# Streampunk/phaneron

Hardware: AMD Instinct MI355X
Metric: frames/sec, 4-layer 2160p50 composite pipeline (v210 unpack->CSC->combine->CSC->v210 pack) (higher is better)
Workload: dtype f32

## Files before the change

### include/phaneron_hip.h

```cpp
#ifndef PHANERON_HIP_H
#define PHANERON_HIP_H

#include <stddef.h>
#include <stdint.h>

#ifdef __cplusplus
extern "C" {
#endif

#define PH_ABI_VERSION 8

enum {
  PH_OK = 0,
  PH_E_INVALID = -1,
  PH_E_NO_DEVICE = -2,
  PH_E_HIP = -3,
  PH_E_UNKNOWN_KERNEL = -4,
  PH_E_RANGE = -5
};

typedef struct ph_ctx ph_ctx;
typedef struct ph_buf ph_buf;
typedef struct ph_program ph_program;

// ... 157 lines not shown
int ph_fused_v210_combine(ph_ctx *ctx, int queue, int n, const void *const *layers, void *out,
                          uint32_t width, uint32_t height, const void *rd_col_matrix12,
                          const void *rd_gamma_lut, const void *rd_gamut_matrix9,
                          const void *wr_col_matrix12, const void *wr_gamma_lut);
int ph_fused_v210_combine_batch(ph_ctx *ctx, int queue, int jobs, int n, const void *const *layers,
                                void *const *outs, uint32_t width, uint32_t height, const void *rd_col_matrix12,
                                const void *rd_gamma_lut, const void *rd_gamut_matrix9, const void *wr_col_matrix12,
                                const void *wr_gamma_lut);

typedef struct ph_layer {
  const void *rgba;
  int width, height;
  const void *matrix9;
} ph_layer;
int ph_compose_write_v210(ph_ctx *ctx, int queue, int n, const ph_layer *layers, void *out,
                          uint32_t out_width, uint32_t out_height, uint32_t interlace,
                          const void *wr_col_matrix12, const void *wr_gamma_lut);

typedef struct ph_layer_wipe {
  const void *incoming_rgba;
  const void *mask_rgba;
} ph_layer_wipe;
int ph_compose_wipe_write_v210(ph_ctx *ctx, int queue, int n, const ph_layer *layers, const ph_layer_wipe *wipes,
                               void *out, uint32_t out_width, uint32_t out_height, uint32_t interlace,
                               const void *wr_col_matrix12, const void *wr_gamma_lut);

typedef struct ph_image_layer {
  const void *data;
  int format;
  int width, height;
  const float *matrix9_host;
} ph_image_layer;
int ph_compose_up_write_v210(ph_ctx *ctx, int queue, int n, const ph_image_layer *layers, void *out, uint32_t out_width,
                             uint32_t out_height, uint32_t interlace, const void *wr_col_matrix12, const void *wr_gamma_lut);
int ph_compose_up_write_v210_pair(ph_ctx *ctx, int queue, int n, const ph_image_layer *layers_a, const ph_image_layer *layers_b, void *out_a,
                                  void *out_b, uint32_t out_width, uint32_t out_height, uint32_t interlace, const void *wr_col_matrix12,
                                  const void *wr_gamma_lut);
int ph_compose_up_write_v210_batch(ph_ctx *ctx, int queue, int jobs, int n, const ph_image_layer *const *layer_sets, void *const *outs,
                                   uint32_t out_width, uint32_t out_height, uint32_t interlace, const void *wr_col_matrix12,
                                   const void *wr_gamma_lut);

#define PH_SRC_NONE 0
#define PH_SRC_V210 1
#define PH_SRC_RGBA_F32 2
#define PH_SRC_YUV422P10 3
#define PH_SRC_YUV422P8 4
#define PH_SRC_YUV420P 5
#define PH_SRC_NV12 6
#define PH_SRC_RGBA8 7
#define PH_SRC_BGRA8 8
#define PH_SRC_YUV420P10 9
#define PH_SRC_P010 10
typedef struct ph_chan_source {
  const void *data;
  int format;
  int width, height;
  const float *matrix9_host;
  const void *data_u, *data_v;
  const void *col_matrix12;
} ph_chan_source;
#define PH_TRANSITION_CUT 0
#define PH_TRANSITION_DISSOLVE 1
#define PH_TRANSITION_WIPE 2
typedef struct ph_chan_layer {
  ph_chan_source src;
  int transition;
  float mix;
  ph_chan_source incoming, mask;
} ph_chan_layer;
int ph_chan_compose_v210(ph_ctx *ctx, int queue, int n, const ph_chan_layer *layers, void *out, uint32_t out_width,
                         uint32_t out_height, uint32_t interlace, const void *rd_col_matrix12, const void *rd_gamma_lut,
                         const void *rd_gamut9, const void *wr_col_matrix12, const void *wr_gamma_lut);
int ph_chan_compose(ph_ctx *ctx, int queue, int n, const ph_chan_layer *layers, int out_format, void *const out_planes[3],
                    uint32_t out_width, uint32_t out_height, uint32_t interlace, const void *rd_col_matrix12, const void *rd_gamma_lut,
                    const void *rd_gamut9, const void *wr_col_matrix12, const void *wr_gamma_lut);
typedef struct ph_chan_job {
  int n;
  const ph_chan_layer *layers;
  void *out;
  uint32_t interlace;
} ph_chan_job;
int ph_chan_compose_batch(ph_ctx *ctx, int queue, int n_jobs, const ph_chan_job *jobs, uint32_t out_width, uint32_t out_height,
                          const void *rd_col_matrix12, const void *rd_gamma_lut, const void *rd_gamut9, const void *wr_col_matrix12,
                          const void *wr_gamma_lut);
typedef struct ph_chan_output {
  int format;
  void *planes[3];
  uint32_t interlace;
  const void *wr_col_matrix12;
  const void *wr_gamma_lut;
} ph_chan_output;
int ph_chan_compose_multi(ph_ctx *ctx, int queue, int n, const ph_chan_layer *layers, int n_out, const ph_chan_output *outs,
                          uint32_t out_width, uint32_t out_height, const void *rd_col_matrix12, const void *rd_gamma_lut,
                          const void *rd_gamut9);
int ph_clip_compose_multi(ph_ctx *ctx, int queue, int n, const ph_chan_layer *layers, int n_out, const ph_chan_output *outs,
                          uint32_t out_width, uint32_t out_height, const void *rd_col_matrix12, const void *rd_gamma_lut,
                          const void *rd_gamut9);
typedef struct ph_chan_job_out {
  int n;
  const ph_chan_layer *layers;
  int n_out;
  const ph_chan_output *outs;
} ph_chan_job_out;
int ph_chan_compose_batch_out(ph_ctx *ctx, int queue, int n_jobs, const ph_chan_job_out *jobs, uint32_t out_width, uint32_t out_height,
                              const void *rd_col_matrix12, const void *rd_gamma_lut, const void *rd_gamut9);
int ph_clip_compose_batch_out(ph_ctx *ctx, int queue, int n_jobs, const ph_chan_job_out *jobs, uint32_t out_width, uint32_t out_height,
                              const void *rd_col_matrix12, const void *rd_gamma_lut, const void *rd_gamut9);
int ph_compose_up_write_multi(ph_ctx *ctx, int queue, int jobs, int n, const ph_image_layer *const *layer_sets, int n_out,
                              const ph_chan_output *outs, uint32_t out_width, uint32_t out_height);
typedef struct ph_image_trans_layer {
  ph_image_layer src;
  int transition;
  float mix;
  ph_image_layer incoming, mask;
} ph_image_trans_layer;
int ph_compose_up_transition_multi(ph_ctx *ctx, int queue, int jobs, int n, const ph_image_trans_layer *const *layer_sets, int n_out,
                                   const ph_chan_output *outs , uint32_t out_width, uint32_t out_height);
int ph_pack_write_multi(ph_ctx *ctx, int queue, const void *in, int n_out, const ph_chan_output *outs, uint32_t width,
                        uint32_t height);
int ph_fused_v210_combine_multi(ph_ctx *ctx, int queue, int n, const void *const *layers, int n_out, const ph_chan_output *outs,
                                uint32_t width, uint32_t height, const void *rd_col_matrix12, const void *rd_gamma_lut,
                                const void *rd_gamut9);
int ph_fused_v210_combine_multi_batch(ph_ctx *ctx, int queue, int jobs, int n, const void *const *layers ,
                                      int n_out, const ph_chan_output *outs , uint32_t width, uint32_t height,
                                      const void *rd_col_matrix12, const void *rd_gamma_lut, const void *rd_gamut9);
typedef struct ph_fused_layer {
  const void *v210;
  int transition;
  float mix;
  const void *incoming_v210;
  const void *mask;
  int mask_format;
} ph_fused_layer;
int ph_fused_v210_transition_multi(ph_ctx *ctx, int queue, int n, const ph_fused_layer *layers, int n_out, const ph_chan_output *outs,
                                   uint32_t width, uint32_t height, const void *rd_col_matrix12, const void *rd_gamma_lut,
                                   const void *rd_gamut9);
typedef struct ph_route_layer {
  const void *data;
  int format;
} ph_route_layer;
int ph_fused_v210_route_multi(ph_ctx *ctx, int queue, int n, const ph_route_layer *layers, void *image_out ,
                              int n_out , const ph_chan_output *outs, uint32_t width, uint32_t height, const void *rd_col_matrix12,
                              const void *rd_gamma_lut, const void *rd_gamut9);

int ph_lut_register(ph_ctx *ctx, const void *device_lut_f32, const float *host_lut65536);
int ph_lut_unregister(ph_ctx *ctx, const void *device_lut_f32);
int ph_lut_query(ph_ctx *ctx, const void *device_lut_f32, uint32_t *lds_bytes, uint32_t *index_bias,
                 uint32_t *blocks_per_octave_log2);
typedef struct ph_lut_layout {
  uint32_t lds_bytes, hole, delta_off, shift, index_bias;
  float a_scale;
} ph_lut_layout;
int ph_lut_layout_of(const float *host_lut65536, ph_lut_layout *layout, void *lds_image, size_t capacity);
int ph_ctx_set_option(ph_ctx *ctx, const char *name, int value);
int ph_debug_image_nt(ph_ctx *ctx, size_t bytes);

int ph_colour_gamma2linear_lut(const char *colspec, float *lut65536);
int ph_colour_linear2gamma_lut(const char *colspec, float *lut65536);
int ph_colour_ycbcr2rgb_matrix(const char *colspec, int num_bits, int luma_black, int luma_white,
                               int chroma_range, float *m12);
int ph_colour_rgb2ycbcr_matrix(const char *colspec, int num_bits, int luma_black, int luma_white,
                               int chroma_range, float *m12);
int ph_colour_rgb2rgb_matrix(const char *src_colspec, const char *dst_colspec, float *m9);
int ph_transform_matrix(int width, int height, int flip_h, int flip_v, double anchor_x,
                        double anchor_y, double scale_x, double scale_y, double offset_x,
                        double offset_y, double rotate, float *m9);

int ph_abi_version(void);

#ifdef __cplusplus
}
#endif
#endif
```

### phaneron_amd/capi.py

```python
import ctypes as C
import os
import sys

import numpy as np

_HERE = os.path.dirname(os.path.abspath(__file__))
LIB_PATH = os.environ.get("PHANERON_HIP_LIB") or os.path.join(_HERE, "lib", "libphaneron_hip.so")

QUEUE_LOAD, QUEUE_PROCESS, QUEUE_UNLOAD = 0, 1, 2
HOST_READONLY, HOST_WRITEONLY, HOST_NONE = 0, 1, 2
ARG_BUF, ARG_U32, ARG_I32, ARG_F32 = 0, 1, 2, 3

EXPORTS = [
    "ph_abi_version", "ph_last_error", "ph_ctx_create", "ph_ctx_destroy", "ph_ctx_info", "ph_ctx_stream",
    "ph_wait_finish", "ph_buf_create", "ph_buf_wrap", "ph_buf_addref", "ph_buf_release", "ph_buf_refcount",
    "ph_buf_bytes", "ph_buf_device_ptr", "ph_buf_dims", "ph_buf_host_access", "ph_buf_host_ptr",
    "ph_ctx_buffer_stats", "ph_program_create", "ph_program_destroy", "ph_program_kernel", "ph_run_program", "ph_check_program", "ph_chan_compose", "ph_yadif_pair_packed",
    "ph_v210_pitch_bytes", "ph_v210_read", "ph_v210_read_batch", "ph_v210_write", "ph_yadif", "ph_yadif_pair", "ph_v210_yadif_pair", "ph_transform", "ph_resize", "ph_combine",
    "ph_transition_dissolve", "ph_transition_wipe", "ph_mixer", "ph_wipe", "ph_fused_v210_combine",
    "ph_colour_gamma2linear_lut", "ph_colour_linear2gamma_lut", "ph_colour_ycbcr2rgb_matrix",
    "ph_colour_rgb2ycbcr_matrix", "ph_colour_rgb2rgb_matrix", "ph_transform_matrix",
    "ph_lut_register", "ph_lut_unregister", "ph_lut_query", "ph_lut_layout_of", "ph_compose_up_write_v210_pair", "ph_compose_up_write_v210_batch", "ph_pack_read_batch", "ph_ctx_set_option", "ph_compose_write_v210", "ph_compose_wipe_write_v210",
    "ph_pack_plane_bytes", "ph_pack_read", "ph_pack_write", "ph_queue_wait_queue", "ph_buf_download_async",
    "ph_event_record", "ph_event_wait", "ph_event_query", "ph_event_destroy", "ph_queue_query",
    "ph_graph_begin", "ph_graph_end", "ph_graph_launch", "ph_graph_destroy", "ph_fused_v210_combine_batch",
    "ph_program_resolve", "ph_route_unique_id", "ph_route_init", "ph_route_destroy", "ph_route_group_begin",
    "ph_route_group_end", "ph_route_send", "ph_route_recv", "ph_route_after_queue", "ph_queue_after_route",
    "ph_route_wait", "ph_route_stream", "ph_route_comm_count", "ph_chan_compose_v210", "ph_chan_compose_batch", "ph_run_programs", "ph_event_record_timed", "ph_event_elapsed_us", "ph_ctx_host_pool_stats",
    "ph_v210_yadif_pair_fmt", "ph_compose_up_write_v210", "ph_trace_begin", "ph_trace_end", "ph_run_programs_progress", "ph_buf_reuse", "ph_image_unpack_rgb",
    "ph_chan_compose_multi", "ph_compose_up_write_multi", "ph_chan_compose_batch_out", "ph_pack_write_multi",
    "ph_fused_v210_combine_multi",
    "ph_fused_v210_combine_multi_batch",
    "ph_compose_up_transition_multi",
    "ph_fused_v210_transition_multi",
    "ph_fused_v210_route_multi",
    "ph_debug_image_nt",
    "ph_clip_compose_multi",
    "ph_clip_compose_batch_out",
]


class PhaneronError(RuntimeError):
    pass


class _ArgVal(C.Union):
    _fields_ = [("buf", C.c_void_p), ("u32", C.c_uint32), ("i32", C.c_int32), ("f32", C.c_float)]


class PhArg(C.Structure):
    _fields_ = [("name", C.c_char_p), ("kind", C.c_int), ("v", _ArgVal)]


class PhLayer(C.Structure):
    _fields_ = [("rgba", C.c_void_p), ("width", C.c_int), ("height", C.c_int), ("matrix9", C.c_void_p)]


class PhLayerWipe(C.Structure):
    _fields_ = [("incoming_rgba", C.c_void_p), ("mask_rgba", C.c_void_p)]


class PhDeintSource(C.Structure):
    _fields_ = [("prev", C.c_void_p), ("cur", C.c_void_p), ("next", C.c_void_p), ("out_parity0", C.c_void_p), ("out_parity1", C.c_void_p),
                ("prev_u", C.c_void_p), ("prev_v", C.c_void_p), ("cur_u", C.c_void_p), ("cur_v", C.c_void_p), ("next_u", C.c_void_p), ("next_v", C.c_void_p)]


class PhChanSource(C.Structure):
    _fields_ = [("data", C.c_void_p), ("format", C.c_int), ("width", C.c_int), ("height", C.c_int),
                ("matrix9_host", C.POINTER(C.c_float)), ("data_u", C.c_void_p), ("data_v", C.c_void_p), ("col_matrix12", C.c_void_p)]


class PhChanLayer(C.Structure):
    _fields_ = [("src", PhChanSource), ("transition", C.c_int), ("mix", C.c_float), ("incoming", PhChanSource), ("mask", PhChanSource)]


class PhChanJob(C.Structure):
    _fields_ = [("n", C.c_int), ("layers", C.POINTER(PhChanLayer)), ("out", C.c_void_p), ("interlace", C.c_uint32)]


class PhChanOutput(C.Structure):
    _fields_ = [("format", C.c_int), ("planes", C.c_void_p * 3), ("interlace", C.c_uint32), ("wr_col_matrix12", C.c_void_p), ("wr_gamma_lut", C.c_void_p)]


class PhChanJobOut(C.Structure):
    _fields_ = [("n", C.c_int), ("layers", C.POINTER(PhChanLayer)), ("n_out", C.c_int), ("outs", C.POINTER(PhChanOutput))]


class PhImageLayer(C.Structure):
    _fields_ = [("data", C.c_void_p), ("format", C.c_int), ("width", C.c_int), ("height", C.c_int), ("matrix9_host", C.POINTER(C.c_float))]


class PhImageTransLayer(C.Structure):
    _fields_ = [("src", PhImageLayer), ("transition", C.c_int), ("mix", C.c_float), ("incoming", PhImageLayer), ("mask", PhImageLayer)]


class PhRouteLayer(C.Structure):
    _fields_ = [("data", C.c_void_p), ("format", C.c_int)]


class PhFusedLayer(C.Structure):
    _fields_ = [("v210", C.c_void_p), ("transition", C.c_int), ("mix", C.c_float), ("incoming_v210", C.c_void_p), ("mask", C.c_void_p), ("mask_format", C.c_int)]


IMG_RGBA_F32, IMG_RGB_F32 = 0, 1
SRC_V210, SRC_RGBA_F32, SRC_YUV422P10, SRC_YUV422P8, SRC_YUV420P, SRC_NV12, SRC_RGBA8, SRC_BGRA8 = 1, 2, 3, 4, 5, 6, 7, 8
SRC_YUV420P10, SRC_P010 = 9, 10
SRC_PLANAR = {"yuv422p10": SRC_YUV422P10, "yuv422p8": SRC_YUV422P8, "yuv420p": SRC_YUV420P, "nv12": SRC_NV12,
              "yuv420p10": SRC_YUV420P10, "p010": SRC_P010}
TRANSITION_CUT, TRANSITION_DISSOLVE, TRANSITION_WIPE = 0, 1, 2


class LutLayout(C.Structure):
    _fields_ = [("lds_bytes", C.c_uint32), ("hole", C.c_uint32), ("delta_off", C.c_uint32), ("shift", C.c_uint32), ("index_bias", C.c_uint32),
                ("a_scale", C.c_float)]


class RunTimings(C.Structure):
    _fields_ = [("data_to_kernel", C.c_uint32), ("kernel_exec", C.c_uint32), ("total_time", C.c_uint32)]


_lib = None


def lib():
    global _lib
    if _lib is not None:
        return _lib
    if not os.path.exists(LIB_PATH):
        raise PhaneronError("%s is missing: build it with `python -m phaneron_amd.build` "
                            "(there is no CPU fallback)" % LIB_PATH)
    if "torch" not in sys.modules and os.environ.get("PH_NO_TORCH_PRELOAD") != "1":
        import importlib.util
        if importlib.util.find_spec("torch") is not None:
            import torch
    l = C.CDLL(LIB_PATH)
    vp, ci, cu, cf, cd, cs = C.c_void_p, C.c_int, C.c_uint32, C.c_float, C.c_double, C.c_size_t
    f32p = np.ctypeslib.ndpointer(dtype=np.float32, flags="C_CONTIGUOUS")
    sig = {
        "ph_abi_version": (ci, []),
        "ph_last_error": (C.c_char_p, [vp]),
        "ph_ctx_create": (ci, [ci, C.POINTER(vp)]),
        "ph_ctx_destroy": (ci, [vp]),
        "ph_ctx_info": (ci, [vp, C.c_char_p, cs, C.c_char_p, cs]),
        "ph_ctx_stream": (vp, [vp, ci]),
        "ph_wait_finish": (ci, [vp, ci]),
        "ph_buf_create": (ci, [vp, cs, ci, ci, ci, ci, C.c_char_p, C.POINTER(vp)]),
        "ph_buf_wrap": (ci, [vp, vp, cs, ci, ci, C.POINTER(vp)]),
        "ph_buf_addref": (ci, [vp]),
        "ph_buf_release": (ci, [vp]),
        "ph_buf_refcount": (ci, [vp]),
        "ph_buf_bytes": (cs, [vp]),
        "ph_buf_device_ptr": (vp, [vp]),
        "ph_buf_dims": (ci, [vp, C.POINTER(ci), C.POINTER(ci)]),
        "ph_buf_host_access": (ci, [vp, ci, ci, vp, cs]),
        "ph_buf_host_ptr": (vp, [vp]),
        "ph_queue_wait_queue": (ci, [vp, ci, ci]),
        "ph_buf_download_async": (ci, [vp, ci]),
        "ph_queue_query": (ci, [vp, ci]),
        "ph_graph_begin": (ci, [vp, ci]),
        "ph_graph_end": (ci, [vp, ci, C.POINTER(vp)]),
        "ph_graph_launch": (ci, [vp, ci]),
        "ph_graph_destroy": (ci, [vp]),
        "ph_event_record": (ci, [vp, ci, C.POINTER(vp)]),
        "ph_event_wait": (ci, [vp]),
        "ph_event_query": (ci, [vp]),
        "ph_event_destroy": (ci, [vp]),
        "ph_ctx_buffer_stats": (ci, [vp, C.POINTER(cs), C.POINTER(cs), C.POINTER(cs)]),
        "ph_program_create": (ci, [vp, C.c_char_p, C.c_char_p, C.POINTER(cu), ci, cu, C.POINTER(vp)]),
        "ph_program_resolve": (ci, [C.c_char_p, C.c_char_p, C.c_char_p, cs, C.POINTER(ci), C.POINTER(ci)]),
        "ph_program_destroy": (ci, [vp]),
        "ph_program_kernel": (C.c_char_p, [vp]),
        "ph_run_program": (ci, [vp, vp, C.POINTER(PhArg), ci, ci, C.POINTER(RunTimings)]),
        "ph_check_program": (ci, [vp, vp, C.POINTER(PhArg), ci, ci]),
        "ph_v210_pitch_bytes": (cu, [cu]),
        "ph_v210_read": (ci, [vp, ci, vp, vp, cu, cu, vp, vp, vp]),
        "ph_v210_read_batch": (ci, [vp, ci, ci, vp, vp, cu, cu, vp, vp, vp]),
        "ph_v210_write": (ci, [vp, ci, vp, vp, cu, cu, cu, vp, vp]),
        "ph_yadif": (ci, [vp, ci, vp, vp, vp, ci, ci, ci, ci, ci, vp]),
        "ph_yadif_pair": (ci, [vp, ci, vp, vp, vp, ci, ci, ci, ci, vp, vp]),
        "ph_v210_yadif_pair": (ci, [vp, ci, ci, vp, cu, cu, ci, ci, vp, vp, vp]),
        "ph_v210_yadif_pair_fmt": (ci, [vp, ci, ci, vp, cu, cu, ci, ci, ci, vp, vp, vp]),
        "ph_yadif_pair_packed": (ci, [vp, ci, ci, vp, ci, cu, cu, ci, ci, ci, vp, vp, vp]),
        "ph_transform": (ci, [vp, ci, vp, ci, ci, vp, vp, ci, ci]),
        "ph_resize": (ci, [vp, ci, vp, ci, ci, cf, cf, cf, vp, vp, ci, ci]),
        "ph_combine": (ci, [vp, ci, ci, C.POINTER(vp), ci, ci, vp]),
        "ph_transition_dissolve": (ci, [vp, ci, vp, vp, cf, ci, ci, vp]),
        "ph_transition_wipe": (ci, [vp, ci, vp, vp, vp, ci, ci, vp]),
        "ph_mixer": (ci, [vp, ci, vp, vp, cf, ci, ci, vp]),
        "ph_wipe": (ci, [vp, ci, vp, vp, cf, ci, ci, vp]),
        "ph_fused_v210_combine": (ci, [vp, ci, ci, C.POINTER(vp), vp, cu, cu, vp, vp, vp, vp, vp]),
        "ph_fused_v210_combine_batch": (ci, [vp, ci, ci, ci, C.POINTER(vp), C.POINTER(vp), cu, cu, vp, vp, vp, vp, vp]),
        "ph_colour_gamma2linear_lut": (ci, [C.c_char_p, f32p]),
        "ph_colour_linear2gamma_lut": (ci, [C.c_char_p, f32p]),
        "ph_colour_ycbcr2rgb_matrix": (ci, [C.c_char_p, ci, ci, ci, ci, f32p]),
        "ph_colour_rgb2ycbcr_matrix": (ci, [C.c_char_p, ci, ci, ci, ci, f32p]),
        "ph_colour_rgb2rgb_matrix": (ci, [C.c_char_p, C.c_char_p, f32p]),
        "ph_transform_matrix": (ci, [ci, ci, ci, ci, cd, cd, cd, cd, cd, cd, cd, f32p]),
        "ph_lut_register": (ci, [vp, vp, f32p]),
        "ph_lut_unregister": (ci, [vp, vp]),
        "ph_lut_query": (ci, [vp, vp, C.POINTER(cu), C.POINTER(cu), C.POINTER(cu)]),
        "ph_lut_layout_of": (ci, [f32p, C.POINTER(LutLayout), vp, C.c_size_t]),
        "ph_compose_up_write_v210_pair": (ci, [vp, ci, ci, C.POINTER(PhImageLayer), C.POINTER(PhImageLayer), vp, vp, cu, cu, cu, vp, vp]),
        "ph_compose_up_write_v210_batch": (ci, [vp, ci, ci, ci, C.POINTER(C.POINTER(PhImageLayer)), C.POINTER(vp), cu, cu, cu, vp, vp]),
        "ph_pack_read_batch": (ci, [vp, ci, ci, ci, C.POINTER(vp * 3), C.POINTER(vp), cu, cu, vp, vp, vp]),
        "ph_ctx_set_option": (ci, [vp, C.c_char_p, ci]),
        "ph_pack_plane_bytes": (ci, [ci, cu, cu, C.POINTER(cs)]),
        "ph_pack_read": (ci, [vp, ci, ci, C.POINTER(vp), vp, cu, cu, vp, vp, vp]),
        "ph_pack_write": (ci, [vp, ci, ci, vp, C.POINTER(vp), cu, cu, cu, vp, vp]),
        "ph_compose_write_v210": (ci, [vp, ci, ci, C.POINTER(PhLayer), vp, cu, cu, cu, vp, vp]),
        "ph_compose_wipe_write_v210": (ci, [vp, ci, ci, C.POINTER(PhLayer), C.POINTER(PhLayerWipe), vp, cu, cu, cu, vp, vp]),
        "ph_compose_up_write_v210": (ci, [vp, ci, ci, C.POINTER(PhImageLayer), vp, cu, cu, cu, vp, vp]),
        "ph_chan_compose_v210": (ci, [vp, ci, ci, C.POINTER(PhChanLayer), vp, cu, cu, cu, vp, vp, vp, vp, vp]),
        "ph_chan_compose": (ci, [vp, ci, ci, C.POINTER(PhChanLayer), ci, C.POINTER(C.c_void_p), cu, cu, cu, vp, vp, vp, vp, vp]),
        "ph_chan_compose_batch": (ci, [vp, ci, ci, C.POINTER(PhChanJob), cu, cu, vp, vp, vp, vp, vp]),
        "ph_chan_compose_multi": (ci, [vp, ci, ci, C.POINTER(PhChanLayer), ci, C.POINTER(PhChanOutput), cu, cu, vp, vp, vp]),
        "ph_clip_compose_multi": (ci, [vp, ci, ci, C.POINTER(PhChanLayer), ci, C.POINTER(PhChanOutput), cu, cu, vp, vp, vp]),
        "ph_compose_up_write_multi": (ci, [vp, ci, ci, ci, C.POINTER(C.POINTER(PhImageLayer)), ci, C.POINTER(PhChanOutput), cu, cu]),
        "ph_compose_up_transition_multi": (ci, [vp, ci, ci, ci, C.POINTER(C.POINTER(PhImageTransLayer)), ci, C.POINTER(PhChanOutput), cu, cu]),
        "ph_pack_write_multi": (ci, [vp, ci, vp, ci, C.POINTER(PhChanOutput), cu, cu]),
        "ph_fused_v210_combine_multi": (ci, [vp, ci, ci, C.POINTER(C.c_void_p), ci, C.POINTER(PhChanOutput), cu, cu, vp, vp, vp]),
        "ph_fused_v210_transition_multi": (ci, [vp, ci, ci, C.POINTER(PhFusedLayer), ci, C.POINTER(PhChanOutput), cu, cu, vp, vp, vp]),
        "ph_fused_v210_route_multi": (ci, [vp, ci, ci, C.POINTER(PhRouteLayer), vp, ci, C.POINTER(PhChanOutput), cu, cu, vp, vp, vp]),
        "ph_fused_v210_combine_multi_batch": (ci, [vp, ci, ci, ci, C.POINTER(C.c_void_p), ci, C.POINTER(PhChanOutput), cu, cu, vp, vp, vp]),
        "ph_chan_compose_batch_out": (ci, [vp, ci, ci, C.POINTER(PhChanJobOut), cu, cu, vp, vp, vp]),
        "ph_clip_compose_batch_out": (ci, [vp, ci, ci, C.POINTER(PhChanJobOut), cu, cu, vp, vp, vp]),
        "ph_ctx_host_pool_stats": (ci, [vp, C.POINTER(C.c_size_t), C.POINTER(C.c_size_t), C.POINTER(C.c_size_t), C.POINTER(C.c_uint64)]),
        "ph_event_record_timed": (ci, [vp, ci, C.POINTER(vp)]),
        "ph_event_elapsed_us": (ci, [vp, vp, C.POINTER(cu)]),
        "ph_run_programs": (ci, [vp, ci, C.POINTER(vp), C.POINTER(C.POINTER(PhArg)), C.POINTER(ci), ci]),
        "ph_route_unique_id": (ci, [vp]),
        "ph_route_init": (ci, [vp, vp, ci, ci, C.POINTER(vp)]),
        "ph_route_destroy": (ci, [vp]),
        "ph_route_group_begin": (ci, [vp]),
        "ph_route_group_end": (ci, [vp]),
        "ph_route_send": (ci, [vp, vp, cs, ci]),
        "ph_route_recv": (ci, [vp, vp, cs, ci]),
        "ph_route_after_queue": (ci, [vp, ci]),
        "ph_queue_after_route": (ci, [vp, ci]),
        "ph_route_wait": (ci, [vp]),
        "ph_route_stream": (vp, [vp]),
        "ph_route_comm_count": (ci, [vp, C.POINTER(C.c_int)]),
        "ph_run_programs_progress": (ci, [C.POINTER(ci)]),
        "ph_buf_reuse": (ci, [vp]),
        "ph_image_unpack_rgb": (ci, [vp, ci, vp, ci, ci]),
        "ph_trace_begin": (ci, [ci]),
        "ph_trace_end": (ci, [C.c_char_p, cs]),
        "ph_debug_image_nt": (ci, [vp, cs]),
    }
    for name, (res, args) in sig.items():
        fn = getattr(l, name)
        fn.restype, fn.argtypes = res, args
    _lib = l
    return l


def check(rc, ctx=None):
    if rc != 0:
        msg = lib().ph_last_error(ctx)
        raise PhaneronError("libphaneron_hip error %d: %s" % (rc, msg.decode() if msg else "?"))


class trace:

    def __init__(self, dry_run=False):
        self.dry_run, self.route = dry_run, None

    def __enter__(self):
        check(lib().ph_trace_begin(1 if self.dry_run else 0))
        return self

    def __exit__(self, *exc):
        buf = C.create_string_buffer(4096)
        rc = lib().ph_trace_end(buf, len(buf))
        if exc[0] is None:
            check(rc)
        self.route = buf.value.decode()
        return False

    @property
    def kernels(self):
        return self.route.split("+") if self.route else []


def lut_layout(lut):
    lut = np.ascontiguousarray(lut, np.float32)
    assert lut.shape == (65536,)
    lay = LutLayout()
    n = lib().ph_lut_layout_of(lut, C.byref(lay), None, 0)
    if n < 0:
        check(n)
    if n == 0:
        return None, None
    image = np.zeros(n, np.uint8)
    if lib().ph_lut_layout_of(lut, C.byref(lay), image.ctypes.data_as(C.c_void_p), n) != n:
        check(-1)
    return {k: getattr(lay, k) for k, _ in LutLayout._fields_}, image


def gamma2linear_lut(colspec):
    out = np.empty(65536, np.float32)
    check(lib().ph_colour_gamma2linear_lut(colspec.encode(), out))
    return out


def linear2gamma_lut(colspec):
    out = np.empty(65536, np.float32)
    check(lib().ph_colour_linear2gamma_lut(colspec.encode(), out))
    return out


def ycbcr2rgb_matrix(colspec, num_bits=10, luma_black=64, luma_white=940, chroma_range=896):
    out = np.empty(12, np.float32)
    check(lib().ph_colour_ycbcr2rgb_matrix(colspec.encode(), num_bits, luma_black, luma_white, chroma_range, out))
    return out


def rgb2ycbcr_matrix(colspec, num_bits=10, luma_black=64, luma_white=940, chroma_range=896):
    out = np.empty(12, np.float32)
    check(lib().ph_colour_rgb2ycbcr_matrix(colspec.encode(), num_bits, luma_black, luma_white, chroma_range, out))
    return out


def rgb2rgb_matrix(src, dst):
    out = np.empty(9, np.float32)
    check(lib().ph_colour_rgb2rgb_matrix(src.encode(), dst.encode(), out))
    return out


def transform_matrix(width, height, flip_h=False, flip_v=False, anchor_x=0.0, anchor_y=0.0, scale_x=1.0,
                     scale_y=1.0, offset_x=0.0, offset_y=0.0, rotate=0.0):
    out = np.empty(9, np.float32)
    check(lib().ph_transform_matrix(width, height, int(flip_h), int(flip_v), anchor_x, anchor_y, scale_x, scale_y,
                                    offset_x, offset_y, rotate, out))
    return out


RESOLVED_HOW = {0: "tag", 1: "name", 2: "text", 3: "signature"}


def resolve_program(source, name):
    buf = C.create_string_buffer(64)
    fmt, how = C.c_int(), C.c_int()
    src = source.encode() if isinstance(source, str) else source
    check(lib().ph_program_resolve(src, name.encode(), buf, 64, C.byref(fmt), C.byref(how)))
    names = {v: k for k, v in FORMATS.items()}
    return buf.value.decode(), names.get(fmt.value), RESOLVED_HOW[how.value]


def v210_pitch_bytes(width):
    return int(lib().ph_v210_pitch_bytes(width))


FORMATS = {"v210": 0, "yuv422p10": 1, "yuv422p8": 2, "yuv420p": 3, "nv12": 4, "rgba8": 5, "bgra8": 6, "yuv420p10": 7, "p010": 8}
FORMAT_RANGE = {"v210": (10, 64, 940, 896), "yuv422p10": (10, 64, 940, 896), "yuv422p8": (8, 16, 235, 224),
                "yuv420p": (8, 16, 235, 224), "nv12": (8, 16, 235, 224), "rgba8": None, "bgra8": None,
                "yuv420p10": (10, 64, 940, 896), "p010": (10, 64, 940, 896)}


def pack_plane_bytes(fmt, width, height):
    b = (C.c_size_t * 3)()
    n = lib().ph_pack_plane_bytes(FORMATS[fmt], width, height, b)
    if n < 0:
        check(n)
    return [int(b[i]) for i in range(n)]


def _ptr(t):
    return C.c_void_p(t if isinstance(t, int) else t.data_ptr())


class Context:

    def __init__(self, device_index=0):
        h = C.c_void_p()
        check(lib().ph_ctx_create(device_index, C.byref(h)))
        self.h = h
        self.device_index = device_index

    def close(self):
        if self.h:
            lib().ph_ctx_destroy(self.h)
            self.h = None

    def __enter__(self):
        return self

    def __exit__(self, *a):
        self.close()

    def info(self):
        v, d = C.create_string_buffer(128), C.create_string_buffer(256)
        check(lib().ph_ctx_info(self.h, v, 128, d, 256), self.h)
        return v.value.decode(), d.value.decode()

    def stream_ptr(self, queue=QUEUE_PROCESS):
        return lib().ph_ctx_stream(self.h, queue)

    def torch_stream(self, queue=QUEUE_PROCESS):
        import torch
        return torch.cuda.ExternalStream(self.stream_ptr(queue), device=torch.device("cuda", self.device_index))

    def wait(self, queue=QUEUE_PROCESS):
        check(lib().ph_wait_finish(self.h, queue), self.h)

    def register_lut(self, device_lut, host_lut):
        rc = lib().ph_lut_register(self.h, _ptr(device_lut), np.ascontiguousarray(host_lut, np.float32))
        if rc < 0:
            check(rc, self.h)
        return rc == 1

    def unregister_lut(self, device_lut):
        check(lib().ph_lut_unregister(self.h, _ptr(device_lut)), self.h)

    def lut_info(self, device_lut):
        b, t, s = C.c_uint32(), C.c_uint32(), C.c_uint32()
        check(lib().ph_lut_query(self.h, _ptr(device_lut), C.byref(b), C.byref(t), C.byref(s)), self.h)
        return dict(lds_bytes=b.value, index_bias=t.value, blocks_per_octave_log2=s.value)

    def set_option(self, name, value):
        check(lib().ph_ctx_set_option(self.h, name.encode(), int(value)), self.h)

    def debug_image_nt(self, nbytes):
        rc = lib().ph_debug_image_nt(self.h, int(nbytes))
        if rc < 0:
            check(rc, self.h)
        return rc

    def v210_read(self, src, dst, width, height, col_matrix, lut, gamut, queue=QUEUE_PROCESS):
        check(lib().ph_v210_read(self.h, queue, _ptr(src), _ptr(dst), width, height, _ptr(col_matrix), _ptr(lut),
                                 _ptr(gamut)), self.h)

    def v210_read_batch(self, srcs, dsts, width, height, col_matrix, lut, gamut, queue=QUEUE_PROCESS):
        n = len(srcs)
        ins = (C.c_void_p * n)(*[_ptr(b).value for b in srcs])
        outs = (C.c_void_p * n)(*[_ptr(b).value for b in dsts])
        check(lib().ph_v210_read_batch(self.h, queue, n, ins, outs, width, height, _ptr(col_matrix), _ptr(lut), _ptr(gamut)), self.h)

    def v210_write(self, src, dst, width, height, interlace, col_matrix, lut, queue=QUEUE_PROCESS):
        check(lib().ph_v210_write(self.h, queue, _ptr(src), _ptr(dst), width, height, interlace, _ptr(col_matrix),
                                  _ptr(lut)), self.h)

    def yadif(self, prev, cur, nxt, dst, width, height, parity, tff, skip_spatial=False, queue=QUEUE_PROCESS):
        check(lib().ph_yadif(self.h, queue, _ptr(prev), _ptr(cur), _ptr(nxt), width, height, int(parity), int(tff),
                             int(skip_spatial), _ptr(dst)), self.h)

    def yadif_pair(self, prev, cur, nxt, dst_parity0, dst_parity1, width, height, tff, skip_spatial=False, queue=QUEUE_PROCESS):
        check(lib().ph_yadif_pair(self.h, queue, _ptr(prev), _ptr(cur), _ptr(nxt), width, height, int(tff), int(skip_spatial),
                                  _ptr(dst_parity0), _ptr(dst_parity1)), self.h)

    def v210_yadif_pair(self, sources, width, height, tff, skip_spatial, col_matrix, lut, gamut, queue=QUEUE_PROCESS, rgb=False,
                        prepare_only=False, packing="v210"):
        arr = (PhDeintSource * len(sources))()
        for i, s in enumerate(sources):
            if packing == "v210":
                arr[i].prev, arr[i].cur, arr[i].next = (_ptr(b).value for b in s[:3])
            else:
                (arr[i].prev, arr[i].prev_u, arr[i].prev_v), (arr[i].cur, arr[i].cur_u, arr[i].cur_v), (arr[i].next, arr[i].next_u, arr[i].next_v) = (
                    (tuple(_ptr(p).value for p in frame) + (None,))[:3] for frame in s[:3])
            arr[i].out_parity0, arr[i].out_parity1 = _ptr(s[3]).value, _ptr(s[4]).value
        args = (self.h, queue, len(sources), arr, FORMATS[packing], width, height, int(tff), int(skip_spatial), IMG_RGB_F32 if rgb else IMG_RGBA_F32,
                _ptr(col_matrix), _ptr(lut), _ptr(gamut))
        if prepare_only:
            fn, h = lib().ph_yadif_pair_packed, self.h

            def job(_keep=(sources,)):
                check(fn(*args), h)
            return job
        check(lib().ph_yadif_pair_packed(*args), self.h)

    def compose_up_write_v210_pair(self, layers_a, layers_b, dst_a, dst_b, out_w, out_h, interlace, wr_cm, wr_lut, queue=QUEUE_PROCESS, rgb=False,
                                   prepare_only=False):
        import numpy as np
        keep = []

        def arr_of(layers):
            arr = (PhImageLayer * len(layers))()
            for i, (t, w, h, m) in enumerate(layers):
                mh = np.ascontiguousarray(m, np.float32)
                keep.append(mh)
                arr[i].data, arr[i].width, arr[i].height = _ptr(t).value, w, h
                arr[i].format = IMG_RGB_F32 if rgb else IMG_RGBA_F32
                arr[i].matrix9_host = mh.ctypes.data_as(C.POINTER(C.c_float))
            return arr
        assert len(layers_a) == len(layers_b)
        aa, ab = arr_of(layers_a), arr_of(layers_b)
        args = (self.h, queue, len(layers_a), aa, ab, _ptr(dst_a), _ptr(dst_b), out_w, out_h, interlace, _ptr(wr_cm), _ptr(wr_lut))
        if prepare_only:
            fn, h = lib().ph_compose_up_write_v210_pair, self.h

            def job(_keep=(keep, layers_a, layers_b, dst_a, dst_b, aa, ab)):
                check(fn(*args), h)
            return job
        check(lib().ph_compose_up_write_v210_pair(*args), self.h)

    def compose_up_write_v210_batch(self, layer_sets, dsts, out_w, out_h, interlace, wr_cm, wr_lut, queue=QUEUE_PROCESS, rgb=False, prepare_only=False):
        import numpy as np
        keep = []
        arrs = []
        for layers in layer_sets:
            arr = (PhImageLayer * len(layers))()
            for i, (t, w, h, m) in enumerate(layers):
                mh = np.ascontiguousarray(m, np.float32)
                keep.append(mh)
                arr[i].data, arr[i].width, arr[i].height = _ptr(t).value, w, h
                arr[i].format = IMG_RGB_F32 if rgb else IMG_RGBA_F32
                arr[i].matrix9_host = mh.ctypes.data_as(C.POINTER(C.c_float))
            arrs.append(arr)
        sets = (C.POINTER(PhImageLayer) * len(arrs))(*[C.cast(a, C.POINTER(PhImageLayer)) for a in arrs])
        outs = (C.c_void_p * len(dsts))(*[_ptr(d).value for d in dsts])
        args = (self.h, queue, len(layer_sets), len(layer_sets[0]), sets, outs, out_w, out_h, interlace, _ptr(wr_cm), _ptr(wr_lut))
        if prepare_only:
            fn, h = lib().ph_compose_up_write_v210_batch, self.h

            def job(_keep=(keep, arrs, layer_sets, dsts, sets, outs)):
                check(fn(*args), h)
            return job
        check(lib().ph_compose_up_write_v210_batch(*args), self.h)

    def compose_up_write_v210(self, layers, dst, out_w, out_h, interlace, wr_cm, wr_lut, queue=QUEUE_PROCESS, rgb=False, prepare_only=False):
        import numpy as np
        arr = (PhImageLayer * len(layers))()
        keep = []
        for i, (t, w, h, m) in enumerate(layers):
            mh = np.ascontiguousarray(m, np.float32)
            keep.append(mh)
            arr[i].data, arr[i].width, arr[i].height = _ptr(t).value, w, h
            arr[i].format = IMG_RGB_F32 if rgb else IMG_RGBA_F32
            arr[i].matrix9_host = mh.ctypes.data_as(C.POINTER(C.c_float))
        args = (self.h, queue, len(layers), arr, _ptr(dst), out_w, out_h, interlace, _ptr(wr_cm), _ptr(wr_lut))
        if prepare_only:
            fn, h = lib().ph_compose_up_write_v210, self.h

            def job(_keep=(keep, layers, dst)):
                check(fn(*args), h)
            return job
        check(lib().ph_compose_up_write_v210(*args), self.h)

    def compose_up_write_multi(self, layer_sets, outputs, out_w, out_h, queue=QUEUE_PROCESS, rgb=False, prepare_only=False):
        import numpy as np
        keep = []
        arrs = []
        for layers in layer_sets:
            arr = (PhImageLayer * len(layers))()
            for i, (t, w, h, m) in enumerate(layers):
                mh = np.ascontiguousarray(m, np.float32)
                keep.append(mh)
                arr[i].data, arr[i].width, arr[i].height = _ptr(t).value, w, h
                arr[i].format = IMG_RGB_F32 if rgb else IMG_RGBA_F32
                arr[i].matrix9_host = mh.ctypes.data_as(C.POINTER(C.c_float))
            arrs.append(arr)
        sets = (C.POINTER(PhImageLayer) * len(arrs))(*[C.cast(a, C.POINTER(PhImageLayer)) for a in arrs])
        n_out = len(outputs[0])
        outs = (PhChanOutput * max(len(outputs) * n_out, 1))()
        for j, per_job in enumerate(outputs):
            if len(per_job) != n_out:
                raise PhaneronError("compose_up_write_multi: every set of layers needs the same number of outputs")
            for k, o in enumerate(per_job):
                d = outs[j * n_out + k]
                planes = o["planes"] if isinstance(o["planes"], (list, tuple)) else [o["planes"]]
                d.format = FORMATS[o["fmt"]]
                for i, p in enumerate(planes):
                    d.planes[i] = _ptr(p).value
                d.interlace = int(o.get("interlace", 0))
                d.wr_col_matrix12 = None if o.get("wr_cm") is None else _ptr(o["wr_cm"]).value
                d.wr_gamma_lut = _ptr(o["wr_lut"]).value
        args = (self.h, queue, len(layer_sets), len(layer_sets[0]), sets, n_out, outs, out_w, out_h)
        fn, h = lib().ph_compose_up_write_multi, self.h
        if prepare_only:

            def job(_keep=(keep, arrs, layer_sets, outputs, sets, outs)):
# ... 580 lines not shown
```

### phaneron_amd/csrc/ph_api.cpp

```cpp
#include <algorithm>
#include <atomic>
#include <chrono>
#include <cstdarg>
#include <cstdio>
#include <cstring>
#include <dlfcn.h>
#include <map>
#include <mutex>
#include <string>
#include <vector>

#include "../../include/phaneron_hip.h"
#include "ph_internal.h"
#include "ph_kernels.h"
#include "ph_lut_host.h"

using ph::KernelId;
using namespace ph;

namespace {
thread_local std::string g_err;
}

int fail(int code, const char *fmt, ...) {
// ... 632 lines not shown
int ph_route_unique_id(void *id128) {
  if (!id128) return fail(PH_E_INVALID, "ph_route_unique_id: NULL argument");
  int rc = load_rccl();
  if (rc) return rc;
  static_assert(PH_ROUTE_ID_BYTES == sizeof(Id128), "ncclUniqueId is 128 bytes");
  PH_NCCL(g_rccl.GetUniqueId(id128));
  return PH_OK;
}

int ph_route_init(ph_ctx *ctx, const void *id128, int rank, int world, ph_route **out) {
  if (!ctx || !id128 || !out) return fail(PH_E_INVALID, "ph_route_init: NULL argument");
  if (world < 1 || rank < 0 || rank >= world) return fail(PH_E_INVALID, "ph_route_init: rank %d of %d", rank, world);
  int rc = set_device(ctx);
  if (rc) return rc;
  rc = load_rccl();
  if (rc) return rc;
  Id128 id;
  memcpy(id.bytes, id128, sizeof id.bytes);
  void *comm = nullptr;
  PH_NCCL(g_rccl.CommInitRank(&comm, world, id, rank));
  hipStream_t s = nullptr;
  hipError_t e = hipStreamCreateWithFlags(&s, hipStreamNonBlocking);
  if (e != hipSuccess) {
    g_rccl.CommDestroy(comm);
    return fail(PH_E_HIP, "ph_route_init: hipStreamCreate: %s", hipGetErrorString(e));
  }
  hipEvent_t ev = nullptr;
  e = hipEventCreateWithFlags(&ev, hipEventDisableTiming);
  if (e != hipSuccess) {
    g_rccl.CommDestroy(comm);
    hipStreamDestroy(s);
    return fail(PH_E_HIP, "ph_route_init: hipEventCreate: %s", hipGetErrorString(e));
  }
  ph_route *r = new ph_route{ctx, comm, s, rank, world};
  r->last = ev;
  {
    std::lock_guard<std::mutex> lock(ctx->mu);
    ctx->routes.push_back(r);
  }
  *out = r;
  ctx_ref(ctx);
  return PH_OK;
}

int ph_route_destroy(ph_route *r) {
  if (!r) return PH_OK;
  hipSetDevice(r->ctx->device);
  hipStreamSynchronize(r->stream);
  ph_ctx *ctx = r->ctx;
  {
    std::lock_guard<std::mutex> lock(ctx->mu);
    for (size_t i = 0; i < ctx->routes.size(); ++i)
      if (ctx->routes[i] == r) {
        ctx->routes.erase(ctx->routes.begin() + (long)i);
        break;
      }
  }
  g_rccl.CommDestroy(r->comm);
  hipStreamDestroy(r->stream);
  if (r->last) hipEventDestroy(r->last);
  delete r;
  ctx_unref(ctx);
  return PH_OK;
}

int ph_route_group_begin(ph_route *r) {
  if (!r) return fail(PH_E_INVALID, "ph_route_group_begin: NULL route");
  PH_NCCL(g_rccl.GroupStart());
  r->in_group = true;
  return PH_OK;
}
int ph_route_group_end(ph_route *r) {
  if (!r) return fail(PH_E_INVALID, "ph_route_group_end: NULL route");
  int rc = set_device(r->ctx);
  if (rc) return rc;
  PH_NCCL(g_rccl.GroupEnd());
  r->in_group = false;
  return route_mark(r);
}

static int route_args(ph_route *r, const void *p, size_t bytes, int peer, const char *fn) {
  if (!r || !p) return fail(PH_E_INVALID, "%s: NULL argument", fn);
  if (bytes % 4) return fail(PH_E_INVALID, "%s: %zu bytes is not a multiple of 4", fn, bytes);
  if (peer < 0 || peer >= r->world) return fail(PH_E_INVALID, "%s: peer %d of %d ranks", fn, peer, r->world);
  return set_device(r->ctx);
}
int ph_route_send(ph_route *r, const void *src, size_t bytes, int peer) {
  int rc = route_args(r, src, bytes, peer, "ph_route_send");
  if (rc) return rc;
  PH_NCCL(g_rccl.Send(src, bytes / 4, kNcclUint32, peer, r->comm, r->stream));
  return r->in_group ? PH_OK : route_mark(r);
}
int ph_route_recv(ph_route *r, void *dst, size_t bytes, int peer) {
  int rc = route_args(r, dst, bytes, peer, "ph_route_recv");
  if (rc) return rc;
  PH_NCCL(g_rccl.Recv(dst, bytes / 4, kNcclUint32, peer, r->comm, r->stream));
  return r->in_group ? PH_OK : route_mark(r);
}

static int order_streams(ph_ctx *ctx, hipStream_t waiter, hipStream_t signal, const char *fn) {
  int rc = set_device(ctx);
  if (rc) return rc;
  hipEvent_t ev;
  PH_HIP(hipEventCreateWithFlags(&ev, hipEventDisableTiming));
  hipError_t e = hipEventRecord(ev, signal);
  if (e == hipSuccess) e = hipStreamWaitEvent(waiter, ev, 0);
  hipEventDestroy(ev);
  if (e != hipSuccess) return fail(PH_E_HIP, "%s: %s", fn, hipGetErrorString(e));
  return PH_OK;
}
int ph_route_after_queue(ph_route *r, int queue) {
  if (!r || queue < 0 || queue > 2) return fail(PH_E_INVALID, "ph_route_after_queue: bad argument");
  return order_streams(r->ctx, r->stream, r->ctx->streams[queue], "ph_route_after_queue");
}
int ph_queue_after_route(ph_route *r, int queue) {
  if (!r || queue < 0 || queue > 2) return fail(PH_E_INVALID, "ph_queue_after_route: bad argument");
  return order_streams(r->ctx, r->ctx->streams[queue], r->stream, "ph_queue_after_route");
}
int ph_route_wait(ph_route *r) {
  if (!r) return fail(PH_E_INVALID, "ph_route_wait: NULL route");
  int rc = set_device(r->ctx);
  if (rc) return rc;
  PH_HIP(hipStreamSynchronize(r->stream));
  return PH_OK;
}
void *ph_route_stream(ph_route *r) { return r ? (void *)r->stream : nullptr; }
int ph_route_comm_count(ph_route *r, int *count) {
  if (!r || !count) return fail(PH_E_INVALID, "ph_route_comm_count: NULL argument");
  PH_NCCL(g_rccl.CommCount(r->comm, count));
  return PH_OK;
}

int ph_ctx_buffer_stats(ph_ctx *ctx, size_t *live_buffers, size_t *live_bytes, size_t *pooled_bytes) {
  if (!ctx) return fail(PH_E_INVALID, "ph_ctx_buffer_stats: ctx is NULL");
  std::lock_guard<std::mutex> lock(ctx->mu);
  if (live_buffers) *live_buffers = ctx->live_buffers;
  if (live_bytes) *live_bytes = ctx->live_bytes;
  if (pooled_bytes) *pooled_bytes = ctx->pooled_bytes;
  return PH_OK;
}

int ph_ctx_host_pool_stats(ph_ctx *ctx, size_t *in_use_bytes, size_t *pooled_bytes, size_t *peak_in_use_bytes, uint64_t *pins) {
  if (!ctx) return fail(PH_E_INVALID, "ph_ctx_host_pool_stats: ctx is NULL");
  std::lock_guard<std::mutex> lock(ctx->mu);
  if (in_use_bytes) *in_use_bytes = ctx->host_live_bytes;
  if (pooled_bytes) *pooled_bytes = ctx->host_pooled_bytes;
  if (peak_in_use_bytes) *peak_in_use_bytes = ctx->host_peak_bytes;
  if (pins) *pins = ctx->host_pins;
  return PH_OK;
}

int ph_lut_unregister(ph_ctx *ctx, const void *dev) {
  if (!ctx) return fail(PH_E_INVALID, "ph_lut_unregister: ctx is NULL");
  void *blob = nullptr;
  {
    std::lock_guard<std::mutex> lock(ctx->mu);
    auto it = ctx->luts.find(dev);
    if (it == ctx->luts.end()) return PH_OK;
    blob = it->second.blob_dev;
    ctx->luts.erase(it);
  }
  if (blob) {
    for (int q = 0; q < 3; ++q) hipStreamSynchronize(ctx->streams[q]);
    hipFree(blob);
  }
  return PH_OK;
}

int ph_lut_register(ph_ctx *ctx, const void *dev, const float *host) {
  if (!ctx || !dev || !host) return fail(PH_E_INVALID, "ph_lut_register: NULL argument");
  int rc = set_device(ctx);
  if (rc) return rc;
  ph_lut_unregister(ctx, dev);
  std::vector<uint32_t> blob;
  ph::LutHostInfo info;
  LutEntry e;
  if (ph::lut_compress(host, ph::kLutMaxLdsBytes, blob, info)) {
    if (!ctx->lds_base_checked.load()) {
      uint32_t *probe = nullptr, base = ~0u;
      PH_HIP(hipMalloc(&probe, 4));
      hipError_t pe = ph::launch_lds_base_probe(ctx->streams[0], probe);
      if (pe == hipSuccess) pe = hipStreamSynchronize(ctx->streams[0]);
      if (pe == hipSuccess) pe = hipMemcpy(&base, probe, 4, hipMemcpyDeviceToHost);
      hipFree(probe);
      if (pe != hipSuccess) return fail(PH_E_HIP, "ph_lut_register: LDS base probe: %s", hipGetErrorString(pe));
      if (base != 0) return fail(PH_E_HIP, "ph_lut_register: dynamic shared memory starts at LDS address %u, not 0: the table kernels cannot run", base);
      ctx->lds_base_checked.store(true);
    }
    const size_t blob_bytes = blob.size() * sizeof(uint32_t);
    PH_HIP(hipMalloc(&e.blob_dev, blob_bytes));
    PH_HIP(hipMemcpy(e.blob_dev, blob.data(), blob_bytes, hipMemcpyHostToDevice));
    e.view = ph::lut_view(info, e.blob_dev);
  }
  {
    std::lock_guard<std::mutex> lock(ctx->mu);
    ctx->luts[dev] = e;
  }
  return e.view.bytes ? 1 : 0;
}

int ph_lut_layout_of(const float *host, ph_lut_layout *layout, void *lds_image, size_t capacity) {
  if (!host || !layout) return fail(PH_E_INVALID, "ph_lut_layout_of: NULL argument");
  std::vector<uint32_t> blob;
  ph::LutHostInfo info;
  memset(layout, 0, sizeof(*layout));
  if (!ph::lut_compress(host, ph::kLutMaxLdsBytes, blob, info)) return 0;
  const ph::LutView v = ph::lut_view(info, nullptr);
  layout->lds_bytes = info.bytes, layout->hole = info.hole, layout->delta_off = info.delta_off, layout->shift = info.shift;
  layout->index_bias = (uint32_t)info.bias, layout->a_scale = v.a_scale;
  if (lds_image) {
    if (capacity < info.bytes) return fail(PH_E_INVALID, "ph_lut_layout_of: the image needs %u bytes, %zu given", info.bytes, capacity);
    memset(lds_image, 0, info.hole);
    memcpy(static_cast<char *>(lds_image) + info.hole, blob.data(), info.bytes - info.hole);
  }
  return (int)info.bytes;
}

int ph_debug_fused_lut_k(const float *host, uint32_t k5[5]) {
  if (!host || !k5) return fail(PH_E_INVALID, "ph_debug_fused_lut_k: NULL argument");
  std::vector<uint32_t> blob;
  ph::LutHostInfo info;
  if (!ph::lut_compress(host, ph::kLutMaxLdsBytes, blob, info)) return 0;
  const ph::FusedLutK k = ph::fused_lut_k(ph::lut_view(info, nullptr));
  memcpy(k5, &k, 5 * sizeof(uint32_t));
  return (int)info.bytes;
}
uint32_t ph_debug_fused_job_of(uint32_t wg_per_job, uint32_t block) {
  return wg_per_job ? ph::fused_job_of(block, ph::fused_wg_magic(wg_per_job)) : 0;
}
int ph_debug_image_nt(ph_ctx *ctx, size_t bytes) {
  if (!ctx) return fail(PH_E_INVALID, "ph_debug_image_nt: ctx is NULL");
  if (int rc = set_device(ctx)) return rc;
  return (int)ph::image_nt(bytes);
}

int ph_lut_query(ph_ctx *ctx, const void *dev, uint32_t *lds_bytes, uint32_t *toe, uint32_t *shift) {
  if (!ctx) return fail(PH_E_INVALID, "ph_lut_query: ctx is NULL");
  std::lock_guard<std::mutex> lock(ctx->mu);
  auto it = ctx->luts.find(dev);
  const bool have = it != ctx->luts.end();
  if (lds_bytes) *lds_bytes = have ? it->second.view.bytes : 0;
  if (toe) *toe = have ? (uint32_t)it->second.view.bias : 0;
  if (shift) *shift = have ? 23 - it->second.view.shift : 0;
  return PH_OK;
}

int ph_ctx_set_option(ph_ctx *ctx, const char *name, int value) {
  if (!ctx || !name) return fail(PH_E_INVALID, "ph_ctx_set_option: NULL argument");
  if (0 == strcmp(name, "lds_lut")) return ctx->use_lds_lut = (value != 0), PH_OK;
  if (0 == strcmp(name, "stream_images")) {
    if (value < 0 || value > 2) return fail(PH_E_INVALID, "stream_images: 0 (cached), 1 (streamed) or 2 (by size)");
    return ctx->stream_images = value, PH_OK;
  }
  if (0 == strcmp(name, "stream_threshold_mb")) {
    if (value < 0) return fail(PH_E_INVALID, "stream_threshold_mb: a size in MiB");
    return ctx->stream_threshold_mb = value, PH_OK;
  }
  if (0 == strcmp(name, "fail_launches")) return ctx->fail_launches.store(value), PH_OK;
  if (0 == strcmp(name, "chan_enlarged")) return ctx->chan_enlarged = (value < 0 || value > 2 ? 1 : value), PH_OK;
  if (0 == strcmp(name, "chan_batch_outs")) {
    if (value != 0 && value != 1) return fail(PH_E_INVALID, "chan_batch_outs: 0 (a launch per such job) or 1 (shared launches)");
    return ctx->chan_batch_outs = value, PH_OK;
  }
  if (0 == strcmp(name, "clip_batch")) {
    if (value != 0 && value != 1) return fail(PH_E_INVALID, "clip_batch: 0 (a launch per such job) or 1 (shared launches)");
    return ctx->clip_batch = value, PH_OK;
  }
  if (0 == strcmp(name, "fused_multi_wgs")) {
    if (value < 0) return fail(PH_E_INVALID, "fused_multi_wgs: a number of workgroups, or 0 for no cap");
    return ctx->fused_multi_wgs = value, PH_OK;
  }
  if (0 == strcmp(name, "fused_multi_batch")) {
    if (value != 0 && value != 1) return fail(PH_E_INVALID, "fused_multi_batch: 0 (a launch per such job) or 1 (shared launches)");
    return ctx->fused_multi_batch = value, PH_OK;
  }
  if (0 == strcmp(name, "host_pool_mb")) {
    if (value < 0) return fail(PH_E_INVALID, "host_pool_mb: a size in MiB");
    std::vector<ph_ctx::HostBlock> drop;
    {
      std::lock_guard<std::mutex> lock(ctx->mu);
      ctx->host_pool_mb = value;
      ctx->host_peak_bytes = ctx->host_live_bytes;
      while (ctx->host_pooled_bytes > (size_t)value << 20 && !ctx->host_pool.empty()) {
        auto it = std::prev(ctx->host_pool.end());
        ctx->host_pooled_bytes -= it->first;
        drop.push_back(it->second);
        ctx->host_pool.erase(it);
      }
    }
    for (auto &v : drop) {
      hipHostFree(v.p);
      if (v.busy) hipEventDestroy(v.busy);
    }
    return PH_OK;
  }
  return fail(PH_E_INVALID, "unknown option '%s'", name);
}

struct LutRef {
  ph::LutView view{};
  bool found = false;
  const ph::LutView *get() const { return found ? &view : nullptr; }
};
static LutRef lds_view(ph_ctx *ctx, const void *dev) {
  LutRef r;
  if (!ctx || !ctx->use_lds_lut) return r;
  std::lock_guard<std::mutex> lock(ctx->mu);
  auto it = ctx->luts.find(dev);
  if (it == ctx->luts.end() || !it->second.view.bytes) return r;
  r.view = it->second.view, r.found = true;
  return r;
}

extern "C++" void refresh_buf_lut(ph_ctx *ctx, ph_buf *b) {
  if (b->lut_dirty && b->hptr && b->bytes >= 65536 * 4) {
    hipStreamSynchronize(ctx->streams[PH_QUEUE_LOAD]);
    ph_lut_register(ctx, b->dptr, (const float *)b->hptr);
    b->lut_dirty = false;
  }
}

extern "C++" int chan_out_refused(const char *fn, int fmt) {
  return fail(PH_E_INVALID, "%s: the channel kernel does not write %s frames - run the separate kernels: the channel's frame as an image, then the format's writer (ph_pack_write)", fn,
              fmt_name(fmt));
}

extern "C++" bool inject_failure(ph_ctx *ctx) {
  const int v = ctx->fail_launches.load();
  if (v > 0) return true;
  if (v < 0 && ctx->fail_launches.fetch_add(1) == -1) ctx->fail_launches.store(1);
  return false;
}

uint32_t ph_v210_pitch_bytes(uint32_t width) { return width ? ph::v210_pitch_bytes(width) : 0; }

#define PH_LAUNCH(expr)                                                                         \
  do {                                                                                          \
    if (!ctx) return fail(PH_E_INVALID, "%s: ctx is NULL", __func__);                           \
    PH_QUEUE(__func__, queue);                                                                  \
    int rc_ = set_device(ctx);                                                                  \
    if (rc_) return rc_;                                                                        \
    hipError_t e_ = ph::trace_launch(#expr) ? hipSuccess : (expr);                              \
    if (e_ != hipSuccess) return fail(PH_E_HIP, "%s: launch failed: %s", __func__, hipGetErrorString(e_)); \
    return PH_OK;                                                                               \
  } while (0)

int ph_v210_read(ph_ctx *ctx, int queue, const void *in, void *out, uint32_t width, uint32_t height, const void *cm,
                 const void *lut, const void *gm) {
  if (!in || !out || !cm || !lut || !gm || !width) return fail(PH_E_INVALID, "ph_v210_read: NULL/zero argument");
  if (!height) return PH_OK;
  if (ctx && width % 2 == 0) {
    const LutRef lref = lds_view(ctx, lut);
    if (const ph::LutView *v = lref.get())
      PH_LAUNCH(ph::launch_v210_read_lds(stream_of(ctx, queue), in, out, width, height, cm, gm, *v,
                                         (uint32_t)ctx->props.multiProcessorCount));
  }
  PH_LAUNCH(ph::launch_v210_read(stream_of(ctx, queue), in, out, width, height, cm, lut, gm));
}

int ph_v210_read_batch(ph_ctx *ctx, int queue, int n, const void *const *ins, void *const *outs, uint32_t width,
                       uint32_t height, const void *cm, const void *lut, const void *gm) {
  if (n < 1 || n > ph::kMaxLayers) return fail(PH_E_INVALID, "ph_v210_read_batch: 1..%d frames", ph::kMaxLayers);
  if (!ins || !outs || !cm || !lut || !gm || !width) return fail(PH_E_INVALID, "ph_v210_read_batch: NULL/zero argument");
  for (int i = 0; i < n; ++i)
    if (!ins[i] || !outs[i]) return fail(PH_E_INVALID, "ph_v210_read_batch: frame %d is NULL", i);
  if (!height) return PH_OK;
  if (ctx && width % 2 == 0) {
    const LutRef lref = lds_view(ctx, lut);
    if (const ph::LutView *v = lref.get())
      PH_LAUNCH(ph::launch_v210_read_lds_batch(stream_of(ctx, queue), n, ins, outs, width, height, cm, gm, *v,
                                               (uint32_t)ctx->props.multiProcessorCount));
  }
  for (int i = 0; i < n; ++i) {
    const int rc = ph_v210_read(ctx, queue, ins[i], outs[i], width, height, cm, lut, gm);
    if (rc) return rc;
  }
  return PH_OK;
}

int ph_v210_write(ph_ctx *ctx, int queue, const void *in, void *out, uint32_t width, uint32_t height,
                  uint32_t interlace, const void *cm, const void *lut) {
  if (!in || !out || !cm || !lut || !width) return fail(PH_E_INVALID, "ph_v210_write: NULL/zero argument");
  if (interlace != 0 && interlace != 1 && interlace != 3) return fail(PH_E_INVALID, "ph_v210_write: interlace must be 0, 1 or 3");
  if (!height) return PH_OK;
  if (ctx && width % 2 == 0) {
    const LutRef lref = lds_view(ctx, lut);
    if (const ph::LutView *v = lref.get())
      PH_LAUNCH(ph::launch_v210_write_lds(stream_of(ctx, queue), in, out, width, height, interlace, cm, *v,
                                          (uint32_t)ctx->props.multiProcessorCount));
  }
  PH_LAUNCH(ph::launch_v210_write(stream_of(ctx, queue), in, out, width, height, interlace, cm, lut));
}

int ph_fused_v210_combine(ph_ctx *ctx, int queue, int n, const void *const *layers, void *out, uint32_t width,
                          uint32_t height, const void *rd_cm, const void *rd_lut, const void *rd_gm,
                          const void *wr_cm, const void *wr_lut) {
  if (n < 1 || n > ph::kMaxLayers) return fail(PH_E_INVALID, "ph_fused_v210_combine: 1..%d layers", ph::kMaxLayers);
  if (!layers || !out || !rd_cm || !rd_lut || !rd_gm || !wr_cm || !wr_lut || !width)
    return fail(PH_E_INVALID, "ph_fused_v210_combine: NULL/zero argument");
  const bool ragged = width % 48 != 0;
  if (width & 1) return fail(PH_E_INVALID, "ph_fused_v210_combine: width %u is odd; run the separate kernels", width);
  if (!height) return PH_OK;
  ph::FusedArgs a{};
  for (int i = 0; i < n; ++i) {
    if (!layers[i]) return fail(PH_E_INVALID, "ph_fused_v210_combine: layer %d is NULL", i);
    a.layers[i] = layers[i];
  }
  a.out = out;
  a.quads_per_line_used = width / 6;
  a.quads_per_line_pitch = ph::v210_pitch_bytes(width) / 16;
  a.total_quads = (ragged ? a.quads_per_line_pitch : a.quads_per_line_used) * height;
  a.tail_px = width % 6, a.magic_qpp = (uint32_t)(((1ull << 32) + a.quads_per_line_pitch - 1) / a.quads_per_line_pitch);
  if (ragged && (uint64_t)a.total_quads * a.quads_per_line_pitch >= (1ull << 32))
    return fail(PH_E_INVALID, "ph_fused_v210_combine: a %u x %u frame with ragged lines is too large; run the separate kernels", width, height);
  a.rd_cm = (const float *)rd_cm, a.rd_lut = (const float *)rd_lut, a.rd_gm = (const float *)rd_gm;
  a.wr_cm = (const float *)wr_cm, a.wr_lut = (const float *)wr_lut;
  if (ctx) {
    const LutRef rref = lds_view(ctx, rd_lut), wref = lds_view(ctx, wr_lut);
    const ph::LutView *rv = rref.get(), *wv = wref.get();
    if (rv && wv) {
      const ph::FusedLdsArgs la = ph::fused_lds_args(a, *rv, *wv);
      PH_LAUNCH(ph::launch_fused_v210_combine_lds(stream_of(ctx, queue), n, la, (uint32_t)ctx->props.multiProcessorCount));
    }
  }
  PH_LAUNCH(ph::launch_fused_v210_combine(stream_of(ctx, queue), n, a));
}

int ph_pack_plane_bytes(int format, uint32_t width, uint32_t height, size_t bytes[3]) {
  if (!bytes || !width) return fail(PH_E_INVALID, "ph_pack_plane_bytes: NULL/zero argument");
  if (const int rc = even_dims("ph_pack_plane_bytes", format, width, height)) return rc;
  const int n = ph::pack_plane_bytes(format, width, height, bytes);
  return n < 0 ? fail(PH_E_INVALID, "ph_pack_plane_bytes: unknown format %d", format) : n;
}

int ph_fused_v210_combine_batch(ph_ctx *ctx, int queue, int jobs, int n, const void *const *layers, void *const *outs,
                                uint32_t width, uint32_t height, const void *rd_cm, const void *rd_lut, const void *rd_gm,
                                const void *wr_cm, const void *wr_lut) {
  if (jobs < 1 || jobs > ph::kMaxBatch) return fail(PH_E_INVALID, "ph_fused_v210_combine_batch: 1..%d jobs", ph::kMaxBatch);
  if (n < 1 || n > ph::kMaxLayers) return fail(PH_E_INVALID, "ph_fused_v210_combine_batch: 1..%d layers", ph::kMaxLayers);
  if (!layers || !outs || !rd_cm || !rd_lut || !rd_gm || !wr_cm || !wr_lut)
    return fail(PH_E_INVALID, "ph_fused_v210_combine_batch: NULL argument");
  for (int j = 0; j < jobs; ++j) {
    if (!outs[j]) return fail(PH_E_INVALID, "ph_fused_v210_combine_batch: output %d is NULL", j);
    for (int l = 0; l < n; ++l)
      if (!layers[j * n + l]) return fail(PH_E_INVALID, "ph_fused_v210_combine_batch: job %d layer %d is NULL", j, l);
  }
  const LutRef rref = lds_view(ctx, rd_lut), wref = lds_view(ctx, wr_lut);
  const ph::LutView *rv = rref.get(), *wv = wref.get();
  if (jobs == 1 || !rv || !wv || !width || width % 48 || !height) {
    for (int j = 0; j < jobs; ++j) {
      int rc = ph_fused_v210_combine(ctx, queue, n, layers + (size_t)j * n, outs[j], width, height, rd_cm, rd_lut, rd_gm,
                                     wr_cm, wr_lut);
      if (rc != PH_OK) return rc;
    }
    return PH_OK;
  }
  ph::FusedArgs f{};
  for (int l = 0; l < n; ++l) f.layers[l] = layers[l];
  f.out = outs[0];
  f.quads_per_line_used = width / 6;
  f.quads_per_line_pitch = ph::v210_pitch_bytes(width) / 16;
  f.total_quads = f.quads_per_line_used * height;
  f.rd_cm = (const float *)rd_cm, f.rd_lut = (const float *)rd_lut, f.rd_gm = (const float *)rd_gm;
  f.wr_cm = (const float *)wr_cm, f.wr_lut = (const float *)wr_lut;
  ph::FusedLdsArgs la = ph::fused_lds_args(f, *rv, *wv);
  la.jobs = (uint32_t)jobs;
  for (int j = 1; j < jobs; ++j) {
    for (int l = 0; l < n; ++l) la.more_layers[j - 1][l] = layers[(size_t)j * n + l];
    la.more_out[j - 1] = outs[j];
  }
  PH_LAUNCH(ph::launch_fused_v210_combine_lds(stream_of(ctx, queue), n, la, (uint32_t)ctx->props.multiProcessorCount));
}

int ph_pack_read(ph_ctx *ctx, int queue, int format, const void *const planes[3], void *out, uint32_t width,
                 uint32_t height, const void *cm, const void *lut, const void *gm) {
  if (!ctx || !planes || !out || !lut || !gm || !width) return fail(PH_E_INVALID, "ph_pack_read: NULL/zero argument");
  if (format == PH_FMT_V210) return ph_v210_read(ctx, queue, planes[0], out, width, height, cm, lut, gm);
  if (const int rc = even_dims("ph_pack_read", format, width, height)) return rc;
  size_t pb[3];
  const int np = ph::pack_plane_bytes(format, width, height, pb);
  if (np < 0) return fail(PH_E_INVALID, "ph_pack_read: unknown format %d", format);
  for (int i = 0; i < np; ++i)
    if (!planes[i]) return fail(PH_E_INVALID, "ph_pack_read: plane %d is NULL", i);
  if (!fmt_rgb8(format) && !cm) return fail(PH_E_INVALID, "ph_pack_read: YCbCr formats need a colMatrix");
  if (!height) return PH_OK;
  PH_LAUNCH(ph::launch_pack_read(stream_of(ctx, queue), format, planes, out, width, height, cm, lut, gm, lds_view(ctx, lut).get(),
                                 (uint32_t)ctx->props.multiProcessorCount));
}

int ph_pack_read_batch(ph_ctx *ctx, int queue, int format, int n, const void *const (*planes)[3], void *const *outs, uint32_t width, uint32_t height,
                       const void *cm, const void *lut, const void *gm) {
  if (!ctx || !planes || !outs || !lut || !gm || !width) return fail(PH_E_INVALID, "ph_pack_read_batch: NULL/zero argument");
  if (n < 1 || n > ph::kMaxLayers) return fail(PH_E_INVALID, "ph_pack_read_batch: 1..%d frames", ph::kMaxLayers);
  if (const int rc = even_dims("ph_pack_read_batch", format, width, height)) return rc;
  const LutRef lref = lds_view(ctx, lut);
  const ph::LutView *v = format == PH_FMT_V210 ? nullptr : lref.get();
  if (n == 1 || !v) {
    if (format == PH_FMT_V210) {
      const void *ins[ph::kMaxLayers];
      for (int i = 0; i < n; ++i) ins[i] = planes[i][0];
      return ph_v210_read_batch(ctx, queue, n, ins, outs, width, height, cm, lut, gm);
    }
    for (int i = 0; i < n; ++i) {
      const int rc = ph_pack_read(ctx, queue, format, planes[i], outs[i], width, height, cm, lut, gm);
      if (rc) return rc;
    }
    return PH_OK;
  }
  size_t pb[3];
  const int np = ph::pack_plane_bytes(format, width, height, pb);
  if (np < 0) return fail(PH_E_INVALID, "ph_pack_read_batch: unknown format %d", format);
  for (int i = 0; i < n; ++i) {
    if (!outs[i]) return fail(PH_E_INVALID, "ph_pack_read_batch: output %d is NULL", i);
    for (int k = 0; k < np; ++k)
      if (!planes[i][k]) return fail(PH_E_INVALID, "ph_pack_read_batch: frame %d: plane %d is NULL", i, k);
  }
  if (!fmt_rgb8(format) && !cm) return fail(PH_E_INVALID, "ph_pack_read_batch: YCbCr formats need a colMatrix");
  if (!height) return PH_OK;
  PH_LAUNCH(ph::launch_pack_read_batch(stream_of(ctx, queue), format, n, planes, outs, width, height, cm, gm, *v, (uint32_t)ctx->props.multiProcessorCount));
}

int ph_pack_write(ph_ctx *ctx, int queue, int format, const void *in, void *const planes[3], uint32_t width,
                  uint32_t height, uint32_t interlace, const void *cm, const void *lut) {
  if (!ctx || !planes || !in || !lut || !width) return fail(PH_E_INVALID, "ph_pack_write: NULL/zero argument");
  if (interlace != 0 && interlace != 1 && interlace != 3) return fail(PH_E_INVALID, "ph_pack_write: interlace must be 0, 1 or 3");
  if (format == PH_FMT_V210) return ph_v210_write(ctx, queue, in, planes[0], width, height, interlace, cm, lut);
  if (const int rc = even_dims("ph_pack_write", format, width, height)) return rc;
  size_t pb[3];
  const int np = ph::pack_plane_bytes(format, width, height, pb);
  if (np < 0) return fail(PH_E_INVALID, "ph_pack_write: unknown format %d", format);
  for (int i = 0; i < np; ++i)
    if (!planes[i]) return fail(PH_E_INVALID, "ph_pack_write: plane %d is NULL", i);
  if (!fmt_rgb8(format) && !cm) return fail(PH_E_INVALID, "ph_pack_write: YCbCr formats need a colMatrix");
  if (!height) return PH_OK;
  PH_LAUNCH(ph::launch_pack_write(stream_of(ctx, queue), format, in, planes, width, height, interlace, cm, lut,
                                  lds_view(ctx, lut).get(), (uint32_t)ctx->props.multiProcessorCount));
}

int ph_pack_write_multi(ph_ctx *ctx, int queue, const void *in, int n_out, const ph_chan_output *outs, uint32_t width, uint32_t height) {
  const char *const fn = "ph_pack_write_multi";
  if (!ctx || !in || !outs || !width) return fail(PH_E_INVALID, "%s: NULL/zero argument", fn);
  if (n_out < 1 || n_out > ph::kMaxPackOuts) return fail(PH_E_INVALID, "%s: 1..%d outputs (%d)", fn, ph::kMaxPackOuts, n_out);
  if (n_out == 1)
    return ph_pack_write(ctx, queue, outs[0].format, in, outs[0].planes, width, height, outs[0].interlace, outs[0].wr_col_matrix12, outs[0].wr_gamma_lut);
  PH_QUEUE(fn, queue);
  for (int k = 0; k < n_out; ++k) {
    const ph_chan_output &o = outs[k];
    if (!o.wr_gamma_lut) return fail(PH_E_INVALID, "%s: output %d: the writer's gamma LUT is missing", fn, k);
    if (!fmt_known(o.format)) return fail(PH_E_INVALID, "%s: output %d: unknown format %d", fn, k, o.format);
    if (o.interlace != 0 && o.interlace != 1 && o.interlace != 3) return fail(PH_E_INVALID, "%s: output %d: interlace must be 0, 1 or 3", fn, k);
    if (const int rc = even_dims(fn, o.format, width, height)) return rc;
    for (int i = 0; i < fmt_planes(o.format); ++i)
      if (!o.planes[i]) return fail(PH_E_INVALID, "%s: output %d: plane %d is NULL", fn, k, i);
    if (!fmt_rgb8(o.format) && !o.wr_col_matrix12) return fail(PH_E_INVALID, "%s: output %d: YCbCr formats need a colMatrix", fn, k);
    for (int j = 0; j < k; ++j)
      if (outs[j].planes[0] == o.planes[0]) return fail(PH_E_INVALID, "%s: outputs %d and %d name the same plane", fn, j, k);
  }
  if (!height) return PH_OK;
  struct Launch {
    int solo;
    ph::PackMultiArgs m;
  };
  std::vector<Launch> launches;
  for (int k = 0; k < n_out; ++k) {
    bool seen = false;
    for (int j = 0; j < k; ++j) seen = seen || outs[j].wr_gamma_lut == outs[k].wr_gamma_lut;
    if (seen) continue;
    const LutRef wref = lds_view(ctx, outs[k].wr_gamma_lut);
    int group[ph::kMaxPackOuts], members = 0, share = 0;
    bool shared_ok[ph::kMaxPackOuts];
    for (int j = k; j < n_out; ++j) {
      if (outs[j].wr_gamma_lut != outs[k].wr_gamma_lut) continue;
      const int f = outs[j].format;
      shared_ok[members] = wref.get() && !(f == PH_FMT_V210 && width % 48) && !(fmt_planar(f) && width % 8);
      share += shared_ok[members] ? 1 : 0;
      group[members++] = j;
    }
    Launch shared{};
    shared.solo = -1;
    for (int g = 0; g < members; ++g) {
      const ph_chan_output &o = outs[group[g]];
      if (!shared_ok[g] || share < 2) {
        Launch own{};
        own.solo = group[g];
        launches.push_back(own);
        continue;
      }
      ph::PackOut &d = shared.m.out[shared.m.n_out++];
      d.fmt = (uint32_t)o.format;
      d.pitch = o.format == PH_FMT_V210 ? width / 6u : ph::pack_pitch(o.format, width);
      d.wr_cm = fmt_rgb8(o.format) ? nullptr : (const float *)o.wr_col_matrix12;
      for (int i = 0; i < 3; ++i) d.plane[i] = i < fmt_planes(o.format) ? o.planes[i] : nullptr;
      d.takes = o.interlace;
    }
    if (!shared.m.n_out) continue;
    ph::PackMultiArgs &m = shared.m;
    const uint32_t first_il = m.out[0].takes;
    bool same_lines = true;
    for (uint32_t i = 0; i < m.n_out; ++i) same_lines = same_lines && m.out[i].takes == first_il;
    const uint32_t il = same_lines ? first_il : 0u;
    m.in = in, m.width = width, m.wr = *wref.get();
    m.line_step = il ? 2 : 1, m.first_line = il == 3 ? 1 : 0, m.lines = il ? height / 2 : height;
    for (uint32_t i = 0; i < m.n_out; ++i) {
      ph::PackOut &d = m.out[i];
      const uint32_t oil = d.takes;
      d.takes = same_lines || !oil ? 0u : oil == 1 ? 1u : 2u;
      d.line_end = oil || fmt_v420((int)d.fmt) ? 2u * (height / 2u) : height;
      d.field = oil ? 1u : 0u;
    }
    launches.push_back(shared);
  }
  int rc = set_device(ctx);
  if (rc) return rc;
  for (const Launch &l : launches) {
    if (l.solo >= 0) {
      const ph_chan_output &o = outs[l.solo];
      if ((rc = ph_pack_write(ctx, queue, o.format, in, o.planes, width, height, o.interlace, o.wr_col_matrix12, o.wr_gamma_lut))) return rc;
      continue;
// ... 1670 lines not shown
```

### phaneron_amd/csrc/ph_internal.h

```cpp
#pragma once
#include <atomic>
#include <cstdlib>
#include <map>
#include <mutex>
#include <string>
#include <vector>

#include "../../include/phaneron_hip.h"
#include "ph_kernels.h"
#include "ph_program.h"
#include "ph_spans.h"

static_assert(ph::kSpanLayers == ph::kMaxLayers && ph::kSpanOuts >= ph::kMaxChanOuts && ph::kSpanOuts >= ph::kMaxFusedOuts && ph::kSpanOuts >= ph::kMaxUpOuts,
              "a Footprint holds any job's ranges: ph_spans.h sizes it by these limits without seeing ph_kernels.h");
static_assert(ph::kMaxChanOps <= ph::kSpanLayers * 3, "a channel job's op list is at most three sources per layer");

#pragma GCC visibility push(hidden)
int fail(int code, const char *fmt, ...) __attribute__((format(printf, 2, 3)));
#pragma GCC visibility pop

#define PH_HIP(call)                                                                          \
  do {                                                                                        \
    hipError_t e_ = (call);                                                                   \
    if (e_ != hipSuccess) return fail(PH_E_HIP, "%s failed: %s", #call, hipGetErrorString(e_)); \
  } while (0)

struct LutEntry {
  ph::LutView view{};
  void *blob_dev = nullptr;
};

struct ph_ctx {
  int device = 0;
  std::map<const void *, LutEntry> luts;
  bool use_lds_lut = true;
  int stream_images = 0;
  int stream_threshold_mb = 64;
  hipStream_t streams[3] = {nullptr, nullptr, nullptr};
  hipDeviceProp_t props;
  std::multimap<size_t, void *> pool;
  size_t pooled_bytes = 0, live_buffers = 0, live_bytes = 0;
  struct HostBlock {
    void *p;
    hipEvent_t busy;
    uint64_t seq;
  };
  std::multimap<size_t, HostBlock> host_pool;
  size_t host_pooled_bytes = 0;
  uint64_t host_pool_seq = 0;
  int chan_enlarged = !(getenv("PH_CHAN_ENLARGED") && getenv("PH_CHAN_ENLARGED")[0] == '0');
  int chan_batch_outs = 0;
  int clip_batch = 0;
  int fused_multi_wgs = 0;
  int fused_multi_batch = 0;
  std::atomic<int> fail_launches{0};
  int host_pool_mb = 4096;
  size_t host_live_bytes = 0, host_peak_bytes = 0;
  uint64_t host_pins = 0;
  void *chan_index[3] = {nullptr, nullptr, nullptr};
  size_t chan_index_bytes[3] = {0, 0, 0};
  std::mutex chan_scratch_mu[3];
  unsigned chan_scratch_turn[3] = {0, 0, 0};
  std::vector<struct ph_route *> routes;
  std::mutex mu;
  std::atomic<int> refs{1};
  std::atomic<bool> closed{false};
  std::atomic<bool> lds_base_checked{false};
};

struct ph_buf {
  ph_ctx *ctx;
  void *dptr;
  void *hptr;
  size_t bytes;
  int width, height;
  std::atomic<int> refs;
  bool owned;
  std::atomic<bool> host_dirty;
  std::atomic<bool> lut_dirty;
  std::string owner;
  hipEvent_t mirror_busy = nullptr;
  hipStream_t mirror_stream = nullptr;
};

struct ph_program {
  ph_ctx *ctx;
  ph::KernelId id;
  int n_layers;
  int format;
  std::string kernel;
  uint32_t global[2];
  uint32_t local;
};

#pragma GCC visibility push(hidden)
int set_device(ph_ctx *ctx);
void ctx_ref(ph_ctx *ctx);
void ctx_unref(ph_ctx *ctx);
int closed_error(const char *fn);
void refresh_buf_lut(ph_ctx *ctx, ph_buf *b);
void mirror_mark(ph_buf *b, hipStream_t s);
int chan_out_refused(const char *fn, int fmt);
bool inject_failure(ph_ctx *ctx);

inline bool queue_ok(int queue) { return queue >= 0 && queue < 3; }
inline int bad_queue(const char *fn, int queue) {
  return fail(PH_E_INVALID, "%s: queue %d is not PH_QUEUE_LOAD (0), PH_QUEUE_PROCESS (1) or PH_QUEUE_UNLOAD (2)", fn, queue);
}
#pragma GCC visibility pop
#define stream_of(ctx, queue)                                  \
  ({                                                           \
    const int ph_q_ = (queue);                                 \
    if (!queue_ok(ph_q_)) return bad_queue(__func__, ph_q_);   \
    (ctx)->streams[ph_q_];                                     \
  })
#define PH_QUEUE(fn, queue)                        \
  do {                                             \
    if (!queue_ok(queue)) return bad_queue(fn, queue); \
  } while (0)
```

### phaneron_amd/csrc/ph_kernels.h

```cpp
#pragma once
#include <hip/hip_runtime.h>
#include <stddef.h>
#include <stdint.h>

#include "ph_formats.h"
#include "ph_lut.h"

namespace ph {

constexpr int kMaxLayers = 8;
constexpr int kMaxDynamicLds = 160 * 1024;

extern thread_local uint32_t t_stream_images;
extern thread_local uint32_t t_stream_threshold_mb;
static inline uint32_t image_nt(size_t bytes) {
  return t_stream_images == 2 ? (bytes > ((size_t)t_stream_threshold_mb << 20) ? 1u : 0u) : t_stream_images;
}

struct FusedArgs {
  const void *layers[kMaxLayers];
  void *out;
  uint32_t quads_per_line_used;
  uint32_t quads_per_line_pitch;
  uint32_t total_quads;
  const float *rd_cm, *rd_lut, *rd_gm, *wr_cm, *wr_lut;
  uint32_t tail_px, magic_qpp;
};

constexpr int kMaxBatch = 8;
struct FusedLutK {
  float a_scale, a_base, delta_scale, delta_base;
  uint32_t a_shift;
};
FusedLutK fused_lut_k(const LutView &v);

static inline uint32_t fused_wg_magic(uint32_t wg_per_job) { return (uint32_t)(((1ull << 31) + wg_per_job - 1) / wg_per_job); }
static inline __host__ __device__ uint32_t fused_job_of(uint32_t block, uint32_t magic) {
#if defined(__HIP_DEVICE_COMPILE__)
  return __umulhi(2u * block + 1u, magic);
#else
  return (uint32_t)(((uint64_t)(2u * block + 1u) * magic) >> 32);
#endif
}

struct alignas(64) FusedLdsArgs {
  const uint32_t *rd_blob;
  uint32_t rd_bytes, rd_hole;
  uint32_t total_quads;
  uint32_t wg_per_job;
  uint32_t per_wg;
  uint32_t magic_wg;
  const void *layers[kMaxLayers];
  void *out;
  const float *rd_cm, *rd_gm, *wr_cm;
  FusedLutK rd_k, wr_k;
  uint32_t wr_bytes, wr_hole;
  const uint32_t *wr_blob;
  uint32_t jobs;
  uint32_t quads_per_line_used;
  uint32_t quads_per_line_pitch;
  uint32_t tail_px, magic_qpp;
  const void *more_layers[kMaxBatch - 1][kMaxLayers];
  void *more_out[kMaxBatch - 1];
};
constexpr size_t kFusedHeadBytes = 192;
static_assert(offsetof(FusedLdsArgs, rd_blob) == 0 && offsetof(FusedLdsArgs, rd_bytes) == 8 && offsetof(FusedLdsArgs, rd_hole) == 12 &&
              offsetof(FusedLdsArgs, total_quads) == 16 && offsetof(FusedLdsArgs, wg_per_job) == 20 && offsetof(FusedLdsArgs, per_wg) == 24 &&
              offsetof(FusedLdsArgs, magic_wg) == 28 && offsetof(FusedLdsArgs, layers) == 32,
              "line 0 of the fused kernel's head: ph_kernels_lds.hip reads it by offset");
static_assert(offsetof(FusedLdsArgs, out) == 96 && offsetof(FusedLdsArgs, rd_cm) == 104 && offsetof(FusedLdsArgs, rd_gm) == 112 &&
              offsetof(FusedLdsArgs, wr_cm) == 120, "the head's pointers end with the first 128 bytes");
static_assert(offsetof(FusedLdsArgs, rd_k) == 128 && offsetof(FusedLdsArgs, wr_k) == 148 && offsetof(FusedLdsArgs, wr_bytes) == 168 &&
              offsetof(FusedLdsArgs, wr_hole) == 172 && offsetof(FusedLdsArgs, wr_blob) == 176 && offsetof(FusedLdsArgs, jobs) == 184 &&
              offsetof(FusedLdsArgs, quads_per_line_used) == 188 && offsetof(FusedLdsArgs, quads_per_line_pitch) == kFusedHeadBytes,
              "line 2 of the fused kernel's head");
static_assert(offsetof(FusedLdsArgs, more_layers) >= kFusedHeadBytes, "the batch arrays lie behind the head");
FusedLdsArgs fused_lds_args(const FusedArgs &f, const LutView &rd, const LutView &wr);

constexpr int kMaxFusedOuts = 4;
struct FusedOut {
  uint32_t fmt;
  uint32_t takes;
  uint32_t line_end;
  uint32_t field;
  uint32_t half_pitch;
  uint32_t pad;
  const float *wr_cm;
  void *plane[3];
  LutView wr;
};
struct FusedMultiArgs {
  const void *layers[kMaxLayers];
  uint32_t quads_per_line, total_quads;
  uint32_t magic_qpl, need_line;
  const float *rd_cm, *rd_gm;
  LutView rd;
  uint32_t n_out;
  FusedOut out[kMaxFusedOuts];
};
hipError_t launch_fused_v210_combine_multi(hipStream_t s, int n, const FusedMultiArgs &a, uint32_t num_cus, uint32_t max_wgs);
hipError_t fused_multi_plan(const FusedMultiArgs &a, uint32_t num_cus, uint32_t max_wgs, FusedMultiArgs &b, uint32_t &grid, uint32_t &lds);
struct FusedMultiBatchArgs {
  FusedMultiArgs m;
  const void *layers[kMaxBatch][kMaxLayers];
  void *plane[kMaxBatch][kMaxFusedOuts][3];
};
hipError_t launch_fused_v210_combine_multi_batch(hipStream_t s, int n, uint32_t jobs, const FusedMultiBatchArgs &a, uint32_t num_cus, uint32_t max_wgs);
enum : uint32_t { kFusedCut = 0, kFusedDissolve = 1, kFusedWipeV210 = 2, kFusedWipeF32 = 3 };
struct FusedTransArgs {
  FusedMultiArgs m;
  const void *incoming[kMaxLayers];
  const void *mask[kMaxLayers];
  uint32_t kind[kMaxLayers];
  float mix[kMaxLayers];
};
hipError_t launch_fused_v210_trans_multi(hipStream_t s, int n, const FusedTransArgs &a, uint32_t num_cus, uint32_t max_wgs);
struct FusedRouteArgs {
  FusedMultiArgs m;
  uint32_t is_image[kMaxLayers];
  void *image_out;
  uint32_t nt;
};
hipError_t launch_fused_v210_route_multi(hipStream_t s, int n, const FusedRouteArgs &a, uint32_t num_cus, uint32_t max_wgs);

struct ComposeArgs {
  const void *layers[kMaxLayers];
  const float *matrix[kMaxLayers];
  const void *wipe_with[kMaxLayers], *wipe_mask[kMaxLayers];
  int lw[kMaxLayers], lh[kMaxLayers];
  int n;
  void *out;
  uint32_t out_w, out_h, lines, first_line, line_step;
  const float *wr_cm;
  LutView wr;
};

enum : uint32_t { kChanNone = 0, kChanV210 = 1, kChanRgba = 2, kChanP10 = 3, kChanP8x422 = 4, kChanP8x420 = 5, kChanNv12 = 6, kChanP10x420 = 7,
                  kChanP010 = 8, kChanRgba8 = 9, kChanBgra8 = 10, kChanPlanarLast = kChanP010 };
enum : uint32_t { kChanCut = 0, kChanDissolve = 1, kChanWipe = 2 };
struct ChanSrc {
  const void *ptr;
  uint32_t w, h, pitch;
  uint32_t kind;
  uint32_t sampled;
  uint32_t tail_from;
  float m[6];
};
enum : uint32_t { kChanActLayer = 0, kChanActHold = 1, kChanActDissolve = 2, kChanActIncoming = 3, kChanActWipe = 4, kChanActFirst = 0x100,
                  kChanActShare = 0x200, kChanActShareShift = 12 };
constexpr int kMaxChanOps = 3 * kMaxLayers;
struct ChanOp {
  ChanSrc src;
  uint32_t action;
  float mix;
};
struct ChanArgs {
  ChanOp op[kMaxChanOps];
  int n_ops;
  uint32_t magic_cpr, magic_cpg;
  void *out;
  void *index;
  uint32_t out_w, out_h, lines, first_line, line_step;
  const float *rd_cm, *rd_gm, *wr_cm;
  LutView rd, wr;
  const void *plane_u[kMaxChanOps], *plane_v[kMaxChanOps];
  const float *cm_op[kMaxChanOps];
  uint32_t planar;
  uint32_t out_fmt, out_pitch;
  void *out_u, *out_v;
  uint32_t out_qpitch, out_tail_from;
  uint32_t halo_off, halo_steps;
  uint32_t any_cm;
  uint32_t images_only;
};

constexpr int kMaxChanOuts = 4;
struct ChanOut {
  uint32_t fmt;
  uint32_t pitch;
  void *plane[3];
  uint32_t tail_from;
  uint32_t takes;
  uint32_t line_end;
  uint32_t field;
  uint32_t round;
  const float *wr_cm;
  LutView wr;
};
struct ChanMultiArgs {
  ChanArgs c;
  uint32_t n_out;
  ChanOut out[kMaxChanOuts];
};
static_assert(sizeof(ChanMultiArgs) < 4096, "kernel arguments are limited to 4 KiB");

constexpr int kMaxChanJobs = 8;
constexpr int kMaxChanBatchOps = 40;
struct ChanJob {
  void *out, *index;
  uint32_t first_op, n_ops, first_line, pad;
};
struct ChanBatchArgs {
  ChanOp op[kMaxChanBatchOps];
  ChanJob job[kMaxChanJobs];
  uint8_t op_job[kMaxChanBatchOps];
  uint32_t share_op[8];
  uint32_t jobs, n_ops, n_share;
  uint32_t magic_cpr, magic_cpg;
  uint32_t steps;
  uint32_t magic_spj, magic_qpj;
  uint32_t out_w, out_h, lines, line_step;
  const float *rd_cm, *rd_gm, *wr_cm;
  LutView rd, wr;
  uint32_t tails;
  uint32_t out_qpitch, out_tail_from;
  uint32_t job_rot[kMaxChanJobs][4];
  uint32_t sched_off;
  uint32_t halo_off, halo_steps;
  uint32_t images_only;
  const void *plane_u[kMaxChanBatchOps], *plane_v[kMaxChanBatchOps];
  const float *cm_tab[8];
  uint8_t cm_idx[kMaxChanBatchOps];
  uint32_t planar;
  uint32_t any_cm;
};
static_assert(sizeof(ChanBatchArgs) <= 4096, "kernel arguments are limited to 4 KiB");
bool trace_launch(const char *name);
hipError_t launch_chan_compose_batch(hipStream_t s, const ChanBatchArgs &a, uint32_t num_cus);

constexpr int kMaxChanOutJobs = 4;
// ... 201 lines not shown
```

### phaneron_amd/csrc/ph_kernels_lds.hip

```cpp
#include "ph_device.h"
#include "ph_kernels.h"
#include "ph_ldslut.h"

#include <atomic>
#include <cstdlib>

#include <type_traits>
#include <utility>

#pragma clang fp contract(off)

#ifndef PH_PROBE
#define PH_PROBE 0
#endif
#if PH_PROBE
constexpr int kProbeWords = 16;
__device__ unsigned long long g_fused_probe[2048 * kProbeWords];
extern "C" int ph_debug_fused_probe(unsigned long long *out, int n_words) {
  return (int)hipMemcpyFromSymbol(out, HIP_SYMBOL(g_fused_probe), (size_t)n_words * 8);
}
#define PH_STAMP_ENTRY() \
  const unsigned long long ph_entry_cycles = __builtin_amdgcn_s_memtime(), ph_entry_ticks = __builtin_amdgcn_s_memrealtime()
#define PH_STAMP(k) PH_STAMP_IF(k, tile_begin == wg_begin)
#define PH_STAMP_IF(k, first_tile)                                                   \
  do {                                                                               \
    if (threadIdx.x == 0 && (first_tile)) {                                          \
      g_fused_probe[blockIdx.x * kProbeWords + 2 * (k)] = __builtin_amdgcn_s_memtime();       \
      g_fused_probe[blockIdx.x * kProbeWords + 2 * (k) + 1] = __builtin_amdgcn_s_memrealtime(); \
      if ((k) == 0) {                                                                \
        g_fused_probe[blockIdx.x * kProbeWords + 10] = ph_entry_cycles;              \
        g_fused_probe[blockIdx.x * kProbeWords + 11] = ph_entry_ticks;               \
      }                                                                              \
    }                                                                                \
  } while (0)
#else
#define PH_STAMP_ENTRY() do { } while (0)
#define PH_STAMP(k) do { } while (0)
#define PH_STAMP_IF(k, first_tile) do { } while (0)
#endif

#ifndef PH_BALANCE_WAVES
#define PH_BALANCE_WAVES 1
#endif
#if PH_BALANCE_WAVES
__device__ __forceinline__ void ph_set_wave_priority(int level) {
  switch (level) {
    case 3: __builtin_amdgcn_s_setprio(3); break;
    case 2: __builtin_amdgcn_s_setprio(2); break;
    case 1: __builtin_amdgcn_s_setprio(1); break;
    default: __builtin_amdgcn_s_setprio(0); break;
  }
}
#define PH_BALANCE(p) ph_set_wave_priority(3 - ((p) * 4) / P)
#else
#define PH_BALANCE(p) do { } while (0)
#endif

namespace ph {


__device__ __forceinline__ uint4 write_quad_lds(const float (&rgb)[18], const WriteK &wk, const LutK &lut) {
  uint32_t y[6], u[3], v[3];
#pragma unroll
  for (int j = 0; j < 6; ++j) {
    if ((j & 1) == 0) {
      const Yuv1 c = write_px_lds(rgb[3 * j], rgb[3 * j + 1], rgb[3 * j + 2], wk, lut);
      y[j] = c.y, u[j >> 1] = c.u, v[j >> 1] = c.v;
    } else {
      y[j] = write_px_luma_lds(rgb[3 * j], rgb[3 * j + 1], rgb[3 * j + 2], wk, lut);
    }
  }
  return pack_quad(y, u, v);
}

#ifndef PH_FUSED_SPLIT
#define PH_FUSED_SPLIT 0
#endif
typedef uint32_t fused_head_line __attribute__((ext_vector_type(16)));
struct FusedHead {
  fused_head_line l0, l1, l2;
  __device__ __forceinline__ uint32_t word(int byte) const { return byte < 64 ? l0[byte / 4] : byte < 128 ? l1[byte / 4 - 16] : l2[byte / 4 - 32]; }
  __device__ __forceinline__ void set_word(int byte, uint32_t v) {
    if (byte < 64) l0[byte / 4] = v;
    else if (byte < 128) l1[byte / 4 - 16] = v;
    else l2[byte / 4 - 32] = v;
  }
  template <typename P>
  __device__ __forceinline__ P ptr(int byte) const { return (P)((uintptr_t)word(byte) | ((uintptr_t)word(byte + 4) << 32)); }
  __device__ __forceinline__ LutK lut_k(int byte) const {
    return LutK{__uint_as_float(word(byte)), __uint_as_float(word(byte + 4)), __uint_as_float(word(byte + 8)), __uint_as_float(word(byte + 12)), word(byte + 16)};
  }
};
typedef const __attribute__((address_space(1))) ph_u4v *global_quad_ptr;
typedef const __attribute__((address_space(1))) uint32_t *global_u32_ptr;
typedef const __attribute__((address_space(4))) float *const_f32_ptr;
__device__ __forceinline__ uint4 load_stream(global_quad_ptr p) {
  const ph_u4v v = __builtin_nontemporal_load(p);
  return make_uint4(v.x, v.y, v.z, v.w);
}
__device__ __forceinline__ ReadK load_read_k(const_f32_ptr cm, const_f32_ptr gm) {
  ReadK k;
  k.r = make_float4(cm[0], cm[1], cm[2], cm[3]);
  k.g = make_float4(cm[4], cm[5], cm[6], cm[7]);
  k.b = make_float4(cm[8], cm[9], cm[10], cm[11]);
#pragma unroll
  for (int i = 0; i < 9; ++i) k.gm[i] = gm[i];
  return k;
}
__device__ __forceinline__ WriteK load_write_k(const_f32_ptr cm) {
  WriteK k;
  k.y = make_float4(cm[0], cm[1], cm[2], cm[3]);
  k.u = make_float4(cm[4], cm[5], cm[6], cm[7]);
  k.v = make_float4(cm[8], cm[9], cm[10], cm[11]);
  return k;
}
static_assert(kFusedHeadBytes == 3 * sizeof(fused_head_line), "fused_head_load asks for three lines");
__device__ __forceinline__ FusedHead fused_head_load() {
  FusedHead h;
  const auto *args = __builtin_amdgcn_kernarg_segment_ptr();
  asm volatile("s_load_dwordx16 %0, %3, 0x0\n\ts_load_dwordx16 %1, %3, 0x40\n\ts_load_dwordx16 %2, %3, 0x80\n\ts_waitcnt lgkmcnt(0)"
               : "=&s"(h.l0), "=&s"(h.l1), "=&s"(h.l2)
               : "s"(args));
  return h;
}

constexpr int kLayerFirst = 1, kLayerLast = 2;
template <int... I, typename F>
__device__ __forceinline__ void static_for_each(std::integer_sequence<int, I...>, F &&f) {
  (f(std::integral_constant<int, I>{}), ...);
}
template <int COUNT, typename F>
__device__ __forceinline__ void static_for(F &&f) {
  static_for_each(std::make_integer_sequence<int, COUNT>{}, f);
}
template <int PLACE, bool STD>
__device__ __forceinline__ void fused_layer_combine(float (&acc)[18], const uint4 w, const ReadK &rk, const LutK &rlut, float last) {
  __builtin_amdgcn_sched_barrier(0);
  const Yuv6 q = unpack_quad(w);
#pragma unroll
  for (int j = 0; j < 6; ++j) {
    const float4 t = read_px_lds<STD>(q.y[j], q.cb[j >> 1], q.cr[j >> 1], rk, rlut, last);
    if (PLACE & kLayerFirst) {
      acc[3 * j] = t.x, acc[3 * j + 1] = t.y, acc[3 * j + 2] = t.z;
      if (PLACE & kLayerLast) {
#pragma unroll
        for (int c = 0; c < 3; ++c) acc[3 * j + c] = __builtin_fminf(__builtin_fmaxf(acc[3 * j + c], 0.0f), 1.0f);
      }
      asm volatile("" : "+v"(acc[3 * j]), "+v"(acc[3 * j + 1]), "+v"(acc[3 * j + 2]));
    } else {
      const float kk = 1.0f - t.w;
      if (PLACE & kLayerLast)
        asm volatile("v_fma_f32 %0, %0, %3, %4 clamp\n\tv_fma_f32 %1, %1, %3, %5 clamp\n\tv_fma_f32 %2, %2, %3, %6 clamp"
                     : "+v"(acc[3 * j]), "+v"(acc[3 * j + 1]), "+v"(acc[3 * j + 2])
                     : "v"(kk), "v"(t.x), "v"(t.y), "v"(t.z));
      else
        asm volatile("v_fma_f32 %0, %0, %3, %4\n\tv_fma_f32 %1, %1, %3, %5\n\tv_fma_f32 %2, %2, %3, %6"
                     : "+v"(acc[3 * j]), "+v"(acc[3 * j + 1]), "+v"(acc[3 * j + 2])
                     : "v"(kk), "v"(t.x), "v"(t.y), "v"(t.z));
    }
  }
}
__device__ __forceinline__ float lds_lut_index_clamped(float t) { return t * 65535.0f + kRoundMagic; }
__device__ __forceinline__ float lds_lut_index_clamped_tail(float t, bool trunc) {
  const float x = t * 65535.0f;
  return (trunc ? __builtin_floorf(x) : x) + kRoundMagic;
}

template <int N, int P, int BS, bool PIPE = false, int MODE = 0, bool TAIL = false>
__global__ __launch_bounds__(BS) void fused_v210_combine_lds_kernel(FusedLdsArgs a, uint32_t *handoff = nullptr) {
  static_assert(!TAIL || (!PIPE && MODE == 0), "the tail instantiation exists for the shipped form only");
  PH_STAMP_ENTRY();
  FusedHead head = fused_head_load();
  const uint32_t total_quads = head.word(offsetof(FusedLdsArgs, total_quads)), wg_per_job = head.word(offsetof(FusedLdsArgs, wg_per_job));
  const uint32_t per_wg = head.word(offsetof(FusedLdsArgs, per_wg));
  uint32_t job = fused_job_of(blockIdx.x, head.word(offsetof(FusedLdsArgs, magic_wg)));
  asm("" : "+s"(job));
  const uint32_t wg_in_job = blockIdx.x - job * wg_per_job;
  auto layer_ptr = [&](int l) { return reinterpret_cast<const uint4 *>(job ? a.more_layers[job - 1][l] : a.layers[l]); };
  const uint32_t wg_begin = wg_in_job * per_wg;
  const uint32_t wg_end = wg_begin + per_wg < total_quads ? wg_begin + per_wg : total_quads;
  if (wg_begin >= wg_end) return;
  const uint32_t tile_quads = BS * P;
  auto quad_at = [&](uint32_t tile_begin, int p) {
    const uint32_t f = tile_begin + p * BS + threadIdx.x;
    return f < wg_end ? f : wg_end - 1;
  };
  constexpr bool kSplitLayers = !PIPE && MODE == 0;
  if (kSplitLayers && job) {
    auto own_layer = [&](int l) {
      const uintptr_t p = (uintptr_t)a.more_layers[job - 1][l];
      head.set_word(offsetof(FusedLdsArgs, layers) + 8 * l, (uint32_t)p);
      head.set_word(offsetof(FusedLdsArgs, layers) + 8 * l + 4, (uint32_t)(p >> 32));
    };
    own_layer(0);
    if (N > 1) own_layer(1);
    if (N > 2) own_layer(2);
    if (N > 3) own_layer(3);
    if (N > 4) own_layer(4);
    if (N > 5) own_layer(5);
    if (N > 6) own_layer(6);
    if (N > 7) own_layer(7);
  }
  static_assert(N <= 8, "the layers' pointers are named one by one");
  typedef const __attribute__((address_space(1))) char *global_byte_ptr;
  auto layer_base = [&](int l) { return (global_byte_ptr)head.ptr<global_quad_ptr>(offsetof(FusedLdsArgs, layers) + 8 * l); };
  auto layer_word = [&](int l, uint32_t at) { return load_stream((global_quad_ptr)(layer_base(l) + at)); };
  auto layer_word_any = [&](int l, uint32_t at) {
    global_byte_ptr base = layer_base(N - 1);
    if (N > 3 && l == 2) base = layer_base(2);
    if (N > 4 && l == 3) base = layer_base(3);
    if (N > 5 && l == 4) base = layer_base(4);
    if (N > 6 && l == 5) base = layer_base(5);
    if (N > 7 && l == 6) base = layer_base(6);
    return load_stream((global_quad_ptr)(base + at));
  };
  uint4 w;
  if (kSplitLayers) w = layer_word(0, quad_at(wg_begin, 0) << 4);
  else if (job) w = load_stream(layer_ptr(0) + quad_at(wg_begin, 0));
  else w = load_stream(head.ptr<global_quad_ptr>(offsetof(FusedLdsArgs, layers)) + quad_at(wg_begin, 0));
  const uint32_t *const rd_blob = (const uint32_t *)head.ptr<global_u32_ptr>(offsetof(FusedLdsArgs, rd_blob));
  const uint32_t rd_bytes = head.word(offsetof(FusedLdsArgs, rd_bytes)), rd_hole = head.word(offsetof(FusedLdsArgs, rd_hole));
  PH_STAMP_IF(0, true);
  if (MODE != 2) lds_lut_load<BS, false>(rd_blob, rd_bytes, rd_hole);
  __builtin_amdgcn_sched_barrier(0);
  const ReadK rk = load_read_k(head.ptr<const_f32_ptr>(offsetof(FusedLdsArgs, rd_cm)), head.ptr<const_f32_ptr>(offsetof(FusedLdsArgs, rd_gm)));
  const WriteK wk = load_write_k(head.ptr<const_f32_ptr>(offsetof(FusedLdsArgs, wr_cm)));
  LutK rlut = head.lut_k(offsetof(FusedLdsArgs, rd_k)), wlut = head.lut_k(offsetof(FusedLdsArgs, wr_k));
  asm("" : "+v"(rlut.a_base), "+v"(rlut.delta_base), "+v"(wlut.a_base), "+v"(wlut.delta_base));
  const uint32_t *const wr_blob = (const uint32_t *)head.ptr<global_u32_ptr>(offsetof(FusedLdsArgs, wr_blob));
  const uint32_t wr_bytes = head.word(offsetof(FusedLdsArgs, wr_bytes)), wr_hole = head.word(offsetof(FusedLdsArgs, wr_hole));
  uint4 *const out_ptr = reinterpret_cast<uint4 *>(job ? a.more_out[job - 1] : a.out);
  const bool std_matrix = ycbcr_matrix_is_standard(rk);
  for (uint32_t tile_begin = wg_begin; tile_begin < wg_end; tile_begin += tile_quads) {
    uint32_t st[P][9];
    auto quad_of = [&](int p) { return quad_at(tile_begin, p); };
    if (tile_begin != wg_begin) {
      w = kSplitLayers ? layer_word(0, quad_of(0) << 4) : load_stream(layer_ptr(0) + quad_of(0));
      if (MODE == 0) lds_lut_load<BS, false>(rd_blob, rd_bytes, rd_hole);
    }
    auto slot_kind = [&](uint32_t f) -> uint32_t {
      const uint32_t g = f - __umulhi(f, a.magic_qpp) * a.quads_per_line_pitch;
      return g < a.quads_per_line_used ? 0u : (g == a.quads_per_line_used && a.tail_px) ? 1u : 2u;
    };
    auto phase1_slice = [&](auto tag, uint4 w, uint32_t f, uint32_t f_next, bool more, uint32_t(&st)[9]) -> uint4 {
      const bool in_tail = TAIL && slot_kind(f) == 1u;
      const float last = TAIL ? (in_tail ? 0.0f : 1.0f) : 1.0f;
      float acc[18];
#pragma unroll
      for (int i = 0; i < 18; ++i) acc[i] = 0.0f;
#pragma unroll 1
      for (int l = 0; l < N; ++l) {
        uint4 nxt = w;
        if (l + 1 < N) nxt = load_stream(layer_ptr(l + 1) + f);
        else if (more) nxt = load_stream(layer_ptr(0) + f_next);
        const Yuv6 q = unpack_quad(w);
#pragma unroll
        for (int j = 0; j < 6; ++j) {
          const float4 t = read_px_lds<decltype(tag)::value>(q.y[j], q.cb[j >> 1], q.cr[j >> 1], rk, rlut, last);
          const float kk = 1.0f - t.w;
          asm volatile("v_fma_f32 %0, %0, %3, %4\n\tv_fma_f32 %1, %1, %3, %5\n\tv_fma_f32 %2, %2, %3, %6"
                       : "+v"(acc[3 * j]), "+v"(acc[3 * j + 1]), "+v"(acc[3 * j + 2])
                       : "v"(kk), "v"(t.x), "v"(t.y), "v"(t.z));
        }
        w = nxt;
      }
#pragma unroll
      for (int i = 0; i < 9; ++i) {
        const uint32_t lo = __float_as_uint(TAIL ? lds_lut_index_unit_tail(acc[2 * i], in_tail) : lds_lut_index_unit(acc[2 * i]));
        const uint32_t hi = __float_as_uint(TAIL ? lds_lut_index_unit_tail(acc[2 * i + 1], in_tail) : lds_lut_index_unit(acc[2 * i + 1]));
        st[i] = __builtin_amdgcn_perm(hi, lo, 0x05040100u);
        asm volatile("" : "+v"(st[i]));
      }
      return w;
    };
    auto phase1_slice_split = [&](auto tag, uint4 w, uint32_t f, uint32_t f_next, bool more, uint32_t(&st)[9]) __attribute__((always_inline)) -> uint4 {
      constexpr int MID = N > 2 ? N - 2 : 0;
      const bool in_tail = TAIL && slot_kind(f) == 1u;
      const float last = TAIL ? (in_tail ? 0.0f : 1.0f) : 1.0f;
      float acc[18];
      constexpr bool STD = decltype(tag)::value;
      auto combine = [&](auto place, const uint4 word) __attribute__((always_inline)) {
        fused_layer_combine<decltype(place)::value, STD>(acc, word, rk, rlut, last);
      };
      constexpr std::integral_constant<int, N == 1 ? (kLayerFirst | kLayerLast) : kLayerFirst> first_layer{};
      constexpr std::integral_constant<int, 0> middle_layer{};
      constexpr std::integral_constant<int, kLayerLast> last_layer{};
      uint32_t at = f << 4;
      if (STD) asm volatile("; standard matrix" : "+v"(at));
      else asm volatile("; any matrix" : "+v"(at));
      uint4 nxt = w;
      if (N > 1) nxt = layer_word(1, at);
      else if (more) nxt = layer_word(0, f_next << 4);
      combine(first_layer, w);
      w = nxt;
      if constexpr (MID > 0 && MID <= 2) {
        nxt = layer_word(2, at);
        combine(middle_layer, w);
        w = nxt;
        if constexpr (MID == 2) {
          nxt = layer_word(3, at);
          combine(middle_layer, w);
          w = nxt;
        }
      } else if constexpr (MID > 2) {
#pragma unroll 1
        for (int l = 1; l + 1 <= MID; l += 2) {
          const uint4 w2 = layer_word_any(l + 1, at);
          combine(middle_layer, w);
          w = layer_word_any(l + 2, at);
          combine(middle_layer, w2);
        }
        if (MID & 1) {
          nxt = layer_word(N - 1, at);
          combine(middle_layer, w);
          w = nxt;
        }
      }
      if constexpr (N > 1) {
        nxt = w;
        if (more) nxt = layer_word(0, f_next << 4);
        combine(last_layer, w);
        w = nxt;
      }
#pragma unroll
      for (int i = 0; i < 9; ++i) {
        const uint32_t lo = __float_as_uint(TAIL ? lds_lut_index_clamped_tail(acc[2 * i], in_tail) : lds_lut_index_clamped(acc[2 * i]));
        const uint32_t hi = __float_as_uint(TAIL ? lds_lut_index_clamped_tail(acc[2 * i + 1], in_tail) : lds_lut_index_clamped(acc[2 * i + 1]));
        st[i] = __builtin_amdgcn_perm(hi, lo, 0x05040100u);
        asm volatile("" : "+v"(st[i]));
      }
      return w;
    };
    if (MODE == 0 || (MODE == 1 && tile_begin == wg_begin)) {
      asm volatile("s_waitcnt vmcnt(0)" ::: "memory");
      __syncthreads();
    }
    PH_STAMP(1);
    const uint32_t tile_left = wg_end - tile_begin;
    if constexpr (PIPE) {
      auto phase1_all = [&](auto tag) {
        constexpr bool STD = decltype(tag)::value;
        auto issue_first = [&](const uint4 &word) {
          return read_px_issue<STD>((float)((word.x >> 10) & 0x3ff), (float)(word.x & 0x3ff), (float)((word.x >> 20) & 0x3ff), rk, rlut);
        };
        auto issue_px = [&](const uint4 &word, int j) {
          const uint32_t wy = j == 0 ? word.x : j < 3 ? word.y : j == 3 ? word.z : word.w;
          const uint32_t sy = (j == 0 || j == 3) ? 10u : (j == 1 || j == 4) ? 0u : 20u;
          const int pr = j >> 1;
          const uint32_t wcb = pr == 0 ? word.x : pr == 1 ? word.y : word.z, scb = 10u * pr;
          const uint32_t wcr = pr == 0 ? word.x : pr == 1 ? word.z : word.w, scr = pr == 0 ? 20u : pr == 1 ? 0u : 10u;
          return read_px_issue<STD>((float)((wy >> sy) & 0x3ff), (float)((wcb >> scb) & 0x3ff), (float)((wcr >> scr) & 0x3ff), rk, rlut);
        };
        PxPending pend = issue_first(w);
#pragma unroll
        for (int p = 0; p < P; ++p) {
          if (p * BS < tile_left) {
            PH_BALANCE(p);
            const uint32_t f = quad_of(p);
            const bool more = (p + 1 < P) && ((p + 1) * BS < tile_left);
            const uint32_t f_next = more ? quad_of(p + 1) : f;
            float acc[18];
#pragma unroll
            for (int i = 0; i < 18; ++i) acc[i] = 0.0f;
#pragma unroll 1
            for (int l = 0; l < N; ++l) {
              uint4 nxt = w;
              if (l + 1 < N) nxt = load_stream(layer_ptr(l + 1) + f);
              else if (more) nxt = load_stream(layer_ptr(0) + f_next);
#pragma unroll
              for (int j = 0; j < 6; ++j) {
                PxPending nx;
                if (j < 5) nx = issue_px(w, j + 1);
                else {
                  uint4 first = nxt;
                  asm volatile("" : "+v"(first.x));
                  nx = issue_first(first);
                }
                __builtin_amdgcn_sched_barrier(0);
                const float4 t = read_px_finish(pend, rk);
                const float kk = 1.0f - t.w;
                asm volatile("v_fma_f32 %0, %0, %3, %4\n\tv_fma_f32 %1, %1, %3, %5\n\tv_fma_f32 %2, %2, %3, %6"
                             : "+v"(acc[3 * j]), "+v"(acc[3 * j + 1]), "+v"(acc[3 * j + 2])
                             : "v"(kk), "v"(t.x), "v"(t.y), "v"(t.z));
                __builtin_amdgcn_sched_barrier(0);
                pend = nx;
              }
              w = nxt;
            }
#pragma unroll
            for (int i = 0; i < 9; ++i) {
              const uint32_t lo = __float_as_uint(lds_lut_index_unit(acc[2 * i]));
              const uint32_t hi = __float_as_uint(lds_lut_index_unit(acc[2 * i + 1]));
              st[p][i] = __builtin_amdgcn_perm(hi, lo, 0x05040100u);
              asm volatile("" : "+v"(st[p][i]));
            }
          }
        }
      };
      if (std_matrix) phase1_all(std::true_type{});
      else phase1_all(std::false_type{});
      PH_STAMP(2);
      __syncthreads();
      lds_lut_load<BS>(wr_blob, wr_bytes, wr_hole);
      __syncthreads();
      PH_STAMP(3);
      auto idx_at = [&](int p, int i) {
        const uint32_t v = st[p][i >> 1];
        return __uint_as_float(((i & 1) ? (v >> 16) : (v & 0xFFFFu)) | 0x4B400000u);
      };
      PxPending wp = write_px_issue(idx_at(0, 0), idx_at(0, 1), idx_at(0, 2), wlut);
#pragma unroll
      for (int p = 0; p < P; ++p) {
        if (p * BS < tile_left) {
          PH_BALANCE(p);
          const uint32_t f = tile_begin + p * BS + threadIdx.x;
          uint32_t y[6], u[3], v[3];
#pragma unroll
          for (int j = 0; j < 6; ++j) {
            PxPending nx = wp;
            if (j < 5) nx = write_px_issue(idx_at(p, 3 * j + 3), idx_at(p, 3 * j + 4), idx_at(p, 3 * j + 5), wlut);
            else if (p + 1 < P) {
              if ((p + 1) * BS < tile_left) nx = write_px_issue(idx_at(p + 1 < P ? p + 1 : p, 0), idx_at(p + 1 < P ? p + 1 : p, 1), idx_at(p + 1 < P ? p + 1 : p, 2), wlut);
            }
            __builtin_amdgcn_sched_barrier(0);
            const float gr = lds_lut_finish(wp.r), gg = lds_lut_finish(wp.g), gb = lds_lut_finish(wp.b);
            y[j] = sat_u16_rte(dot4(gr, gg, gb, 1.0f, wk.y));
            if ((j & 1) == 0) {
              u[j >> 1] = sat_u16_rte(dot4(gr, gg, gb, 1.0f, wk.u));
              v[j >> 1] = sat_u16_rte(dot4(gr, gg, gb, 1.0f, wk.v));
            }
            __builtin_amdgcn_sched_barrier(0);
            wp = nx;
          }
          if (f < wg_end) store_stream(out_ptr + f, pack_quad(y, u, v));
        }
      }
    } else {
    const uint32_t wave_first = (uint32_t)__builtin_amdgcn_readfirstlane((int)(threadIdx.x & ~63u));
    if constexpr (kSplitLayers) {
      static_for<P>([&](auto slice) __attribute__((always_inline)) {
        constexpr int p = decltype(slice)::value;
        const uint32_t f = quad_of(p);
        if (p * BS + wave_first < wg_end - tile_begin) {
          PH_BALANCE(p);
          const bool more = (p + 1 < P) && ((p + 1) * BS + wave_first < wg_end - tile_begin);
          const uint32_t f_next = more ? quad_of(p + 1) : f;
          if (std_matrix) w = phase1_slice_split(std::true_type{}, w, f, f_next, more, st[p]);
          else w = phase1_slice_split(std::false_type{}, w, f, f_next, more, st[p]);
        }
      });
    } else if (MODE != 2) {
#pragma unroll
    for (int p = 0; p < P; ++p) {
      const uint32_t f = quad_of(p);
      if (p * BS + wave_first < wg_end - tile_begin) {
        PH_BALANCE(p);
        const bool more = (p + 1 < P) && ((p + 1) * BS + wave_first < wg_end - tile_begin);
        const uint32_t f_next = more ? quad_of(p + 1) : f;
        if (std_matrix) w = phase1_slice(std::true_type{}, w, f, f_next, more, st[p]);
        else w = phase1_slice(std::false_type{}, w, f, f_next, more, st[p]);
      }
    }
    }
    if (MODE == 1) {
#pragma unroll
      for (int p = 0; p < P; ++p)
        if (p * BS + wave_first < wg_end - tile_begin) {
          const uint32_t f = quad_of(p);
#pragma unroll
          for (int i = 0; i < 9; ++i) handoff[(size_t)i * a.total_quads + f] = st[p][i];
        }
      continue;
    }
    if (MODE == 2) {
#pragma unroll
      for (int p = 0; p < P; ++p)
        if (p * BS + wave_first < wg_end - tile_begin) {
          const uint32_t f = quad_of(p);
#pragma unroll
          for (int i = 0; i < 9; ++i) st[p][i] = __builtin_nontemporal_load(handoff + (size_t)i * a.total_quads + f);
        }
    }
    PH_STAMP(2);
    if (MODE == 0 || tile_begin == wg_begin) {
      __syncthreads();
      lds_lut_load<BS>(wr_blob, wr_bytes, wr_hole);
      __syncthreads();
    }
    PH_STAMP(3);
#pragma unroll
    for (int p = 0; p < P; ++p) {
      const uint32_t f = tile_begin + p * BS + threadIdx.x;
      if (p * BS + wave_first < wg_end - tile_begin) {
        PH_BALANCE(p);
        float yi[18];
#pragma unroll
        for (int i = 0; i < 9; ++i) {
          yi[2 * i] = __uint_as_float((st[p][i] & 0xFFFFu) | 0x4B400000u);
          yi[2 * i + 1] = __uint_as_float((st[p][i] >> 16) | 0x4B400000u);
        }
        uint4 packed;
        if (TAIL) {
          const uint32_t kind = slot_kind(f < wg_end ? f : wg_end - 1);
          if (kind == 0u) packed = write_quad_idx_lds(yi, wk, wlut);
          else if (kind == 1u) packed = write_quad_idx_lds_tail(yi, wk, wlut, a.tail_px);
          else packed = make_uint4(0u, 0u, 0u, 0u);
        } else {
          packed = write_quad_idx_lds(yi, wk, wlut);
        }
        if (f < wg_end) store_stream(out_ptr + f, packed);
      }
    }
    }
    PH_STAMP(4);
    if (PIPE || MODE != 0 || tile_begin + tile_quads < wg_end) __syncthreads();
    PH_STAMP(6);
  }
}

__global__ __launch_bounds__(kLdsBlock) void v210_read_lds_kernel(const uint4 *__restrict__ in, float4 *__restrict__ out,
                                                                   uint32_t width, uint32_t quads_per_line_pitch,
                                                                   uint32_t total_px, const float *__restrict__ cm,
                                                                   const float *__restrict__ gm, LutView lut, uint32_t nt) {
  const ReadK k = load_read_k(cm, gm);
  const LutK lk = make_lut_k(lut);
  lds_lut_load(lut);
  __syncthreads();
  const uint32_t tail_from = width - width % 6u;
  for (uint32_t p = blockIdx.x * kLdsBlock + threadIdx.x; p < total_px; p += gridDim.x * kLdsBlock) {
    const uint32_t line = p / width, x = p - line * width;
    const uint32_t g = x / 6, j = x - 6 * g, pr = j >> 1;
    const uint4 w = in[(size_t)line * quads_per_line_pitch + g];
    const uint32_t wy = (j == 0) ? w.x : (j < 3) ? w.y : (j == 3) ? w.z : w.w;
    const uint32_t sy = (j == 0 || j == 3) ? 10u : (j == 1 || j == 4) ? 0u : 20u;
    const uint32_t wcb = pr == 0 ? w.x : pr == 1 ? w.y : w.z;
    const uint32_t wcr = pr == 0 ? w.x : pr == 1 ? w.z : w.w;
    const uint32_t scr = pr == 0 ? 20u : pr == 1 ? 0u : 10u;
    const float yf = (float)((wy >> sy) & 0x3ff);
    const float cbf = (float)((wcb >> (10u * pr)) & 0x3ff);
    const float crf = (float)((wcr >> scr) & 0x3ff);
    store_image(out + p, read_px_lds(yf, cbf, crf, k, lk, x < tail_from ? 1.0f : 0.0f), nt);
  }
}

struct ReadBatchArgs {
  const uint4 *in[kMaxLayers];
  float4 *out[kMaxLayers];
  uint32_t wg_per_frame;
};
__global__ __launch_bounds__(kLdsBlock) void v210_read_lds_batch_kernel(ReadBatchArgs a, uint32_t width, uint32_t quads_per_line_pitch,
                                                                         uint32_t total_px, const float *__restrict__ cm,
                                                                         const float *__restrict__ gm, LutView lut, uint32_t nt) {
  const ReadK k = load_read_k(cm, gm);
  const LutK lk = make_lut_k(lut);
  lds_lut_load(lut);
  __syncthreads();
  const uint32_t frame = blockIdx.x / a.wg_per_frame, wg = blockIdx.x - frame * a.wg_per_frame;
  const uint4 *__restrict__ in = a.in[frame];
  float4 *__restrict__ out = a.out[frame];
  const uint32_t tail_from = width - width % 6u;
  for (uint32_t p = wg * kLdsBlock + threadIdx.x; p < total_px; p += a.wg_per_frame * kLdsBlock) {
    const uint32_t line = p / width, x = p - line * width;
    const uint32_t g = x / 6, j = x - 6 * g, pr = j >> 1;
    const uint4 w = in[(size_t)line * quads_per_line_pitch + g];
    const uint32_t wy = (j == 0) ? w.x : (j < 3) ? w.y : (j == 3) ? w.z : w.w;
    const uint32_t sy = (j == 0 || j == 3) ? 10u : (j == 1 || j == 4) ? 0u : 20u;
    const uint32_t wcb = pr == 0 ? w.x : pr == 1 ? w.y : w.z;
    const uint32_t wcr = pr == 0 ? w.x : pr == 1 ? w.z : w.w;
    const uint32_t scr = pr == 0 ? 20u : pr == 1 ? 0u : 10u;
    const float yf = (float)((wy >> sy) & 0x3ff);
    const float cbf = (float)((wcb >> (10u * pr)) & 0x3ff);
    const float crf = (float)((wcr >> scr) & 0x3ff);
    store_image(out + p, read_px_lds(yf, cbf, crf, k, lk, x < tail_from ? 1.0f : 0.0f), nt);
  }
}

__global__ __launch_bounds__(kLdsBlock) void v210_write_lds_kernel(const float4 *__restrict__ in, uint4 *__restrict__ out,
                                                                    uint32_t width, uint32_t quads_per_line,
                                                                    uint32_t lines, uint32_t first_line,
                                                                    uint32_t line_step, const float *__restrict__ cm,
                                                                    LutView lut) {
  const WriteK k = load_write_k(cm);
  const LutK lk = make_lut_k(lut);
  lds_lut_load(lut);
  __syncthreads();
  const uint32_t total = quads_per_line * lines, full = width / 6u, remain = width - 6u * full;
  for (uint32_t f = blockIdx.x * kLdsBlock + threadIdx.x; f < total; f += gridDim.x * kLdsBlock) {
    const uint32_t li = f / quads_per_line, g = f - li * quads_per_line;
    const uint32_t line = first_line + li * line_step;
    if (g > full || (g == full && !remain)) {
      store_stream(out + (size_t)line * quads_per_line + g, make_uint4(0u, 0u, 0u, 0u));
      continue;
    }
    const float4 *row = in + (size_t)line * width;
    float rgb[18];
#pragma unroll
    for (int j = 0; j < 6; ++j) {
      const uint32_t x = 6u * g + (uint32_t)j < width ? 6u * g + (uint32_t)j : width - 1u;
      const float4 p = row[x];
      rgb[3 * j] = p.x, rgb[3 * j + 1] = p.y, rgb[3 * j + 2] = p.z;
    }
    if (g == full) {
      float yi[18];
#pragma unroll
      for (int i = 0; i < 18; ++i) yi[i] = lds_lut_index_unit_tail(rgb[i], true);
      store_stream(out + (size_t)line * quads_per_line + g, write_quad_idx_lds_tail(yi, k, lk, remain));
      continue;
    }
    store_stream(out + (size_t)line * quads_per_line + g, write_quad_lds(rgb, k, lk));
  }
}

__global__ __launch_bounds__(kLdsBlock) void compose_write_v210_kernel(ComposeArgs a) {
  const WriteK wk = load_write_k(a.wr_cm);
  const LutK lk = make_lut_k(a.wr);
  lds_lut_load(a.wr);
  __syncthreads();
  const uint32_t qpl = (a.out_w + 47u) / 48u * 8u, full = a.out_w / 6u, remain = a.out_w - 6u * full;
  const uint32_t total = qpl * a.lines;
  for (uint32_t f = blockIdx.x * kLdsBlock + threadIdx.x; f < total; f += gridDim.x * kLdsBlock) {
    const uint32_t li = f / qpl, g = f - li * qpl;
    const uint32_t line = a.first_line + li * a.line_step;
    if (g > full || (g == full && !remain)) {
      store_stream(reinterpret_cast<uint4 *>(a.out) + (size_t)line * qpl + g, make_uint4(0u, 0u, 0u, 0u));
      continue;
    }
    float acc[24];
#pragma unroll 1
    for (int l = 0; l < a.n; ++l) {
      const float4 *img = reinterpret_cast<const float4 *>(a.layers[l]);
      const int lw = a.lw[l], lh = a.lh[l];
      const float *m = a.matrix[l];
      float m0 = 0, m1 = 0, m2 = 0, m3 = 0, m4 = 0, m5 = 0;
      if (m) m0 = m[0], m1 = m[1], m2 = m[2], m3 = m[3], m4 = m[4], m5 = m[5];
      const float py = (float)(int)line / (float)(int)a.out_h - 0.5f;
#pragma unroll
      for (int j = 0; j < 6; ++j) {
        const int x = 6 * g + j < a.out_w ? (int)(6 * g + j) : (int)a.out_w - 1;
        float4 t;
        if (m) {
          const float px = (float)x / (float)(int)a.out_w - 0.5f;
          const float s = dot3(m0, m1, m2, px, py, 1.0f) + 0.5f;
          const float tt = dot3(m3, m4, m5, px, py, 1.0f) + 0.5f;
          t = sample_linear(img, lw, lh, s, tt);
        } else {
          t = img[(size_t)line * a.out_w + x];
        }
        if (l == 0) {
          acc[4 * j] = t.x, acc[4 * j + 1] = t.y, acc[4 * j + 2] = t.z, acc[4 * j + 3] = t.w;
        } else {
          const float kk = 1.0f - t.w;
          acc[4 * j] = fma_rn(acc[4 * j], kk, t.x);
          acc[4 * j + 1] = fma_rn(acc[4 * j + 1], kk, t.y);
          acc[4 * j + 2] = fma_rn(acc[4 * j + 2], kk, t.z);
          acc[4 * j + 3] = fma_rn(acc[4 * j + 3], 0.0f, t.w);
        }
      }
    }
    float rgb[18];
#pragma unroll
    for (int j = 0; j < 6; ++j) rgb[3 * j] = acc[4 * j], rgb[3 * j + 1] = acc[4 * j + 1], rgb[3 * j + 2] = acc[4 * j + 2];
// ... 204 lines not shown
        t.y = ((w00 * t00.y + w10 * t10.y) + w01 * t01.y) + w11 * t11.y;
        t.z = ((w00 * t00.z + w10 * t10.z) + w01 * t01.z) + w11 * t11.z;
        t.w = ((w00 * t00.w + w10 * t10.w) + w01 * t01.w) + w11 * t11.w;
        if (MIXED) t.x = direct[l] ? t00.x : t.x, t.y = direct[l] ? t00.y : t.y, t.z = direct[l] ? t00.z : t.z, t.w = direct[l] ? t00.w : t.w;
        if (WIPE && a.wipe_with[l]) {
          const float m = wipe_m[l], rm = 1.0f - m;
          t.x = fma_rn(wipe_b[l].x, m, t.x * rm), t.y = fma_rn(wipe_b[l].y, m, t.y * rm);
          t.z = fma_rn(wipe_b[l].z, m, t.z * rm), t.w = fma_rn(wipe_b[l].w, m, t.w * rm);
        }
        if (l == 0) {
          r = t.x, g = t.y, b = t.z;
        } else {
          const float kk = 1.0f - t.w;
          r = fma_rn(r, kk, t.x), g = fma_rn(g, kk, t.y), b = fma_rn(b, kk, t.z);
        }
      }
      const Yuv1 c = write_px_lds(r, g, b, wk, lk);
      ys[local] = (uint16_t)c.y;
      if (!(x & 1)) us[local >> 1] = (uint16_t)c.u, vs[local >> 1] = (uint16_t)c.v;
    }
    __builtin_amdgcn_fence(__ATOMIC_RELEASE, "wavefront");
    __builtin_amdgcn_wave_barrier();
    __builtin_amdgcn_fence(__ATOMIC_ACQUIRE, "wavefront");
    if (lane < kComposeChunk / 6) {
      uint32_t y[6], u[3], v[3];
#pragma unroll
      for (int j = 0; j < 6; ++j) y[j] = ys[lane * 6 + j];
#pragma unroll
      for (int j = 0; j < 3; ++j) u[j] = us[lane * 3 + j], v[j] = vs[lane * 3 + j];
      store_stream(reinterpret_cast<uint4 *>(a.out) + (size_t)line * qpl + (x_first + lane * 6) / 6, pack_quad(y, u, v));
    }
    __builtin_amdgcn_wave_barrier();
  }
}

template <int N, bool MIXED, bool SHARED = false, bool WIPE = false>
__global__ __launch_bounds__(kLdsBlock) void compose_write_v210_taps_kernel(ComposeArgs a, uint32_t stage_off) {
  const WriteK wk = load_write_k(a.wr_cm);
  const LutK lk = make_lut_k(a.wr);
  float mm[N][6];
  bool direct[N];
  __amdgpu_buffer_rsrc_t img[N];
  bool all_aligned = true;
#pragma unroll
  for (int l = 0; l < N; ++l) {
    direct[l] = a.matrix[l] == nullptr;
#pragma unroll
    for (int i = 0; i < 6; ++i) mm[l][i] = direct[l] ? 0.0f : a.matrix[l][i];
    all_aligned = all_aligned && mm[l][1] == 0.0f && mm[l][3] == 0.0f;
    img[l] = __builtin_amdgcn_make_buffer_rsrc(const_cast<void *>(a.layers[l]), 0, a.lw[l] * a.lh[l] * 16, 0x00020000);
  }
  lds_lut_load(a.wr);
  __syncthreads();
  const uint32_t wave = __builtin_amdgcn_readfirstlane(threadIdx.x >> 6), lane = threadIdx.x & 63;
  uint16_t *ys = reinterpret_cast<uint16_t *>(g_lds + stage_off + wave * kComposeChunk * 4);
  uint16_t *us = ys + kComposeChunk, *vs = us + kComposeChunk / 2;
  if (all_aligned)
    compose_taps_body<N, MIXED, true, SHARED, WIPE>(a, mm, direct, img, wk, lk, ys, us, vs, wave, lane);
  else
    compose_taps_body<N, MIXED, false, SHARED, WIPE>(a, mm, direct, img, wk, lk, ys, us, vs, wave, lane);
}

template <int N>
static hipError_t launch_compose_taps_n(hipStream_t s, const ComposeArgs &a, uint32_t grid, uint32_t stage_off) {
  bool mixed = false, shared = N > 1, wipe = false;
  for (int l = 0; l < N; ++l) {
    wipe = wipe || a.wipe_with[l] != nullptr;
    mixed = mixed || a.matrix[l] == nullptr;
    shared = shared && a.matrix[l] != nullptr && a.matrix[l] == a.matrix[0] && a.lw[l] == a.lw[0] && a.lh[l] == a.lh[0];
  }
  if (wipe) {
    hipError_t e = hipFuncSetAttribute(reinterpret_cast<const void *>(compose_write_v210_taps_kernel<N, true, false, true>),
                                       hipFuncAttributeMaxDynamicSharedMemorySize, kMaxDynamicLds);
    if (e != hipSuccess) return e;
    compose_write_v210_taps_kernel<N, true, false, true><<<grid, kLdsBlock, stage_off + kComposeStageBytes, s>>>(a, stage_off);
    return hipGetLastError();
  }
  const void *fn = shared ? reinterpret_cast<const void *>(compose_write_v210_taps_kernel<N, false, true>)
                   : mixed ? reinterpret_cast<const void *>(compose_write_v210_taps_kernel<N, true>)
                           : reinterpret_cast<const void *>(compose_write_v210_taps_kernel<N, false>);
  hipError_t e = hipFuncSetAttribute(fn, hipFuncAttributeMaxDynamicSharedMemorySize, kMaxDynamicLds);
  if (e != hipSuccess) return e;
  if (shared)
    compose_write_v210_taps_kernel<N, false, true><<<grid, kLdsBlock, stage_off + kComposeStageBytes, s>>>(a, stage_off);
  else if (mixed)
    compose_write_v210_taps_kernel<N, true><<<grid, kLdsBlock, stage_off + kComposeStageBytes, s>>>(a, stage_off);
  else
    compose_write_v210_taps_kernel<N, false><<<grid, kLdsBlock, stage_off + kComposeStageBytes, s>>>(a, stage_off);
  return hipGetLastError();
}

static bool compose_taps_eligible(const ComposeArgs &a) {
  if (a.out_w % kComposeChunk) return false;
  bool sampled = false;
  for (int l = 0; l < a.n; ++l) {
    const uint64_t bytes = (uint64_t)a.lw[l] * (uint64_t)a.lh[l] * 16u, pitch = (uint64_t)a.lw[l] * 16u;
    if (bytes + 2 * pitch > 0x80000000ull || pitch >= (1u << 23) || a.lh[l] >= (1 << 22)) return false;
    sampled = sampled || a.matrix[l] != nullptr;
  }
  for (int l = 0; l < a.n; ++l) sampled = sampled || a.wipe_with[l] != nullptr;
  return sampled;
}
static bool compose_stage_fits(const ComposeArgs &a) { return ((a.wr.bytes + 15u) & ~15u) + kComposeStageBytes <= 160u * 1024u; }
static bool compose_quad_forced() {
  static const int quad_env = [] {
    const char *e = getenv("PH_COMPOSE_QUAD");
    return e ? atoi(e) : 0;
  }();
  return quad_env != 0;
}
static bool compose_taps_enabled() {
  static const int taps_env = [] {
    const char *e = getenv("PH_COMPOSE_TAPS");
    return e ? atoi(e) : 1;
  }();
  return taps_env != 0;
}
static bool compose_uses_taps(const ComposeArgs &a) {
  return !compose_quad_forced() && compose_stage_fits(a) && compose_taps_enabled() && compose_taps_eligible(a);
}
bool compose_can_wipe(const ComposeArgs &a) { return compose_uses_taps(a); }

template <int N, bool ALL_DIRECT>
static hipError_t launch_compose_px_nd(hipStream_t s, const ComposeArgs &a, uint32_t grid, uint32_t stage_off) {
  hipError_t e = hipFuncSetAttribute(reinterpret_cast<const void *>(compose_write_v210_px_kernel<N, ALL_DIRECT>),
                                     hipFuncAttributeMaxDynamicSharedMemorySize, kMaxDynamicLds);
  if (e != hipSuccess) return e;
  compose_write_v210_px_kernel<N, ALL_DIRECT><<<grid, kLdsBlock, stage_off + kComposeStageBytes, s>>>(a, stage_off);
  return hipGetLastError();
}
template <int N>
static hipError_t launch_compose_px_n(hipStream_t s, const ComposeArgs &a, uint32_t grid, uint32_t stage_off) {
  bool all_direct = true;
  for (int l = 0; l < N; ++l) all_direct = all_direct && a.matrix[l] == nullptr;
  return all_direct ? launch_compose_px_nd<N, true>(s, a, grid, stage_off) : launch_compose_px_nd<N, false>(s, a, grid, stage_off);
}

template <typename K>
static hipError_t allow_lds(K kernel, uint32_t bytes) {
  return hipFuncSetAttribute(reinterpret_cast<const void *>(kernel), hipFuncAttributeMaxDynamicSharedMemorySize, kMaxDynamicLds);
}
template <typename K>
static hipError_t allow_lds_once(K kernel, std::atomic<uint64_t> &done) {
  int dev = 0;
  hipError_t e = hipGetDevice(&dev);
  if (e != hipSuccess) return e;
  const uint64_t bit = 1ull << (dev & 63);
  if (dev < 64 && (done.load(std::memory_order_acquire) & bit)) return hipSuccess;
  e = allow_lds(kernel, kMaxDynamicLds);
  if (e == hipSuccess && dev < 64) done.fetch_or(bit, std::memory_order_release);
  return e;
}

FusedLutK fused_lut_k(const LutView &v) {
#if defined(__x86_64__)
  const unsigned csr = __builtin_ia32_stmxcsr();
  __builtin_ia32_ldmxcsr(csr & ~0x8040u);
#endif
  const volatile float lds0 = 0.0f, magic = 12582912.0f;
  const float small = (v.delta_base + lds0) + v.bias * v.delta_scale;
  const float b = small - magic * v.delta_scale;
  const FusedLutK k{v.a_scale, -((magic - v.bias) * v.a_scale), v.delta_scale, b, v.shift - 2u};
#if defined(__x86_64__)
  __builtin_ia32_ldmxcsr(csr);
#endif
  return k;
}

FusedLdsArgs fused_lds_args(const FusedArgs &f, const LutView &rd, const LutView &wr) {
  FusedLdsArgs a{};
  a.rd_blob = rd.blob, a.rd_bytes = rd.bytes, a.rd_hole = rd.hole;
  a.wr_blob = wr.blob, a.wr_bytes = wr.bytes, a.wr_hole = wr.hole;
  a.rd_k = fused_lut_k(rd), a.wr_k = fused_lut_k(wr);
  for (int l = 0; l < kMaxLayers; ++l) a.layers[l] = f.layers[l];
  a.out = f.out, a.rd_cm = f.rd_cm, a.rd_gm = f.rd_gm, a.wr_cm = f.wr_cm;
  a.total_quads = f.total_quads, a.quads_per_line_used = f.quads_per_line_used, a.quads_per_line_pitch = f.quads_per_line_pitch;
  a.tail_px = f.tail_px, a.magic_qpp = f.magic_qpp, a.jobs = 1;
  return a;
}

#if PH_FUSED_SPLIT
template <int N, int P, int BS, int MODE>
static hipError_t launch_fused_half(hipStream_t s, FusedLdsArgs b, uint32_t lds) {
  static uint32_t *handoff = nullptr;
  static size_t handoff_quads = 0;
  if (handoff_quads < b.total_quads) {
    if (handoff) hipFree(handoff);
    if (hipMalloc(&handoff, (size_t)b.total_quads * 36) != hipSuccess) return hipErrorOutOfMemory;
    handoff_quads = b.total_quads;
  }
  static std::atomic<uint64_t> lds_allowed{0};
  hipError_t e = allow_lds_once(fused_v210_combine_lds_kernel<N, P, BS, false, MODE>, lds_allowed);
  if (e != hipSuccess) return e;
  fused_v210_combine_lds_kernel<N, P, BS, false, MODE><<<b.wg_per_job * b.jobs, BS, lds, s>>>(b, handoff);
  return hipGetLastError();
}
#endif

template <int N, int P, int BS, bool PIPE = false, bool TAIL = false>
static hipError_t launch_fused_npb(hipStream_t s, const FusedLdsArgs &a, uint32_t grid_in, uint32_t lds) {
  uint32_t grid = grid_in;
#if PH_FUSED_SPLIT
  static const int cus_env = [] {
    const char *e = getenv("PH_FUSED_CUS");
    return e ? atoi(e) : 0;
  }();
  if (cus_env > 0 && (uint32_t)cus_env < grid) grid = (uint32_t)cus_env;
#endif
  static std::atomic<uint64_t> lds_allowed{0};
  hipError_t e = allow_lds_once(fused_v210_combine_lds_kernel<N, P, BS, PIPE, 0, TAIL>, lds_allowed);
  if (e != hipSuccess) return e;
  const uint32_t slices = (a.total_quads + BS - 1) / BS;
  FusedLdsArgs b = a;
  if (b.jobs < 1) b.jobs = 1;
  b.wg_per_job = grid / b.jobs ? grid / b.jobs : 1;
  if (b.wg_per_job > slices) b.wg_per_job = slices;
  b.per_wg = (b.total_quads + b.wg_per_job - 1) / b.wg_per_job;
  b.magic_wg = fused_wg_magic(b.wg_per_job);
#if PH_FUSED_SPLIT
  if (!PIPE && N == 4) {
    static const int mode_env = [] {
      const char *e = getenv("PH_FUSED_MODE");
      return e ? atoi(e) : 0;
    }();
    if (mode_env == 1) return launch_fused_half<N, P, BS, 1>(s, b, lds);
    if (mode_env == 2) return launch_fused_half<N, P, BS, 2>(s, b, lds);
    if (mode_env == 3) {
      hipError_t e1 = launch_fused_half<N, P, BS, 1>(s, b, lds);
      return e1 != hipSuccess ? e1 : launch_fused_half<N, P, BS, 2>(s, b, lds);
    }
  }
#endif
  fused_v210_combine_lds_kernel<N, P, BS, PIPE, 0, TAIL><<<b.wg_per_job * b.jobs, BS, lds, s>>>(b);
  return hipGetLastError();
}

template <int N>
static hipError_t launch_fused_n(hipStream_t s, const FusedLdsArgs &a, uint32_t grid, uint32_t lds) {
  static const int geom_env = [] {
    const char *e = getenv("PH_FUSED_GEOM");
    return e ? atoi(e) : 0;
  }();
  if (a.quads_per_line_used != a.quads_per_line_pitch) return launch_fused_npb<N, 6, 1024, false, true>(s, a, grid, lds);
  int geom = geom_env ? geom_env : 6;
  static const int pipe_env = [] {
    const char *e = getenv("PH_FUSED_PIPE");
    return e ? atoi(e) : 0;
  }();
#ifdef PH_FUSED_EXPERIMENT
  static const int bs_env = [] {
    const char *e = getenv("PH_FUSED_BS");
    return e ? atoi(e) : 0;
  }();
  if (N == 4 && bs_env == 768) return pipe_env ? launch_fused_npb<4, 8, 768, true>(s, a, grid, lds) : launch_fused_npb<4, 8, 768>(s, a, grid, lds);
  if (N == 4 && bs_env == 512) return pipe_env ? launch_fused_npb<4, 11, 512, true>(s, a, grid, lds) : launch_fused_npb<4, 11, 512>(s, a, grid, lds);
#endif
  if (pipe_env && geom == 6) return launch_fused_npb<N, 6, 1024, true>(s, a, grid, lds);
  if (geom == 4) return launch_fused_npb<N, 4, 1024>(s, a, grid, lds);
  if (geom == 8) return launch_fused_npb<N, 8, 1024>(s, a, grid, lds);
  return launch_fused_npb<N, 6, 1024>(s, a, grid, lds);
}

hipError_t launch_fused_v210_combine_lds(hipStream_t s, int n, const FusedLdsArgs &a, uint32_t num_cus) {
  const uint32_t lds = a.rd_bytes > a.wr_bytes ? a.rd_bytes : a.wr_bytes;
  if (a.total_quads > (1u << 28)) return hipErrorInvalidValue;
  switch (n) {
    case 1: return launch_fused_n<1>(s, a, num_cus, lds);
    case 2: return launch_fused_n<2>(s, a, num_cus, lds);
    case 3: return launch_fused_n<3>(s, a, num_cus, lds);
    case 4: return launch_fused_n<4>(s, a, num_cus, lds);
    case 5: return launch_fused_n<5>(s, a, num_cus, lds);
    case 6: return launch_fused_n<6>(s, a, num_cus, lds);
    case 7: return launch_fused_n<7>(s, a, num_cus, lds);
    case 8: return launch_fused_n<8>(s, a, num_cus, lds);
    default: return hipErrorInvalidValue;
  }
}

hipError_t launch_compose_write_v210(hipStream_t s, const ComposeArgs &a, uint32_t num_cus) {
  const uint32_t total = (a.out_w + 47u) / 48u * 8u * a.lines;
  if (!total) return hipSuccess;
  bool any_wipe = false;
  for (int l = 0; l < a.n; ++l) any_wipe = any_wipe || a.wipe_with[l] != nullptr;
  if (any_wipe && !compose_uses_taps(a)) return hipErrorInvalidValue;
  const uint32_t stage_off = (a.wr.bytes + 15u) & ~15u;
  if (!compose_quad_forced() && compose_stage_fits(a) && a.out_w % 48u == 0) {
    const uint32_t chunks = (a.out_w * a.lines + kComposeChunk - 1) / kComposeChunk;
    const uint32_t want = (chunks + kLdsBlock / 64 - 1) / (kLdsBlock / 64);
    const uint32_t grid = want < num_cus ? want : num_cus;
    if (compose_uses_taps(a)) {
      switch (a.n) {
        case 1: return launch_compose_taps_n<1>(s, a, grid, stage_off);
        case 2: return launch_compose_taps_n<2>(s, a, grid, stage_off);
        case 3: return launch_compose_taps_n<3>(s, a, grid, stage_off);
        case 4: return launch_compose_taps_n<4>(s, a, grid, stage_off);
        case 5: return launch_compose_taps_n<5>(s, a, grid, stage_off);
        case 6: return launch_compose_taps_n<6>(s, a, grid, stage_off);
        case 7: return launch_compose_taps_n<7>(s, a, grid, stage_off);
        case 8: return launch_compose_taps_n<8>(s, a, grid, stage_off);
        default: return hipErrorInvalidValue;
      }
    }
    switch (a.n) {
      case 1: return launch_compose_px_n<1>(s, a, grid, stage_off);
      case 2: return launch_compose_px_n<2>(s, a, grid, stage_off);
      case 3: return launch_compose_px_n<3>(s, a, grid, stage_off);
      case 4: return launch_compose_px_n<4>(s, a, grid, stage_off);
      case 5: return launch_compose_px_n<5>(s, a, grid, stage_off);
      case 6: return launch_compose_px_n<6>(s, a, grid, stage_off);
      case 7: return launch_compose_px_n<7>(s, a, grid, stage_off);
      case 8: return launch_compose_px_n<8>(s, a, grid, stage_off);
      default: return hipErrorInvalidValue;
    }
  }
  hipError_t e = allow_lds(compose_write_v210_kernel, a.wr.bytes);
  if (e != hipSuccess) return e;
  const uint32_t want = (total + kLdsBlock - 1) / kLdsBlock;
  compose_write_v210_kernel<<<want < num_cus ? want : num_cus, kLdsBlock, a.wr.bytes, s>>>(a);
  return hipGetLastError();
}

__global__ void lds_base_probe_kernel(uint32_t *out) {
  *out = (uint32_t)(uintptr_t)(__attribute__((address_space(3))) unsigned char *)g_lds;
}
hipError_t launch_lds_base_probe(hipStream_t s, uint32_t *out_dev) {
  lds_base_probe_kernel<<<1, 64, 16, s>>>(out_dev);
  return hipGetLastError();
}

hipError_t launch_v210_read_lds(hipStream_t s, const void *in, void *out, uint32_t width, uint32_t height,
                                const void *cm, const void *gm, const LutView &lut, uint32_t num_cus) {
  hipError_t e = allow_lds(v210_read_lds_kernel, lut.bytes);
  if (e != hipSuccess) return e;
  const uint32_t total = width * height;
  const uint32_t want = (total + kLdsBlock - 1) / kLdsBlock;
  v210_read_lds_kernel<<<want < num_cus ? want : num_cus, kLdsBlock, lut.bytes, s>>>(
      (const uint4 *)in, (float4 *)out, width, v210_pitch_bytes(width) / 16, total, (const float *)cm, (const float *)gm,
      lut, image_nt((size_t)width * height * 16));
  return hipGetLastError();
}

hipError_t launch_v210_read_lds_batch(hipStream_t s, int n, const void *const *ins, void *const *outs, uint32_t width,
                                      uint32_t height, const void *cm, const void *gm, const LutView &lut, uint32_t num_cus) {
  hipError_t e = allow_lds(v210_read_lds_batch_kernel, lut.bytes);
  if (e != hipSuccess) return e;
  ReadBatchArgs a{};
  for (int i = 0; i < n; ++i) a.in[i] = (const uint4 *)ins[i], a.out[i] = (float4 *)outs[i];
  const uint32_t total = width * height;
  const uint32_t want = (total + kLdsBlock - 1) / kLdsBlock;
  uint32_t per = num_cus / (uint32_t)n ? num_cus / (uint32_t)n : 1;
  a.wg_per_frame = want < per ? want : per;
  v210_read_lds_batch_kernel<<<a.wg_per_frame * n, kLdsBlock, lut.bytes, s>>>(a, width, v210_pitch_bytes(width) / 16, total,
                                                                              (const float *)cm, (const float *)gm, lut,
                                                                              image_nt((size_t)width * height * 16));
  return hipGetLastError();
}

hipError_t launch_v210_write_lds(hipStream_t s, const void *in, void *out, uint32_t width, uint32_t height,
                                 uint32_t interlace, const void *cm, const LutView &lut, uint32_t num_cus) {
  hipError_t e = allow_lds(v210_write_lds_kernel, lut.bytes);
  if (e != hipSuccess) return e;
  const uint32_t step = interlace ? 2 : 1, first = (interlace == 3) ? 1 : 0;
  const uint32_t lines = interlace ? height / 2 : height, qpl = v210_pitch_bytes(width) / 16;
  if (!lines) return hipSuccess;
  const uint32_t want = (qpl * lines + kLdsBlock - 1) / kLdsBlock;
  v210_write_lds_kernel<<<want < num_cus ? want : num_cus, kLdsBlock, lut.bytes, s>>>(
      (const float4 *)in, (uint4 *)out, width, qpl, lines, first, step, (const float *)cm, lut);
  return hipGetLastError();
}

}
```

### phaneron_amd/csrc/ph_ldslut.h

```cpp
#pragma once
#include "ph_device.h"
#include "ph_lut.h"

#pragma clang fp contract(off)

namespace ph {

constexpr int kLdsBlock = 1024;

#ifndef PH_ABLATE
#define PH_ABLATE 0
#endif

extern __shared__ __attribute__((aligned(16))) unsigned char g_lds[];

template <int BS = kLdsBlock, bool WAIT = true>
__device__ __forceinline__ void lds_lut_load(const uint32_t *blob, uint32_t bytes, uint32_t hole) {
#if PH_ABLATE & 2
  return;
#endif
  const uint32_t n = (bytes - hole) / 16;
  unsigned char *const dst = g_lds + hole;
  const uint32_t wave = threadIdx.x >> 6, lane = threadIdx.x & 63;
  const uint4 *src = reinterpret_cast<const uint4 *>(blob);
  for (uint32_t base = wave * 64; base < n; base += BS) {
    const uint32_t i = base + lane;
    if (i < n)
      __builtin_amdgcn_global_load_lds((const __attribute__((address_space(1))) void *)(src + i),
                                       (__attribute__((address_space(3))) void *)(dst + 16 * base), 16, 0, 0);
  }
  if (WAIT) asm volatile("s_waitcnt vmcnt(0)" ::: "memory");
}
template <int BS = kLdsBlock, bool WAIT = true>
__device__ __forceinline__ void lds_lut_load(const LutView &v) {
  lds_lut_load<BS, WAIT>(v.blob, v.bytes, v.hole);
}

struct LutK {
  float a_scale, a_base;
  float delta_scale, delta_base;
  uint32_t a_shift;
};
typedef const __attribute__((address_space(3))) uint32_t *lds_u32_ptr;
typedef const __attribute__((address_space(3))) uint16_t *lds_u16_ptr;
__device__ __forceinline__ LutK make_lut_k(const LutView &v) {
  const uint32_t lds0 = (uint32_t)(uintptr_t)(__attribute__((address_space(3))) unsigned char *)g_lds;
  const float small = (v.delta_base + __uint_as_float(lds0)) + v.bias * v.delta_scale;
  const float b = small - kRoundMagic * v.delta_scale;
  return LutK{v.a_scale, -((kRoundMagic - v.bias) * v.a_scale), v.delta_scale, b, v.shift - 2u};
}
__device__ __forceinline__ uint32_t lds_lut_anchor_addr(const LutK &k, float y) {
  return (__float_as_uint(fma_rn(y, k.a_scale, k.a_base)) >> k.a_shift) & ~3u;
}
__device__ __forceinline__ float lds_lut_fetch(const LutK &k, float y) {
  const uint32_t a_addr = lds_lut_anchor_addr(k, y);
  const uint32_t d_addr = __float_as_uint(fma_rn(y, k.delta_scale, k.delta_base));
#if PH_ABLATE & 8
  const uint32_t a = *(lds_u32_ptr)(a_addr & 4u);
  const uint32_t d = *(lds_u16_ptr)(d_addr & 2u);
#elif PH_ABLATE & 1
  const uint32_t a = a_addr, d = d_addr;
#elif PH_ABLATE & 4
  const uint32_t a = *(lds_u32_ptr)a_addr, d = d_addr;
#else
  const uint32_t a = *(lds_u32_ptr)a_addr;
  const uint32_t d = *(lds_u16_ptr)d_addr;
#endif
#if PH_ABLATE & 16
  {
    uint32_t t;
    asm volatile("v_and_or_b32 %0, %1, %2, %3\n\tv_fma_f32 %0, %0, %0, %0\n\tv_sub_f32 %0, %0, %1\n\tv_fma_f32 %0, %0, %1, %0\n\tv_add_u32 %0, %0, %2"
                 : "=&v"(t)
                 : "v"(a), "v"(d), "v"(a_addr));
  }
#endif
  return __uint_as_float(a + d);
}
struct LutPending {
  uint32_t a, d;
};
__device__ __forceinline__ LutPending lds_lut_issue(const LutK &k, float y) {
  const uint32_t a_addr = lds_lut_anchor_addr(k, y);
  const uint32_t d_addr = __float_as_uint(fma_rn(y, k.delta_scale, k.delta_base));
#if PH_ABLATE & 8
  return LutPending{*(lds_u32_ptr)(a_addr & 4u), *(lds_u16_ptr)(d_addr & 2u)};
#elif PH_ABLATE & 1
  return LutPending{a_addr, d_addr};
#else
  return LutPending{*(lds_u32_ptr)a_addr, *(lds_u16_ptr)d_addr};
#endif
}
__device__ __forceinline__ float lds_lut_finish(const LutPending &p) {
#if PH_ABLATE & 16
  {
    uint32_t t;
    asm volatile("v_and_or_b32 %0, %1, %2, %1\n\tv_fma_f32 %0, %0, %0, %0\n\tv_sub_f32 %0, %0, %1\n\tv_fma_f32 %0, %0, %1, %0\n\tv_add_u32 %0, %0, %2"
                 : "=&v"(t)
                 : "v"(p.a), "v"(p.d));
  }
#endif
  return __uint_as_float(p.a + p.d);
}

__device__ __forceinline__ float lds_lut_index_unit(float t) {
  t = __builtin_fminf(__builtin_fmaxf(t, 0.0f), 1.0f);
  return t * 65535.0f + kRoundMagic;
}
__device__ __forceinline__ float lds_lut_index_unit_tail(float t, bool trunc) {
  t = __builtin_fminf(__builtin_fmaxf(t, 0.0f), 1.0f);
  const float x = t * 65535.0f;
  return (trunc ? __builtin_floorf(x) : x) + kRoundMagic;
}
__device__ __forceinline__ float lds_lut_at(const LutK &k, float x) {
  x = __builtin_fminf(__builtin_fmaxf(x, 0.0f), 65535.0f);
  return lds_lut_fetch(k, x + kRoundMagic);
}
__device__ __forceinline__ float lds_lut_at_unit(const LutK &k, float t) {
  return lds_lut_fetch(k, lds_lut_index_unit(t));
}

__device__ __forceinline__ uint4 write_quad_idx_lds(const float (&yi)[18], const WriteK &wk, const LutK &lut) {
  uint32_t y[6], u[3], v[3];
#pragma unroll
  for (int j = 0; j < 6; ++j) {
    const float gr = lds_lut_fetch(lut, yi[3 * j]), gg = lds_lut_fetch(lut, yi[3 * j + 1]);
    const float gb = lds_lut_fetch(lut, yi[3 * j + 2]);
    y[j] = sat_u16_rte(dot4(gr, gg, gb, 1.0f, wk.y));
    if ((j & 1) == 0) {
      u[j >> 1] = sat_u16_rte(dot4(gr, gg, gb, 1.0f, wk.u));
      v[j >> 1] = sat_u16_rte(dot4(gr, gg, gb, 1.0f, wk.v));
    }
  }
  return pack_quad(y, u, v);
}

__device__ __forceinline__ uint4 write_quad_idx_lds_tail(const float (&yi)[18], const WriteK &wk, const LutK &lut, uint32_t remain) {
  uint32_t y[4], u[2], v[2];
#pragma unroll
  for (int j = 0; j < 4; ++j) {
    const float gr = lds_lut_fetch(lut, yi[3 * j]), gg = lds_lut_fetch(lut, yi[3 * j + 1]);
    const float gb = lds_lut_fetch(lut, yi[3 * j + 2]);
    y[j] = sat_u16_trunc(__builtin_roundf(dot4(gr, gg, gb, 1.0f, wk.y)));
    if ((j & 1) == 0) {
      u[j >> 1] = sat_u16_trunc(__builtin_roundf(dot4(gr, gg, gb, 1.0f, wk.u)));
      v[j >> 1] = sat_u16_trunc(__builtin_roundf(dot4(gr, gg, gb, 1.0f, wk.v)));
    }
  }
  uint4 w = make_uint4(v[0] << 20 | y[0] << 10 | u[0], 0u, 0u, 0u);
  if (remain == 2u) {
    w.y = y[1];
  } else if (remain == 4u) {
    w.y = y[2] << 20 | u[1] << 10 | y[1];
    w.z = y[3] << 10 | v[1];
  }
  return w;
}

struct LutInLds {
  LutK k;
  __device__ __forceinline__ float at(float x) const { return lds_lut_at(k, x); }
  __device__ __forceinline__ float at_unit(float t) const { return lds_lut_at_unit(k, t); }
};
struct LutInGlobal {
  const float *__restrict__ t;
  __device__ __forceinline__ float at(float x) const { return t[sat_u16_rte(x)]; }
  __device__ __forceinline__ float at_unit(float u) const { return t[sat_u16_rte(u * 65535.0f)]; }
};

__device__ __forceinline__ bool ycbcr_matrix_is_standard(const ReadK &k) {
  return k.r.y == 0.0f && k.b.z == 0.0f && k.r.x == k.g.x && k.g.x == k.b.x;
}
template <bool STD = false>
__device__ __forceinline__ float4 read_px_lds(float y, float cb, float cr, const ReadK &k, const LutK &lut, float last = 1.0f) {
  float tr, tg, tb;
  if (STD) {
    const float ym = y * k.r.x;
    tr = fma_rn(last, k.r.w, fma_rn(cr, k.r.z, ym));
    tg = fma_rn(last, k.g.w, fma_rn(cr, k.g.z, fma_rn(cb, k.g.y, ym)));
    tb = fma_rn(last, k.b.w, fma_rn(cb, k.b.y, ym));
  } else {
    tr = dot4(y, cb, cr, last, k.r), tg = dot4(y, cb, cr, last, k.g), tb = dot4(y, cb, cr, last, k.b);
  }
  const float r = lds_lut_at_unit(lut, tr);
  const float g = lds_lut_at_unit(lut, tg);
  const float b = lds_lut_at_unit(lut, tb);
  return make_float4(dot3(r, g, b, k.gm[0], k.gm[1], k.gm[2]), dot3(r, g, b, k.gm[3], k.gm[4], k.gm[5]),
                     dot3(r, g, b, k.gm[6], k.gm[7], k.gm[8]), 1.0f);
}

struct PxPending {
  LutPending r, g, b;
};
template <bool STD>
__device__ __forceinline__ PxPending read_px_issue(float y, float cb, float cr, const ReadK &k, const LutK &lut, float last = 1.0f) {
  float tr, tg, tb;
  if (STD) {
    const float ym = y * k.r.x;
    tr = fma_rn(last, k.r.w, fma_rn(cr, k.r.z, ym));
    tg = fma_rn(last, k.g.w, fma_rn(cr, k.g.z, fma_rn(cb, k.g.y, ym)));
    tb = fma_rn(last, k.b.w, fma_rn(cb, k.b.y, ym));
  } else {
    tr = dot4(y, cb, cr, last, k.r), tg = dot4(y, cb, cr, last, k.g), tb = dot4(y, cb, cr, last, k.b);
  }
  PxPending p;
  p.r = lds_lut_issue(lut, lds_lut_index_unit(tr));
  p.g = lds_lut_issue(lut, lds_lut_index_unit(tg));
  p.b = lds_lut_issue(lut, lds_lut_index_unit(tb));
  return p;
}
__device__ __forceinline__ float4 read_px_finish(const PxPending &p, const ReadK &k) {
  const float r = lds_lut_finish(p.r), g = lds_lut_finish(p.g), b = lds_lut_finish(p.b);
  return make_float4(dot3(r, g, b, k.gm[0], k.gm[1], k.gm[2]), dot3(r, g, b, k.gm[3], k.gm[4], k.gm[5]),
                     dot3(r, g, b, k.gm[6], k.gm[7], k.gm[8]), 1.0f);
}
__device__ __forceinline__ PxPending write_px_issue(float yr, float yg, float yb, const LutK &lut) {
  PxPending p;
  p.r = lds_lut_issue(lut, yr), p.g = lds_lut_issue(lut, yg), p.b = lds_lut_issue(lut, yb);
  return p;
}

__device__ __forceinline__ Yuv1 write_px_lds(float r, float g, float b, const WriteK &k, const LutK &lut) {
  const float gr = lds_lut_at_unit(lut, r);
  const float gg = lds_lut_at_unit(lut, g);
  const float gb = lds_lut_at_unit(lut, b);
  Yuv1 o;
  o.y = sat_u16_rte(dot4(gr, gg, gb, 1.0f, k.y));
  o.u = sat_u16_rte(dot4(gr, gg, gb, 1.0f, k.u));
  o.v = sat_u16_rte(dot4(gr, gg, gb, 1.0f, k.v));
  return o;
}
__device__ __forceinline__ uint32_t write_px_luma_lds(float r, float g, float b, const WriteK &k, const LutK &lut) {
  const float gr = lds_lut_at_unit(lut, r);
  const float gg = lds_lut_at_unit(lut, g);
  const float gb = lds_lut_at_unit(lut, b);
  return sat_u16_rte(dot4(gr, gg, gb, 1.0f, k.y));
}

}
```

### phaneron_amd/csrc/ph_lut.cpp

```cpp
#include "ph_lut_host.h"

#include <algorithm>
#include <cmath>
#include <cstring>

namespace ph {

namespace {
inline uint32_t f2u(float f) {
  uint32_t u;
  std::memcpy(&u, &f, 4);
  return u;
}
inline float u2f(uint32_t u) {
  float f;
  std::memcpy(&f, &u, 4);
  return f;
}
}

LutView lut_view(const LutHostInfo &info, const void *blob_dev) {
  LutView v;
  v.blob = static_cast<const uint32_t *>(blob_dev);
  v.bytes = info.bytes;
  v.hole = info.hole;
  v.bias = info.bias;
  v.shift = info.shift;
  v.a_scale = std::ldexp(1.0f, 1 - (int)(f2u(info.bias) >> 23));
  v.delta_scale = u2f(2u);
  v.delta_base = u2f(info.delta_off - 2u * (uint32_t)info.bias);
  return v;
}

bool lut_compress(const float *lut, uint32_t max_bytes, std::vector<uint32_t> &blob, LutHostInfo &info) {
  std::vector<uint32_t> p(65536), blk(65536);
  std::memcpy(p.data(), lut, 65536 * sizeof(uint32_t));
  bool found = false;
  for (float bias : {16.0f, 32.0f, 64.0f, 128.0f}) {
    for (uint32_t m = 7; m <= 10; ++m) {
      const uint32_t shift = 23 - m;
      const uint32_t first = f2u(bias) >> shift;
      const uint32_t n_blocks = (f2u(65535.0f + bias) >> shift) - first + 1;
      const uint32_t n_anchors = (n_blocks + 3) & ~3u;
      const uint32_t hole = 4u << m;
      const uint32_t bytes = hole + n_anchors * 4 + 65536 * 2;
      if (bytes > max_bytes || (found && bytes >= info.bytes)) continue;
      std::vector<uint32_t> lo(n_blocks, 0xffffffffu), hi(n_blocks, 0);
      for (uint32_t i = 0; i < 65536; ++i) {
        blk[i] = (f2u((float)i + bias) >> shift) - first;
        lo[blk[i]] = std::min(lo[blk[i]], p[i]);
        hi[blk[i]] = std::max(hi[blk[i]], p[i]);
      }
      bool ok = true;
      for (uint32_t b = 0; b < n_blocks && ok; ++b)
        if (lo[b] != 0xffffffffu && hi[b] - lo[b] >= 65536u) ok = false;
      if (!ok) continue;
      found = true;
      info.bytes = bytes, info.shift = shift, info.first = first, info.n_anchors = n_anchors;
      info.hole = hole, info.delta_off = hole + n_anchors * 4, info.bias = bias;
      blob.assign((bytes - hole) / 4, 0);
      for (uint32_t b = 0; b < n_blocks; ++b) blob[b] = lo[b] == 0xffffffffu ? 0 : lo[b];
      uint16_t *delta = reinterpret_cast<uint16_t *>(blob.data() + n_anchors);
      for (uint32_t i = 0; i < 65536; ++i) delta[i] = (uint16_t)(p[i] - lo[blk[i]]);
    }
  }
  if (!found) return false;
  const LutView v = lut_view(info, nullptr);
  const float magic = 12582912.0f;
  const float abase = -((magic - v.bias) * v.a_scale);
  const float dbase = (v.delta_base + v.bias * v.delta_scale) - magic * v.delta_scale;
  std::vector<uint8_t> lds(info.bytes, 0);
  std::memcpy(lds.data() + info.hole, blob.data(), info.bytes - info.hole);
  for (uint32_t i = 0; i < 65536; ++i) {
    const float y = (float)i + magic;
    const float fs = std::fmaf(y, v.a_scale, abase);
    if (fs != ((float)i + v.bias) * v.a_scale) return false;
    const uint32_t a_addr = (f2u(fs) >> (v.shift - 2u)) & ~3u;
    const uint32_t d_addr = f2u(std::fmaf(y, v.delta_scale, dbase));
    if (a_addr < info.hole || a_addr + 4 > info.delta_off || d_addr != info.delta_off + 2 * i) return false;
    if (a_addr != info.hole + 4u * ((f2u((float)i + v.bias) >> v.shift) - info.first)) return false;
    uint32_t a;
    uint16_t d;
    std::memcpy(&a, lds.data() + a_addr, 4);
    std::memcpy(&d, lds.data() + d_addr, 2);
    if (a + d != p[i]) return false;
  }
  return true;
}

}
```

### phaneron_amd/csrc/ph_lut_host.h

```cpp
#pragma once
#include <stdint.h>
#include <vector>

#include "ph_lut.h"

namespace ph {

struct LutHostInfo {
  uint32_t bytes = 0, shift = 0, first = 0, n_anchors = 0, delta_off = 0, hole = 0;
  float bias = 0;
};

constexpr uint32_t kLutMaxLdsBytes = 160 * 1024;

bool lut_compress(const float *lut65536, uint32_t max_bytes, std::vector<uint32_t> &blob, LutHostInfo &info);
LutView lut_view(const LutHostInfo &info, const void *blob_dev);

}
```

Measured before the change: 20530.

## Add piecewise-linear predicted LUT form for the fused LDS v210 kernel

Adds a second compressed LUT layout in which each piece stores a float slope and base, and a 16-bit delta corrects the linear prediction. The fused v210 combine kernel uses it when both read and write LUTs compress and the width is a multiple of 48. With far fewer pieces per octave the LDS footprint shrinks, which could allow higher occupancy or faster LDS setup, at the cost of an extra FMA per lookup. Host-side LUT compression is also memoised by table hash, and the new form can be switched off with a context option.

```diff
diff --git a/include/phaneron_hip.h b/include/phaneron_hip.h
--- a/include/phaneron_hip.h
+++ b/include/phaneron_hip.h
@@ -333,6 +333,10 @@
   float a_scale;
 } ph_lut_layout;
 int ph_lut_layout_of(const float *host_lut65536, ph_lut_layout *layout, void *lds_image, size_t capacity);
+int ph_lut_pred_layout_of(const float *host_lut65536, ph_lut_layout *layout, uint32_t k5[5], void *lds_image, size_t capacity);
+int ph_lut_query_pred(ph_ctx *ctx, const void *device_lut_f32, uint32_t *pred_lds_bytes, uint32_t *pieces_per_octave_log2);
+int ph_fused_lut_form(ph_ctx *ctx, const void *rd_device_lut_f32, const void *wr_device_lut_f32, uint32_t width);
+int ph_fused_lut_form_of(const float *rd_host_lut65536, const float *wr_host_lut65536, int lds_lut_pred, uint32_t width);
 int ph_ctx_set_option(ph_ctx *ctx, const char *name, int value);
 int ph_debug_image_nt(ph_ctx *ctx, size_t bytes);
 
diff --git a/phaneron_amd/capi.py b/phaneron_amd/capi.py
--- a/phaneron_amd/capi.py
+++ b/phaneron_amd/capi.py
@@ -37,6 +37,7 @@
     "ph_debug_image_nt",
     "ph_clip_compose_multi",
     "ph_clip_compose_batch_out",
+    "ph_lut_pred_layout_of", "ph_lut_query_pred", "ph_fused_lut_form", "ph_fused_lut_form_of",
 ]
 
 
@@ -200,6 +201,10 @@
         "ph_lut_unregister": (ci, [vp, vp]),
         "ph_lut_query": (ci, [vp, vp, C.POINTER(cu), C.POINTER(cu), C.POINTER(cu)]),
         "ph_lut_layout_of": (ci, [f32p, C.POINTER(LutLayout), vp, C.c_size_t]),
+        "ph_lut_pred_layout_of": (ci, [f32p, C.POINTER(LutLayout), C.POINTER(cu), vp, C.c_size_t]),
+        "ph_lut_query_pred": (ci, [vp, vp, C.POINTER(cu), C.POINTER(cu)]),
+        "ph_fused_lut_form": (ci, [vp, vp, vp, cu]),
+        "ph_fused_lut_form_of": (ci, [f32p, f32p, ci, cu]),
         "ph_compose_up_write_v210_pair": (ci, [vp, ci, ci, C.POINTER(PhImageLayer), C.POINTER(PhImageLayer), vp, vp, cu, cu, cu, vp, vp]),
         "ph_compose_up_write_v210_batch": (ci, [vp, ci, ci, ci, C.POINTER(C.POINTER(PhImageLayer)), C.POINTER(vp), cu, cu, cu, vp, vp]),
         "ph_pack_read_batch": (ci, [vp, ci, ci, ci, C.POINTER(vp * 3), C.POINTER(vp), cu, cu, vp, vp, vp]),
@@ -297,6 +302,34 @@
     return {k: getattr(lay, k) for k, _ in LutLayout._fields_}, image
 
 
+LUT_FORM_NONE, LUT_FORM_ANCHOR, LUT_FORM_PRED = 0, 1, 2
+
+
+def lut_pred_layout(lut):
+    lut = np.ascontiguousarray(lut, np.float32)
+    assert lut.shape == (65536,)
+    lay = LutLayout()
+    k5 = (C.c_uint32 * 5)()
+    n = lib().ph_lut_pred_layout_of(lut, C.byref(lay), k5, None, 0)
+    if n < 0:
+        check(n)
+    if n == 0:
+        return None, None, None
+    image = np.zeros(n, np.uint8)
+    if lib().ph_lut_pred_layout_of(lut, C.byref(lay), k5, image.ctypes.data_as(C.c_void_p), n) != n:
+        check(-1)
+    return {k: getattr(lay, k) for k, _ in LutLayout._fields_}, np.array(list(k5), np.uint32), image
+
+
+def fused_lut_form_of(rd_lut, wr_lut, lds_lut_pred=1, width=3840):
+    rd, wr = np.ascontiguousarray(rd_lut, np.float32), np.ascontiguousarray(wr_lut, np.float32)
+    assert rd.shape == (65536,) and wr.shape == (65536,)
+    rc = lib().ph_fused_lut_form_of(rd, wr, int(lds_lut_pred), int(width))
+    if rc < 0:
+        check(rc)
+    return rc
+
+
 def gamma2linear_lut(colspec):
     out = np.empty(65536, np.float32)
     check(lib().ph_colour_gamma2linear_lut(colspec.encode(), out))
@@ -412,10 +445,20 @@
     def unregister_lut(self, device_lut):
         check(lib().ph_lut_unregister(self.h, _ptr(device_lut)), self.h)
 
-    def lut_info(self, device_lut):
+    def lut_info(self, device_lut, pred=False):
         b, t, s = C.c_uint32(), C.c_uint32(), C.c_uint32()
         check(lib().ph_lut_query(self.h, _ptr(device_lut), C.byref(b), C.byref(t), C.byref(s)), self.h)
-        return dict(lds_bytes=b.value, index_bias=t.value, blocks_per_octave_log2=s.value)
+        info = dict(lds_bytes=b.value, index_bias=t.value, blocks_per_octave_log2=s.value)
+        if pred:
+            check(lib().ph_lut_query_pred(self.h, _ptr(device_lut), C.byref(b), C.byref(s)), self.h)
+            info.update(pred_lds_bytes=b.value, pred_pieces_per_octave_log2=s.value)
+        return info
+
+    def fused_lut_form(self, rd_device_lut, wr_device_lut, width):
+        rc = lib().ph_fused_lut_form(self.h, _ptr(rd_device_lut), _ptr(wr_device_lut), int(width))
+        if rc < 0:
+            check(rc, self.h)
+        return rc
 
     def set_option(self, name, value):
         check(lib().ph_ctx_set_option(self.h, name.encode(), int(value)), self.h)
diff --git a/phaneron_amd/csrc/ph_api.cpp b/phaneron_amd/csrc/ph_api.cpp
--- a/phaneron_amd/csrc/ph_api.cpp
+++ b/phaneron_amd/csrc/ph_api.cpp
@@ -808,17 +808,18 @@
 
 int ph_lut_unregister(ph_ctx *ctx, const void *dev) {
   if (!ctx) return fail(PH_E_INVALID, "ph_lut_unregister: ctx is NULL");
-  void *blob = nullptr;
+  void *blob = nullptr, *pred_blob = nullptr;
   {
     std::lock_guard<std::mutex> lock(ctx->mu);
     auto it = ctx->luts.find(dev);
     if (it == ctx->luts.end()) return PH_OK;
-    blob = it->second.blob_dev;
+    blob = it->second.blob_dev, pred_blob = it->second.pred_blob_dev;
     ctx->luts.erase(it);
   }
-  if (blob) {
+  if (blob || pred_blob) {
     for (int q = 0; q < 3; ++q) hipStreamSynchronize(ctx->streams[q]);
-    hipFree(blob);
+    if (blob) hipFree(blob);
+    if (pred_blob) hipFree(pred_blob);
   }
   return PH_OK;
 }
@@ -847,6 +848,18 @@
     PH_HIP(hipMalloc(&e.blob_dev, blob_bytes));
     PH_HIP(hipMemcpy(e.blob_dev, blob.data(), blob_bytes, hipMemcpyHostToDevice));
     e.view = ph::lut_view(info, e.blob_dev);
+    ph::LutHostInfo pinfo;
+    if (ph::lut_compress_pred(host, ph::kLutMaxLdsBytes, blob, pinfo)) {
+      const size_t pred_bytes = blob.size() * sizeof(uint32_t);
+      hipError_t pe = hipMalloc(&e.pred_blob_dev, pred_bytes);
+      if (pe == hipSuccess) pe = hipMemcpy(e.pred_blob_dev, blob.data(), pred_bytes, hipMemcpyHostToDevice);
+      if (pe != hipSuccess) {
+        if (e.pred_blob_dev) hipFree(e.pred_blob_dev);
+        hipFree(e.blob_dev);
+        return fail(PH_E_HIP, "ph_lut_register: the predicted form's upload failed: %s", hipGetErrorString(pe));
+      }
+      e.pred = ph::lut_view(pinfo, e.pred_blob_dev);
+    }
   }
   {
     std::lock_guard<std::mutex> lock(ctx->mu);
@@ -872,6 +885,53 @@
   return (int)info.bytes;
 }
 
+int ph_lut_pred_layout_of(const float *host, ph_lut_layout *layout, uint32_t k5[5], void *lds_image, size_t capacity) {
+  if (!host || !layout) return fail(PH_E_INVALID, "ph_lut_pred_layout_of: NULL argument");
+  std::vector<uint32_t> blob;
+  ph::LutHostInfo info;
+  memset(layout, 0, sizeof(*layout));
+  if (!ph::lut_compress_pred(host, ph::kLutMaxLdsBytes, blob, info)) return 0;
+  const ph::LutView v = ph::lut_view(info, nullptr);
+  layout->lds_bytes = info.bytes, layout->hole = info.hole, layout->delta_off = info.delta_off, layout->shift = info.shift;
+  layout->index_bias = (uint32_t)info.bias, layout->a_scale = v.a_scale;
+  if (k5) {
+    const ph::FusedLutK k = ph::fused_lut_k(v, 1);
+    memcpy(k5, &k, 5 * sizeof(uint32_t));
+  }
+  if (lds_image) {
+    if (capacity < info.bytes) return fail(PH_E_INVALID, "ph_lut_pred_layout_of: the image needs %u bytes, %zu given", info.bytes, capacity);
+    memset(lds_image, 0, info.hole);
+    memcpy(static_cast<char *>(lds_image) + info.hole, blob.data(), info.bytes - info.hole);
+  }
+  return (int)info.bytes;
+}
+
+int ph_fused_lut_form_of(const float *rd_host, const float *wr_host, int lds_lut_pred, uint32_t width) {
+  if (!rd_host || !wr_host) return fail(PH_E_INVALID, "ph_fused_lut_form_of: NULL argument");
+  std::vector<uint32_t> blob;
+  ph::LutHostInfo rd, wr, rd_pred, wr_pred;
+  if (!ph::lut_compress(rd_host, ph::kLutMaxLdsBytes, blob, rd) || !ph::lut_compress(wr_host, ph::kLutMaxLdsBytes, blob, wr)) return 0;
+  const bool have_rd = ph::lut_compress_pred(rd_host, ph::kLutMaxLdsBytes, blob, rd_pred);
+  const bool have_wr = ph::lut_compress_pred(wr_host, ph::kLutMaxLdsBytes, blob, wr_pred);
+  return 1 + ph::fused_lut_form(lds_lut_pred != 0, have_rd ? rd_pred.bytes : 0, have_wr ? wr_pred.bytes : 0, width);
+}
+int ph_fused_lut_form(ph_ctx *ctx, const void *rd_dev, const void *wr_dev, uint32_t width) {
+  if (!ctx) return fail(PH_E_INVALID, "ph_fused_lut_form: ctx is NULL");
+  std::lock_guard<std::mutex> lock(ctx->mu);
+  auto r = ctx->luts.find(rd_dev), w = ctx->luts.find(wr_dev);
+  if (!ctx->use_lds_lut || r == ctx->luts.end() || w == ctx->luts.end() || !r->second.view.bytes || !w->second.view.bytes) return 0;
+  return 1 + ph::fused_lut_form(ctx->use_lds_lut_pred, r->second.pred.bytes, w->second.pred.bytes, width);
+}
+int ph_lut_query_pred(ph_ctx *ctx, const void *dev, uint32_t *pred_lds_bytes, uint32_t *pieces_per_octave_log2) {
+  if (!ctx) return fail(PH_E_INVALID, "ph_lut_query_pred: ctx is NULL");
+  std::lock_guard<std::mutex> lock(ctx->mu);
+  auto it = ctx->luts.find(dev);
+  const bool have = it != ctx->luts.end() && it->second.pred.bytes;
+  if (pred_lds_bytes) *pred_lds_bytes = have ? it->second.pred.bytes : 0;
+  if (pieces_per_octave_log2) *pieces_per_octave_log2 = have ? 23 - it->second.pred.shift : 0;
+  return PH_OK;
+}
+
 int ph_debug_fused_lut_k(const float *host, uint32_t k5[5]) {
   if (!host || !k5) return fail(PH_E_INVALID, "ph_debug_fused_lut_k: NULL argument");
   std::vector<uint32_t> blob;
@@ -904,6 +964,7 @@
 int ph_ctx_set_option(ph_ctx *ctx, const char *name, int value) {
   if (!ctx || !name) return fail(PH_E_INVALID, "ph_ctx_set_option: NULL argument");
   if (0 == strcmp(name, "lds_lut")) return ctx->use_lds_lut = (value != 0), PH_OK;
+  if (0 == strcmp(name, "lds_lut_pred")) return ctx->use_lds_lut_pred = (value != 0), PH_OK;
   if (0 == strcmp(name, "stream_images")) {
     if (value < 0 || value > 2) return fail(PH_E_INVALID, "stream_images: 0 (cached), 1 (streamed) or 2 (by size)");
     return ctx->stream_images = value, PH_OK;
@@ -955,6 +1016,7 @@
 
 struct LutRef {
   ph::LutView view{};
+  ph::LutView pred{};
   bool found = false;
   const ph::LutView *get() const { return found ? &view : nullptr; }
 };
@@ -965,6 +1027,7 @@
   auto it = ctx->luts.find(dev);
   if (it == ctx->luts.end() || !it->second.view.bytes) return r;
   r.view = it->second.view, r.found = true;
+  if (ctx->use_lds_lut_pred) r.pred = it->second.pred;
   return r;
 }
 
@@ -1075,7 +1138,8 @@
     const LutRef rref = lds_view(ctx, rd_lut), wref = lds_view(ctx, wr_lut);
     const ph::LutView *rv = rref.get(), *wv = wref.get();
     if (rv && wv) {
-      const ph::FusedLdsArgs la = ph::fused_lds_args(a, *rv, *wv);
+      const int form = ph::fused_lut_form(true, rref.pred.bytes, wref.pred.bytes, width);
+      const ph::FusedLdsArgs la = ph::fused_lds_args(a, form ? rref.pred : *rv, form ? wref.pred : *wv, form);
       PH_LAUNCH(ph::launch_fused_v210_combine_lds(stream_of(ctx, queue), n, la, (uint32_t)ctx->props.multiProcessorCount));
     }
   }
@@ -1119,7 +1183,8 @@
   f.total_quads = f.quads_per_line_used * height;
   f.rd_cm = (const float *)rd_cm, f.rd_lut = (const float *)rd_lut, f.rd_gm = (const float *)rd_gm;
   f.wr_cm = (const float *)wr_cm, f.wr_lut = (const float *)wr_lut;
-  ph::FusedLdsArgs la = ph::fused_lds_args(f, *rv, *wv);
+  const int form = ph::fused_lut_form(true, rref.pred.bytes, wref.pred.bytes, width);
+  ph::FusedLdsArgs la = ph::fused_lds_args(f, form ? rref.pred : *rv, form ? wref.pred : *wv, form);
   la.jobs = (uint32_t)jobs;
   for (int j = 1; j < jobs; ++j) {
     for (int l = 0; l < n; ++l) la.more_layers[j - 1][l] = layers[(size_t)j * n + l];
diff --git a/phaneron_amd/csrc/ph_internal.h b/phaneron_amd/csrc/ph_internal.h
--- a/phaneron_amd/csrc/ph_internal.h
+++ b/phaneron_amd/csrc/ph_internal.h
@@ -28,12 +28,15 @@
 struct LutEntry {
   ph::LutView view{};
   void *blob_dev = nullptr;
+  ph::LutView pred{};
+  void *pred_blob_dev = nullptr;
 };
 
 struct ph_ctx {
   int device = 0;
   std::map<const void *, LutEntry> luts;
   bool use_lds_lut = true;
+  bool use_lds_lut_pred = true;
   int stream_images = 0;
   int stream_threshold_mb = 64;
   hipStream_t streams[3] = {nullptr, nullptr, nullptr};
diff --git a/phaneron_amd/csrc/ph_kernels.h b/phaneron_amd/csrc/ph_kernels.h
--- a/phaneron_amd/csrc/ph_kernels.h
+++ b/phaneron_amd/csrc/ph_kernels.h
@@ -32,7 +32,10 @@
   float a_scale, a_base, delta_scale, delta_base;
   uint32_t a_shift;
 };
-FusedLutK fused_lut_k(const LutView &v);
+FusedLutK fused_lut_k(const LutView &v, int form = 0);
+static inline int fused_lut_form(bool allowed, uint32_t rd_pred_bytes, uint32_t wr_pred_bytes, uint32_t width) {
+  return allowed && rd_pred_bytes && wr_pred_bytes && width % 48u == 0 ? 1 : 0;
+}
 
 static inline uint32_t fused_wg_magic(uint32_t wg_per_job) { return (uint32_t)(((1ull << 31) + wg_per_job - 1) / wg_per_job); }
 static inline __host__ __device__ uint32_t fused_job_of(uint32_t block, uint32_t magic) {
@@ -60,6 +63,7 @@
   uint32_t quads_per_line_used;
   uint32_t quads_per_line_pitch;
   uint32_t tail_px, magic_qpp;
+  uint32_t lut_form;
   const void *more_layers[kMaxBatch - 1][kMaxLayers];
   void *more_out[kMaxBatch - 1];
 };
@@ -75,7 +79,7 @@
               offsetof(FusedLdsArgs, quads_per_line_used) == 188 && offsetof(FusedLdsArgs, quads_per_line_pitch) == kFusedHeadBytes,
               "line 2 of the fused kernel's head");
 static_assert(offsetof(FusedLdsArgs, more_layers) >= kFusedHeadBytes, "the batch arrays lie behind the head");
-FusedLdsArgs fused_lds_args(const FusedArgs &f, const LutView &rd, const LutView &wr);
+FusedLdsArgs fused_lds_args(const FusedArgs &f, const LutView &rd, const LutView &wr, int form = 0);
 
 constexpr int kMaxFusedOuts = 4;
 struct FusedOut {
diff --git a/phaneron_amd/csrc/ph_kernels_lds.hip b/phaneron_amd/csrc/ph_kernels_lds.hip
--- a/phaneron_amd/csrc/ph_kernels_lds.hip
+++ b/phaneron_amd/csrc/ph_kernels_lds.hip
@@ -133,13 +133,13 @@
 __device__ __forceinline__ void static_for(F &&f) {
   static_for_each(std::make_integer_sequence<int, COUNT>{}, f);
 }
-template <int PLACE, bool STD>
+template <int PLACE, bool STD, int FORM = kLutAnchor>
 __device__ __forceinline__ void fused_layer_combine(float (&acc)[18], const uint4 w, const ReadK &rk, const LutK &rlut, float last) {
   __builtin_amdgcn_sched_barrier(0);
   const Yuv6 q = unpack_quad(w);
 #pragma unroll
   for (int j = 0; j < 6; ++j) {
-    const float4 t = read_px_lds<STD>(q.y[j], q.cb[j >> 1], q.cr[j >> 1], rk, rlut, last);
+    const float4 t = read_px_lds<STD, FORM>(q.y[j], q.cb[j >> 1], q.cr[j >> 1], rk, rlut, last);
     if (PLACE & kLayerFirst) {
       acc[3 * j] = t.x, acc[3 * j + 1] = t.y, acc[3 * j + 2] = t.z;
       if (PLACE & kLayerLast) {
@@ -166,9 +166,10 @@
   return (trunc ? __builtin_floorf(x) : x) + kRoundMagic;
 }
 
-template <int N, int P, int BS, bool PIPE = false, int MODE = 0, bool TAIL = false>
+template <int N, int P, int BS, bool PIPE = false, int MODE = 0, bool TAIL = false, int FORM = kLutAnchor>
 __global__ __launch_bounds__(BS) void fused_v210_combine_lds_kernel(FusedLdsArgs a, uint32_t *handoff = nullptr) {
   static_assert(!TAIL || (!PIPE && MODE == 0), "the tail instantiation exists for the shipped form only");
+  static_assert(FORM == kLutAnchor || (!PIPE && MODE == 0 && !TAIL), "the predicted table form exists for the shipped form of whole 48-pixel blocks only");
   PH_STAMP_ENTRY();
   FusedHead head = fused_head_load();
   const uint32_t total_quads = head.word(offsetof(FusedLdsArgs, total_quads)), wg_per_job = head.word(offsetof(FusedLdsArgs, wg_per_job));
@@ -280,7 +281,7 @@
       float acc[18];
       constexpr bool STD = decltype(tag)::value;
       auto combine = [&](auto place, const uint4 word) __attribute__((always_inline)) {
-        fused_layer_combine<decltype(place)::value, STD>(acc, word, rk, rlut, last);
+        fused_layer_combine<decltype(place)::value, STD, FORM>(acc, word, rk, rlut, last);
       };
       constexpr std::integral_constant<int, N == 1 ? (kLayerFirst | kLayerLast) : kLayerFirst> first_layer{};
       constexpr std::integral_constant<int, 0> middle_layer{};
@@ -502,11 +503,11 @@
         uint4 packed;
         if (TAIL) {
           const uint32_t kind = slot_kind(f < wg_end ? f : wg_end - 1);
-          if (kind == 0u) packed = write_quad_idx_lds(yi, wk, wlut);
-          else if (kind == 1u) packed = write_quad_idx_lds_tail(yi, wk, wlut, a.tail_px);
+          if (kind == 0u) packed = write_quad_idx_lds<FORM>(yi, wk, wlut);
+          else if (kind == 1u) packed = write_quad_idx_lds_tail<FORM>(yi, wk, wlut, a.tail_px);
           else packed = make_uint4(0u, 0u, 0u, 0u);
         } else {
-          packed = write_quad_idx_lds(yi, wk, wlut);
+          packed = write_quad_idx_lds<FORM>(yi, wk, wlut);
         }
         if (f < wg_end) store_stream(out_ptr + f, packed);
       }
@@ -1017,7 +1018,7 @@
   return e;
 }
 
-FusedLutK fused_lut_k(const LutView &v) {
+FusedLutK fused_lut_k(const LutView &v, int form) {
 #if defined(__x86_64__)
   const unsigned csr = __builtin_ia32_stmxcsr();
   __builtin_ia32_ldmxcsr(csr & ~0x8040u);
@@ -1025,18 +1026,19 @@
   const volatile float lds0 = 0.0f, magic = 12582912.0f;
   const float small = (v.delta_base + lds0) + v.bias * v.delta_scale;
   const float b = small - magic * v.delta_scale;
-  const FusedLutK k{v.a_scale, -((magic - v.bias) * v.a_scale), v.delta_scale, b, v.shift - 2u};
+  const FusedLutK k{v.a_scale, -((magic - v.bias) * v.a_scale), v.delta_scale, b, v.shift - (form == kLutPred ? 3u : 2u)};
 #if defined(__x86_64__)
   __builtin_ia32_ldmxcsr(csr);
 #endif
   return k;
 }
 
-FusedLdsArgs fused_lds_args(const FusedArgs &f, const LutView &rd, const LutView &wr) {
+FusedLdsArgs fused_lds_args(const FusedArgs &f, const LutView &rd, const LutView &wr, int form) {
   FusedLdsArgs a{};
+  a.lut_form = (uint32_t)form;
   a.rd_blob = rd.blob, a.rd_bytes = rd.bytes, a.rd_hole = rd.hole;
   a.wr_blob = wr.blob, a.wr_bytes = wr.bytes, a.wr_hole = wr.hole;
-  a.rd_k = fused_lut_k(rd), a.wr_k = fused_lut_k(wr);
+  a.rd_k = fused_lut_k(rd, form), a.wr_k = fused_lut_k(wr, form);
   for (int l = 0; l < kMaxLayers; ++l) a.layers[l] = f.layers[l];
   a.out = f.out, a.rd_cm = f.rd_cm, a.rd_gm = f.rd_gm, a.wr_cm = f.wr_cm;
   a.total_quads = f.total_quads, a.quads_per_line_used = f.quads_per_line_used, a.quads_per_line_pitch = f.quads_per_line_pitch;
@@ -1062,7 +1064,7 @@
 }
 #endif
 
-template <int N, int P, int BS, bool PIPE = false, bool TAIL = false>
+template <int N, int P, int BS, bool PIPE = false, bool TAIL = false, int FORM = kLutAnchor>
 static hipError_t launch_fused_npb(hipStream_t s, const FusedLdsArgs &a, uint32_t grid_in, uint32_t lds) {
   uint32_t grid = grid_in;
 #if PH_FUSED_SPLIT
@@ -1073,7 +1075,7 @@
   if (cus_env > 0 && (uint32_t)cus_env < grid) grid = (uint32_t)cus_env;
 #endif
   static std::atomic<uint64_t> lds_allowed{0};
-  hipError_t e = allow_lds_once(fused_v210_combine_lds_kernel<N, P, BS, PIPE, 0, TAIL>, lds_allowed);
+  hipError_t e = allow_lds_once(fused_v210_combine_lds_kernel<N, P, BS, PIPE, 0, TAIL, FORM>, lds_allowed);
   if (e != hipSuccess) return e;
   const uint32_t slices = (a.total_quads + BS - 1) / BS;
   FusedLdsArgs b = a;
@@ -1096,7 +1098,7 @@
     }
   }
 #endif
-  fused_v210_combine_lds_kernel<N, P, BS, PIPE, 0, TAIL><<<b.wg_per_job * b.jobs, BS, lds, s>>>(b);
+  fused_v210_combine_lds_kernel<N, P, BS, PIPE, 0, TAIL, FORM><<<b.wg_per_job * b.jobs, BS, lds, s>>>(b);
   return hipGetLastError();
 }
 
@@ -1106,6 +1108,9 @@
     const char *e = getenv("PH_FUSED_GEOM");
     return e ? atoi(e) : 0;
   }();
+  if (a.lut_form == (uint32_t)kLutPred)
+    return a.quads_per_line_used != a.quads_per_line_pitch ? hipErrorInvalidValue : launch_fused_npb<N, 6, 1024, false, false, kLutPred>(s, a, grid, lds);
+  if (a.lut_form != (uint32_t)kLutAnchor) return hipErrorInvalidValue;
   if (a.quads_per_line_used != a.quads_per_line_pitch) return launch_fused_npb<N, 6, 1024, false, true>(s, a, grid, lds);
   int geom = geom_env ? geom_env : 6;
   static const int pipe_env = [] {
diff --git a/phaneron_amd/csrc/ph_ldslut.h b/phaneron_amd/csrc/ph_ldslut.h
--- a/phaneron_amd/csrc/ph_ldslut.h
+++ b/phaneron_amd/csrc/ph_ldslut.h
@@ -41,6 +41,7 @@
   float delta_scale, delta_base;
   uint32_t a_shift;
 };
+constexpr int kLutAnchor = 0, kLutPred = 1;
 typedef const __attribute__((address_space(3))) uint32_t *lds_u32_ptr;
 typedef const __attribute__((address_space(3))) uint16_t *lds_u16_ptr;
 __device__ __forceinline__ LutK make_lut_k(const LutView &v) {
@@ -76,6 +77,30 @@
 #endif
   return __uint_as_float(a + d);
 }
+typedef float lds_f32x2 __attribute__((ext_vector_type(2)));
+typedef const __attribute__((address_space(3))) lds_f32x2 *lds_f32x2_ptr;
+__device__ __forceinline__ float lds_lut_fetch_pred(const LutK &k, float y) {
+  const uint32_t e_addr = (__float_as_uint(fma_rn(y, k.a_scale, k.a_base)) >> k.a_shift) & ~7u;
+  const uint32_t d_addr = __float_as_uint(fma_rn(y, k.delta_scale, k.delta_base));
+#if PH_ABLATE & 8
+  const lds_f32x2 e = *(lds_f32x2_ptr)(e_addr & 8u);
+  const uint32_t d = *(lds_u16_ptr)(d_addr & 2u);
+#elif PH_ABLATE & 1
+  const lds_f32x2 e = {__uint_as_float(e_addr), __uint_as_float(e_addr)};
+  const uint32_t d = d_addr;
+#elif PH_ABLATE & 4
+  const lds_f32x2 e = *(lds_f32x2_ptr)e_addr;
+  const uint32_t d = d_addr;
+#else
+  const lds_f32x2 e = *(lds_f32x2_ptr)e_addr;
+  const uint32_t d = *(lds_u16_ptr)d_addr;
+#endif
+  return __uint_as_float(__float_as_uint(fma_rn(y, e.x, e.y)) + d);
+}
+template <int FORM>
+__device__ __forceinline__ float lds_lut_fetch_as(const LutK &k, float y) {
+  return FORM == kLutPred ? lds_lut_fetch_pred(k, y) : lds_lut_fetch(k, y);
+}
 struct LutPending {
   uint32_t a, d;
 };
@@ -119,12 +144,13 @@
   return lds_lut_fetch(k, lds_lut_index_unit(t));
 }
 
+template <int FORM = kLutAnchor>
 __device__ __forceinline__ uint4 write_quad_idx_lds(const float (&yi)[18], const WriteK &wk, const LutK &lut) {
   uint32_t y[6], u[3], v[3];
 #pragma unroll
   for (int j = 0; j < 6; ++j) {
-    const float gr = lds_lut_fetch(lut, yi[3 * j]), gg = lds_lut_fetch(lut, yi[3 * j + 1]);
-    const float gb = lds_lut_fetch(lut, yi[3 * j + 2]);
+    const float gr = lds_lut_fetch_as<FORM>(lut, yi[3 * j]), gg = lds_lut_fetch_as<FORM>(lut, yi[3 * j + 1]);
+    const float gb = lds_lut_fetch_as<FORM>(lut, yi[3 * j + 2]);
     y[j] = sat_u16_rte(dot4(gr, gg, gb, 1.0f, wk.y));
     if ((j & 1) == 0) {
       u[j >> 1] = sat_u16_rte(dot4(gr, gg, gb, 1.0f, wk.u));
@@ -134,12 +160,13 @@
   return pack_quad(y, u, v);
 }
 
+template <int FORM = kLutAnchor>
 __device__ __forceinline__ uint4 write_quad_idx_lds_tail(const float (&yi)[18], const WriteK &wk, const LutK &lut, uint32_t remain) {
   uint32_t y[4], u[2], v[2];
 #pragma unroll
   for (int j = 0; j < 4; ++j) {
-    const float gr = lds_lut_fetch(lut, yi[3 * j]), gg = lds_lut_fetch(lut, yi[3 * j + 1]);
-    const float gb = lds_lut_fetch(lut, yi[3 * j + 2]);
+    const float gr = lds_lut_fetch_as<FORM>(lut, yi[3 * j]), gg = lds_lut_fetch_as<FORM>(lut, yi[3 * j + 1]);
+    const float gb = lds_lut_fetch_as<FORM>(lut, yi[3 * j + 2]);
     y[j] = sat_u16_trunc(__builtin_roundf(dot4(gr, gg, gb, 1.0f, wk.y)));
     if ((j & 1) == 0) {
       u[j >> 1] = sat_u16_trunc(__builtin_roundf(dot4(gr, gg, gb, 1.0f, wk.u)));
@@ -170,7 +197,7 @@
 __device__ __forceinline__ bool ycbcr_matrix_is_standard(const ReadK &k) {
   return k.r.y == 0.0f && k.b.z == 0.0f && k.r.x == k.g.x && k.g.x == k.b.x;
 }
-template <bool STD = false>
+template <bool STD = false, int FORM = kLutAnchor>
 __device__ __forceinline__ float4 read_px_lds(float y, float cb, float cr, const ReadK &k, const LutK &lut, float last = 1.0f) {
   float tr, tg, tb;
   if (STD) {
@@ -181,9 +208,9 @@
   } else {
     tr = dot4(y, cb, cr, last, k.r), tg = dot4(y, cb, cr, last, k.g), tb = dot4(y, cb, cr, last, k.b);
   }
-  const float r = lds_lut_at_unit(lut, tr);
-  const float g = lds_lut_at_unit(lut, tg);
-  const float b = lds_lut_at_unit(lut, tb);
+  const float r = lds_lut_fetch_as<FORM>(lut, lds_lut_index_unit(tr));
+  const float g = lds_lut_fetch_as<FORM>(lut, lds_lut_index_unit(tg));
+  const float b = lds_lut_fetch_as<FORM>(lut, lds_lut_index_unit(tb));
   return make_float4(dot3(r, g, b, k.gm[0], k.gm[1], k.gm[2]), dot3(r, g, b, k.gm[3], k.gm[4], k.gm[5]),
                      dot3(r, g, b, k.gm[6], k.gm[7], k.gm[8]), 1.0f);
 }
diff --git a/phaneron_amd/csrc/ph_lut.cpp b/phaneron_amd/csrc/ph_lut.cpp
--- a/phaneron_amd/csrc/ph_lut.cpp
+++ b/phaneron_amd/csrc/ph_lut.cpp
@@ -3,6 +3,8 @@
 #include <algorithm>
 #include <cmath>
 #include <cstring>
+#include <deque>
+#include <mutex>
 
 namespace ph {
 
@@ -16,6 +18,50 @@
   float f;
   std::memcpy(&f, &u, 4);
   return f;
+}
+
+constexpr size_t kMemoTables = 8;
+struct Memo {
+  uint64_t hash;
+  uint32_t max_bytes;
+  std::vector<uint32_t> table, blob;
+  LutHostInfo info;
+  bool ok;
+};
+std::mutex g_memo_mu;
+std::deque<Memo> g_memo[2];
+
+uint64_t table_hash(const float *lut) {
+  uint64_t h = 0xcbf29ce484222325ull, w;
+  for (uint32_t i = 0; i < 65536; i += 2) {
+    std::memcpy(&w, lut + i, 8);
+    h = (h ^ w) * 0x100000001b3ull;
+    h ^= h >> 29;
+  }
+  return h;
+}
+template <typename F>
+bool memoised(int form, const float *lut, uint32_t max_bytes, std::vector<uint32_t> &blob, LutHostInfo &info, F &&compress) {
+  const uint64_t hash = table_hash(lut);
+  {
+    std::lock_guard<std::mutex> lock(g_memo_mu);
+    for (const Memo &m : g_memo[form])
+      if (m.hash == hash && m.max_bytes == max_bytes && 0 == std::memcmp(m.table.data(), lut, 65536 * sizeof(float))) {
+        if (m.ok) blob = m.blob, info = m.info;
+        return m.ok;
+      }
+  }
+  Memo m;
+  m.hash = hash, m.max_bytes = max_bytes;
+  m.ok = compress(lut, max_bytes, m.blob, m.info);
+  m.table.resize(65536);
+  std::memcpy(m.table.data(), lut, 65536 * sizeof(float));
+  if (m.ok) blob = m.blob, info = m.info;
+  const bool ok = m.ok;
+  std::lock_guard<std::mutex> lock(g_memo_mu);
+  g_memo[form].push_front(std::move(m));
+  if (g_memo[form].size() > kMemoTables) g_memo[form].pop_back();
+  return ok;
 }
 }
 
@@ -32,7 +78,7 @@
   return v;
 }
 
-bool lut_compress(const float *lut, uint32_t max_bytes, std::vector<uint32_t> &blob, LutHostInfo &info) {
+static bool compress_anchor(const float *lut, uint32_t max_bytes, std::vector<uint32_t> &blob, LutHostInfo &info) {
   std::vector<uint32_t> p(65536), blk(65536);
   std::memcpy(p.data(), lut, 65536 * sizeof(uint32_t));
   bool found = false;
@@ -88,4 +134,145 @@
   return true;
 }
 
-}
+namespace {
+constexpr float kMagic = 12582912.0f;
+constexpr int kSlopeSteps = 48;
+
+struct PieceFit {
+  const uint32_t *p;
+  uint32_t i0, i1;
+  std::vector<double> lo, hi;
+  PieceFit(const uint32_t *p_, uint32_t a, uint32_t b) : p(p_), i0(a), i1(b), lo(b - a + 1), hi(b - a + 1) {
+    for (uint32_t i = i0; i <= i1; ++i) {
+      hi[i - i0] = (double)u2f(p[i]);
+      lo[i - i0] = (double)u2f(p[i] > 65535u ? p[i] - 65535u : 0u);
+    }
+  }
+  void bases(double s, double &b_lo, double &b_hi, uint32_t step = 1) const {
+    b_lo = -INFINITY, b_hi = INFINITY;
+    if (step > 1) {
+      const double sy = s * (double)(kMagic + (float)i1);
+      b_lo = lo[i1 - i0] - sy, b_hi = hi[i1 - i0] - sy;
+    }
+    for (uint32_t i = i0; i <= i1; i += step) {
+      const double sy = s * (double)(kMagic + (float)i);
+      b_lo = std::max(b_lo, lo[i - i0] - sy);
+      b_hi = std::min(b_hi, hi[i - i0] - sy);
+    }
+  }
+  bool verify(float s, float b) const {
+    for (uint32_t i = i0; i <= i1; ++i) {
+      const uint32_t q = f2u(std::fmaf(kMagic + (float)i, s, b));
+      if ((q >> 31) || q > p[i] || p[i] - q > 65535u) return false;
+    }
+    return true;
+  }
+  bool try_slope(float s, float &base) const {
+    double b_lo, b_hi;
+    bases(s, b_lo, b_hi);
+    if (!(b_lo <= b_hi)) return false;
+    float c[3] = {(float)(0.5 * (b_lo + b_hi)), (float)b_hi, (float)b_lo};
+    if ((double)c[1] > b_hi) c[1] = std::nextafterf(c[1], -INFINITY);
+    if ((double)c[2] < b_lo) c[2] = std::nextafterf(c[2], INFINITY);
+    for (float b : c)
+      if ((double)b >= b_lo && (double)b <= b_hi && verify(s, b)) return base = b, true;
+    return false;
+  }
+  bool fit(float &slope, float &base) const {
+    if (i0 == i1) return slope = 0.0f, base = u2f(p[i0]), verify(slope, base);
+    const uint32_t step = (i1 - i0) / 32u + 1u;
+    return fit_from(step, slope, base) || (step > 1 && fit_from(1, slope, base));
+  }
+  bool fit_from(uint32_t step, float &slope, float &base) const {
+    const double n = (double)(i1 - i0);
+    double a = (lo[i1 - i0] - hi[0]) / n, b = (hi[i1 - i0] - lo[0]) / n;
+    for (int it = 0; it < 48; ++it) {
+      const double m1 = a + (b - a) / 3.0, m2 = b - (b - a) / 3.0;
+      double l1, h1, l2, h2;
+      bases(m1, l1, h1, step), bases(m2, l2, h2, step);
+      if (h1 - l1 < h2 - l2) a = m1;
+      else b = m2;
+    }
+    float down = (float)(0.5 * (a + b)), up = down;
+    if (try_slope(down, base)) return slope = down, true;
+    for (int k = 0; k < kSlopeSteps; ++k) {
+      down = std::nextafterf(down, -INFINITY), up = std::nextafterf(up, INFINITY);
+      if (try_slope(down, base)) return slope = down, true;
+      if (try_slope(up, base)) return slope = up, true;
+    }
+    return false;
+  }
+};
+}
+
+static bool compress_pred(const float *lut, uint32_t max_bytes, std::vector<uint32_t> &blob, LutHostInfo &info) {
+#if defined(__x86_64__)
+  struct KeepDenormals {
+    unsigned csr = __builtin_ia32_stmxcsr();
+    KeepDenormals() { __builtin_ia32_ldmxcsr(csr & ~0x8040u); }
+    ~KeepDenormals() { __builtin_ia32_ldmxcsr(csr); }
+  } keep_denormals;
+#endif
+  std::vector<uint32_t> p(65536), piece(65536);
+  std::memcpy(p.data(), lut, 65536 * sizeof(uint32_t));
+  for (uint32_t i = 0; i < 65536; ++i)
+    if ((p[i] >> 31) || p[i] >= 0x7f800000u) return false;
+  for (uint32_t m = 3; m <= 5; ++m) {
+    for (float bias : {128.0f, 64.0f, 32.0f, 16.0f}) {
+      const uint32_t shift = 23 - m;
+      const uint32_t first = f2u(bias) >> shift;
+      const uint32_t n_pieces = (f2u(65535.0f + bias) >> shift) - first + 1;
+      const uint32_t n_entries = (n_pieces + 1) & ~1u;
+      const uint32_t hole = 8u << m;
+      const uint32_t bytes = hole + n_entries * 8 + 65536 * 2;
+      if (bytes > max_bytes) continue;
+      for (uint32_t i = 0; i < 65536; ++i) piece[i] = (f2u((float)i + bias) >> shift) - first;
+      blob.assign((bytes - hole) / 4, 0);
+      uint16_t *delta = reinterpret_cast<uint16_t *>(blob.data() + 2 * n_entries);
+      bool ok = true;
+      for (uint32_t i0 = 0; i0 < 65536 && ok;) {
+        uint32_t i1 = i0;
+        while (i1 + 1 < 65536 && piece[i1 + 1] == piece[i0]) ++i1;
+        float slope, base;
+        ok = PieceFit(p.data(), i0, i1).fit(slope, base);
+        if (ok) {
+          blob[2 * piece[i0]] = f2u(slope), blob[2 * piece[i0] + 1] = f2u(base);
+          for (uint32_t i = i0; i <= i1; ++i) delta[i] = (uint16_t)(p[i] - f2u(std::fmaf(kMagic + (float)i, slope, base)));
+        }
+        i0 = i1 + 1;
+      }
+      if (!ok) continue;
+      info.bytes = bytes, info.shift = shift, info.first = first, info.n_anchors = n_entries;
+      info.hole = hole, info.delta_off = hole + n_entries * 8, info.bias = bias;
+      const LutView v = lut_view(info, nullptr);
+      const float abase = -((kMagic - v.bias) * v.a_scale);
+      const float dbase = (v.delta_base + v.bias * v.delta_scale) - kMagic * v.delta_scale;
+      std::vector<uint8_t> lds(info.bytes, 0);
+      std::memcpy(lds.data() + info.hole, blob.data(), info.bytes - info.hole);
+      for (uint32_t i = 0; i < 65536 && ok; ++i) {
+        const float y = (float)i + kMagic;
+        const uint32_t e_addr = (f2u(std::fmaf(y, v.a_scale, abase)) >> (v.shift - 3u)) & ~7u;
+        const uint32_t d_addr = f2u(std::fmaf(y, v.delta_scale, dbase));
+        ok = e_addr == info.hole + 8u * piece[i] && e_addr + 8 <= info.delta_off && d_addr == info.delta_off + 2 * i;
+        if (!ok) break;
+        float e[2];
+        uint16_t d;
+        std::memcpy(e, lds.data() + e_addr, 8);
+        std::memcpy(&d, lds.data() + d_addr, 2);
+        const uint32_t q = f2u(std::fmaf(y, e[0], e[1]));
+        ok = !(q >> 31) && q + d == p[i];
+      }
+      if (ok) return true;
+    }
+  }
+  return false;
+}
+
+bool lut_compress(const float *lut, uint32_t max_bytes, std::vector<uint32_t> &blob, LutHostInfo &info) {
+  return memoised(0, lut, max_bytes, blob, info, compress_anchor);
+}
+bool lut_compress_pred(const float *lut, uint32_t max_bytes, std::vector<uint32_t> &blob, LutHostInfo &info) {
+  return memoised(1, lut, max_bytes, blob, info, compress_pred);
+}
+
+}
diff --git a/phaneron_amd/csrc/ph_lut_host.h b/phaneron_amd/csrc/ph_lut_host.h
--- a/phaneron_amd/csrc/ph_lut_host.h
+++ b/phaneron_amd/csrc/ph_lut_host.h
@@ -14,6 +14,7 @@
 constexpr uint32_t kLutMaxLdsBytes = 160 * 1024;
 
 bool lut_compress(const float *lut65536, uint32_t max_bytes, std::vector<uint32_t> &blob, LutHostInfo &info);
+bool lut_compress_pred(const float *lut65536, uint32_t max_bytes, std::vector<uint32_t> &blob, LutHostInfo &info);
 LutView lut_view(const LutHostInfo &info, const void *blob_dev);
 
 }
```

New measurement: 20820, median of 6. 1.01x the previous value.
